# birdnet-team/birdnet-stm32

Hardware: AMD Instinct MI355X
Metric: audio chunks/sec (3 s @ 24 kHz) (higher is better)
Workload: dtype i8

## Files before the change

### birdnet-stm32_amd/birdnet_stm32/_hip.py

```python

from __future__ import annotations

import ctypes
import os
from ctypes import POINTER, byref, c_char_p, c_float, c_int, c_int32, c_int64, c_size_t, c_void_p

_PKG_ROOT = os.path.dirname(os.path.dirname(os.path.abspath(__file__)))
LIB_PATH = os.path.join(_PKG_ROOT, "lib", "libbirdnet_hip.so")

ABI_VERSION = 2

EXPORTS = (
    "bn_version", "bn_last_error", "bn_device_count", "bn_ctx_create", "bn_ctx_destroy", "bn_model_load",
    "bn_model_free", "bn_model_get_info", "bn_stft_mag", "bn_forward", "bn_infer_audio", "bn_debug_op_output",
    "bn_kernel_names", "bn_profile_enable", "bn_profile_collect", "bn_ingest_resample", "bn_ingest_chunks",
    "bn_pool_scores", "bn_mel_spectrogram", "bn_profile_only", "bn_chunk_peak_normalize", "bn_set_option", "bn_get_option", "bn_ctx_set_option", "bn_ctx_get_option", "bn_ctx_reset_options", "bn_preload_kernels", "bn_host_alloc_pinned", "bn_host_free_pinned", "bn_rank_orders",
    "bn_blob_check", "bn_debug_requant", "bn_stft_mag_exact", "bn_debug_input_bytes", "bn_debug_guard_stats", "bn_debug_tail_form", "bn_debug_mid_form", "bn_debug_mid_plan", "bn_debug_mid_split_giveups",
    "bn_forward_embed", "bn_infer_audio_embed", "bn_model_get_embedding_info", "bn_ingest_resample_span",
    "bn_head_forward", "bn_probe_create", "bn_probe_destroy", "bn_probe_epoch", "bn_probe_loss", "bn_probe_get", "bn_probe_set",
    "bn_probe_sweep_create", "bn_probe_sweep_destroy", "bn_probe_sweep_epoch", "bn_probe_sweep_loss", "bn_probe_sweep_snapshot", "bn_probe_sweep_get",
    "bn_probe_set_loss", "bn_probe_epoch_weighted", "bn_probe_sweep_set_loss", "bn_probe_sweep_epoch_weighted",
    "bn_probe_set_qat", "bn_probe_get_quantized", "bn_probe_scores",
    "bn_short_time_energy", "bn_activity_counts", "bn_search_inv_norms", "bn_search_topk", "bn_augment_inputs",
    "bn_kmeans_assign", "bn_kmeans_accumulate", "bn_kmeans_centroids",
    "bn_tsne_perplexity", "bn_tsne_gradient", "bn_tsne_update",
    "bn_bootstrap_rejections", "bn_bootstrap_counts", "bn_bootstrap_ap", "bn_head_i8_forward", "bn_head_i8_pass_classes",
)

EMB_F32, EMB_I8 = 0, 1
PROBE_ACTIVATIONS = {"sigmoid": 0, "softmax": 1}
PROBE_OPTIMIZERS = {"adam": 0, "adamw": 1, "sgd": 2}
PROBE_LOSSES = {"auto": 0, "focal": 1}
PROBE_QAT_WEIGHTS = {"off": 0, "per_class": 1, "per_tensor": 2}
PROBE_MAX_D, PROBE_MAX_C = 2048, 4096
PROBE_SWEEP_MAX_TRIALS = 64
PROBE_SWEEP_CURRENT, PROBE_SWEEP_SNAPSHOT = 0, 1
HEAD_I8_STEP_ROWS, HEAD_I8_MIN_WG_STEPS, HEAD_I8_MAX_WGS, HEAD_I8_LDS_BYTES = 64, 8, 1024, 160 * 1024



def head_i8_pass_classes(D: int, C: int) -> int:
    v = int(load_library().bn_head_i8_pass_classes(int(D), int(C)))
    check(min(v, 0))
    return v


class ProbeTrialStruct(ctypes.Structure):

    _fields_ = [("optimizer", ctypes.c_int32), ("lr", ctypes.c_float), ("weight_decay", ctypes.c_float), ("clipnorm", ctypes.c_float),
                ("dropout", ctypes.c_float), ("label_smoothing", ctypes.c_float)]


DTYPE_F32, DTYPE_I8 = 0, 1
SEARCH_METRICS = {"cosine": 0, "dot": 1}
SEARCH_MAX_K, SEARCH_MAX_D = 128, 2048
AUGMENT_MAX_MASKS = 4
SEARCH_STEP_ROWS, SEARCH_MIN_WG_STEPS, SEARCH_MAX_WGS = 64, 8, 1024
KMEANS_MAX_K, KMEANS_MAX_D = 4096, 2048
BOOTSTRAP_MAX_N = 32768
KMEANS_LDS_BYTES, KMEANS_MAX_TILE, KMEANS_STEP_ROWS, KMEANS_MIN_WG_STEPS, KMEANS_MAX_WGS, KMEANS_SEGMENT_ROWS = 160 * 1024, 128, 64, 8, 1024, 256
TSNE_TILE_I, TSNE_TILE_J, TSNE_SPLIT_J, TSNE_ROW_LANES, TSNE_MAX_K, TSNE_MAX_N = 256, 1024, 4096, 16, 128, 1 << 21


def kmeans_tile_centroids(D: int, K: int) -> int:
    pitch_bytes = (-(-int(D) // 64) * 64 + 4) * 4
    nt = 1
    while nt < KMEANS_MAX_TILE // 16 and 16 * nt < K:
        nt *= 2
    while nt > 1 and 16 * nt * pitch_bytes > KMEANS_LDS_BYTES:
        nt //= 2
    return 16 * nt


OPTION_NAMES = ("f32_strip", "f32_strip_th", "f32_front_staged", "f32_front2", "f32_pwdw", "f32_tile_slice", "f32_pw_ws", "i8_pwdw", "i8_pw_lds", "i8_pw_forms", "i8_add_tab", "front_tpw", "wave_dwpw", "i8_strip", "i8_strip_mfdw", "i8_strip_th", "i8_dw_pool", "i8_tail_fclds", "i8_tail", "i8_tail_mfdw", "i8_mid",
                "i8_mel_generic", "stft_rowmajor", "stft_exact", "stft_flagcap", "stft_guard", "stft_audit", "stft_minint", "ingest_blk", "ingest_generic")
SCHEDULING_OPTION_NAMES = ("i8_mid_split",)


class BnModelInfo(ctypes.Structure):
    _fields_ = [
        ("dtype", c_int32), ("input_kind", c_int32), ("input_elems", c_int32), ("fft_bins", c_int32),
        ("spec_width", c_int32), ("num_classes", c_int32), ("n_ops", c_int32), ("max_batch", c_int32),
        ("workspace_bytes", c_int64), ("const_bytes", c_int64),
    ]


class HipError(RuntimeError):
    """A libbirdnet_hip call returned a negative status."""


_lib = None


def load_library(path: str | None = None):
    global _lib
    if _lib is not None:
        return _lib
    path = path or os.environ.get("BIRDNET_HIP_LIB", LIB_PATH)
    if not os.path.isfile(path):
        raise RuntimeError(
            f"{path} not found: the HIP extension has not been built. Run `python -c 'import __graft_entry__ as g; "
            "g.build()'` (or `make -C birdnet-stm32_amd/csrc`). There is no CPU fallback for this path."
        )
    import torch

    lib = ctypes.CDLL(path)
    for name in EXPORTS:
        if not hasattr(lib, name):
            raise RuntimeError(f"{path} does not export {name}")
    lib.bn_version.restype = c_int
    lib.bn_last_error.restype = c_char_p
    lib.bn_device_count.restype = c_int
    lib.bn_ctx_create.argtypes = [c_int, c_int, POINTER(c_void_p)]
    lib.bn_ctx_destroy.argtypes = [c_void_p]
    lib.bn_ctx_destroy.restype = None
    lib.bn_model_load.argtypes = [c_void_p, c_char_p, c_size_t, POINTER(c_void_p)]
    lib.bn_model_free.argtypes = [c_void_p]
    lib.bn_model_free.restype = None
    lib.bn_model_get_info.argtypes = [c_void_p, POINTER(BnModelInfo)]
    lib.bn_stft_mag.argtypes = [c_void_p, c_void_p, c_int, c_int, c_int, c_int, c_int, c_int, c_void_p, c_void_p, c_void_p]
    lib.bn_stft_mag_exact.argtypes = lib.bn_stft_mag.argtypes
    lib.bn_debug_input_bytes.argtypes = [c_void_p, c_int, c_void_p, c_void_p]
    lib.bn_debug_guard_stats.argtypes = [c_void_p, c_int, POINTER(c_int64)]
    lib.bn_debug_tail_form.argtypes = [c_void_p, POINTER(c_int), POINTER(c_int)]
    lib.bn_debug_mid_form.argtypes = [c_void_p, POINTER(c_int), POINTER(c_int)]
    lib.bn_debug_mid_plan.argtypes = [c_void_p, POINTER(c_int), c_int]
    lib.bn_debug_mid_split_giveups.argtypes = [c_void_p, POINTER(c_int64)]
    lib.bn_forward.argtypes = [c_void_p, c_void_p, c_void_p, c_int, c_void_p, c_void_p, c_void_p]
    lib.bn_infer_audio.argtypes = [c_void_p, c_void_p, c_int, c_int, c_int, c_void_p, c_void_p, c_void_p]
    lib.bn_forward_embed.argtypes = [c_void_p, c_void_p, c_void_p, c_int, c_void_p, c_void_p, c_void_p, c_int, c_void_p]
    lib.bn_infer_audio_embed.argtypes = [c_void_p, c_void_p, c_int, c_int, c_int, c_void_p, c_void_p, c_void_p, c_int, c_void_p]
    lib.bn_model_get_embedding_info.argtypes = [c_void_p, POINTER(c_int), POINTER(c_int), POINTER(c_float), POINTER(c_int)]
    lib.bn_debug_op_output.argtypes = [c_void_p, c_int, c_int, c_void_p, c_size_t, POINTER(c_size_t), c_void_p]
    lib.bn_kernel_names.restype = c_char_p
    lib.bn_profile_enable.argtypes = [c_void_p, c_int]
    lib.bn_profile_only.argtypes = [c_void_p, c_int]
    lib.bn_chunk_peak_normalize.argtypes = [c_void_p, c_void_p, c_int, c_int, c_float, c_void_p, c_void_p]
    lib.bn_profile_collect.argtypes = [c_void_p, POINTER(ctypes.c_double), POINTER(c_int64), c_int]
    lib.bn_ingest_resample.argtypes = [c_void_p, c_void_p, c_int, c_int, c_void_p, c_void_p, c_int, c_int64, c_int64,
                                       c_void_p, c_int, c_int, c_int, c_int, c_void_p, c_void_p, c_void_p]
    lib.bn_ingest_resample_span.argtypes = [c_void_p, c_void_p, c_int, c_int, c_int64, c_int64, c_int64, c_int64, c_int64, c_void_p,
                                            c_int, c_int, c_int, c_int, c_void_p, c_void_p, c_void_p]
    lib.bn_ingest_chunks.argtypes = [c_void_p, c_void_p, c_void_p, c_void_p, c_void_p, c_void_p, c_int, c_int, c_void_p,
                                     c_void_p]
    lib.bn_pool_scores.argtypes = [c_void_p, c_void_p, c_void_p, c_int, c_int, c_int, c_float, c_void_p, c_void_p]
    lib.bn_mel_spectrogram.argtypes = [c_void_p, c_void_p, c_int, c_int, c_int, c_int, c_int, c_void_p, c_void_p, c_int, c_int, c_int,
                                       ctypes.c_double, c_void_p, c_int, c_void_p, c_void_p, c_void_p]
    lib.bn_blob_check.argtypes = [c_char_p, c_size_t]
    lib.bn_debug_requant.argtypes = [c_void_p, c_void_p, c_void_p, c_void_p, c_int, c_int, c_int, c_void_p, c_void_p]
    lib.bn_set_option.argtypes = [c_char_p, c_int]
    lib.bn_get_option.argtypes = [c_char_p, POINTER(c_int)]
    lib.bn_ctx_set_option.argtypes = [c_void_p, c_char_p, c_int]
    lib.bn_ctx_get_option.argtypes = [c_void_p, c_char_p, POINTER(c_int)]
    lib.bn_ctx_reset_options.argtypes = [c_void_p]
    lib.bn_preload_kernels.argtypes = [c_void_p]
    lib.bn_rank_orders.argtypes = [c_void_p, c_void_p, c_int, c_int, c_void_p, c_void_p, c_void_p]
    lib.bn_short_time_energy.argtypes = [c_void_p, c_void_p, c_void_p, c_void_p, c_void_p, c_void_p, c_int, c_int, c_int, c_void_p, c_void_p]
    lib.bn_activity_counts.argtypes = [c_void_p, c_void_p, c_int, c_int64, c_void_p, c_int, c_float, c_void_p, c_void_p, c_void_p]
    lib.bn_search_inv_norms.argtypes = [c_void_p, c_void_p, c_int, c_int64, c_int, c_int, c_void_p, c_void_p]
    lib.bn_search_topk.argtypes = [c_void_p, c_void_p, c_int, c_int64, c_int, c_int, c_void_p, c_void_p, c_int64, c_void_p, c_int, c_void_p, c_void_p,
                                   c_int, c_void_p, c_void_p, c_void_p]
    lib.bn_kmeans_assign.argtypes = [c_void_p, c_void_p, c_int, c_int64, c_int, c_int, c_void_p, c_void_p, c_void_p, c_int, c_void_p, c_void_p, c_void_p,
                                     c_void_p, c_void_p]
    lib.bn_kmeans_accumulate.argtypes = [c_void_p, c_void_p, c_int, c_int64, c_int, c_int, c_void_p, c_void_p, c_int, c_int, c_void_p, c_void_p, c_void_p]
    lib.bn_kmeans_centroids.argtypes = [c_void_p, c_void_p, c_void_p, c_int, c_int, c_void_p, c_void_p, c_void_p]
    lib.bn_tsne_perplexity.argtypes = [c_void_p, c_void_p, c_int64, c_int, ctypes.c_double, c_void_p, c_void_p, c_void_p]
    lib.bn_tsne_gradient.argtypes = [c_void_p, c_void_p, c_int64, c_void_p, c_void_p, c_void_p, c_float, c_void_p, c_void_p, c_void_p, c_void_p]
    lib.bn_tsne_update.argtypes = [c_void_p, c_void_p, c_void_p, c_void_p, c_void_p, c_int64, c_float, c_float, c_void_p]
    u64 = ctypes.c_uint64
    lib.bn_bootstrap_rejections.argtypes = [c_void_p, u64, u64, u64, u64, ctypes.c_uint32, c_int64, c_int64, c_void_p, c_int64, POINTER(c_int64), c_void_p]
    lib.bn_bootstrap_counts.argtypes = [c_void_p, u64, u64, u64, u64, c_int, c_int, c_void_p, c_void_p, c_void_p]
    lib.bn_bootstrap_ap.argtypes = [c_void_p, u64, u64, u64, u64, c_int, c_int, c_void_p, c_void_p, c_void_p, c_void_p, c_int, c_int, c_void_p, c_void_p, c_void_p]
    lib.bn_augment_inputs.argtypes = [c_void_p, c_void_p, c_int64, c_int, c_int, c_void_p, c_void_p, c_void_p, c_void_p, c_int, c_void_p, c_int, c_int64,
                                      c_void_p, c_void_p]
    lib.bn_host_alloc_pinned.argtypes = [c_void_p, ctypes.c_size_t]
    lib.bn_host_alloc_pinned.restype = c_void_p
    lib.bn_host_free_pinned.argtypes = [c_void_p]
    lib.bn_head_forward.argtypes = [c_void_p, c_void_p, c_int64, c_int, c_void_p, c_void_p, c_int, c_int, c_void_p, c_void_p]
    lib.bn_head_i8_forward.argtypes = [c_void_p, c_void_p, c_int64, c_int, c_void_p, c_void_p, c_void_p, c_void_p, c_int, c_int, c_void_p, c_int, c_float,
                                       c_void_p, c_void_p, c_void_p]
    lib.bn_head_i8_pass_classes.argtypes = [c_int, c_int]
    lib.bn_probe_create.argtypes = [c_void_p, c_int, c_int, c_int, c_int, c_float, c_float, c_float, c_float, ctypes.c_uint32, c_int64,
                                    c_void_p, c_void_p, POINTER(c_void_p), c_void_p]
    lib.bn_probe_destroy.argtypes = [c_void_p]
    lib.bn_probe_destroy.restype = None
    lib.bn_probe_epoch.argtypes = [c_void_p, c_void_p, c_void_p, c_void_p, c_int64, c_int, c_void_p, c_void_p]
    lib.bn_probe_loss.argtypes = [c_void_p, c_void_p, c_void_p, c_int64, c_void_p, c_void_p]
    lib.bn_probe_get.argtypes = [c_void_p, c_void_p, c_void_p, c_void_p]
    lib.bn_probe_set.argtypes = [c_void_p, c_void_p, c_void_p, c_void_p]
    lib.bn_probe_sweep_create.argtypes = [c_void_p, c_int, c_int, c_int, c_int, POINTER(ProbeTrialStruct), ctypes.c_uint32, c_int64, c_void_p, c_void_p,
                                          POINTER(c_void_p), c_void_p]
    lib.bn_probe_sweep_destroy.argtypes = [c_void_p]
    lib.bn_probe_sweep_destroy.restype = None
    lib.bn_probe_sweep_epoch.argtypes = [c_void_p, c_void_p, c_void_p, c_void_p, c_int64, c_int, c_void_p, c_void_p, c_void_p, c_void_p]
    lib.bn_probe_sweep_loss.argtypes = [c_void_p, c_void_p, c_void_p, c_int64, c_void_p, c_void_p, c_void_p]
    lib.bn_probe_sweep_snapshot.argtypes = [c_void_p, c_void_p, c_void_p]
    lib.bn_probe_sweep_get.argtypes = [c_void_p, c_int, c_int, c_void_p, c_void_p, c_void_p]
    lib.bn_probe_set_loss.argtypes = [c_void_p, c_int, c_float]
    lib.bn_probe_epoch_weighted.argtypes = [c_void_p, c_void_p, c_void_p, c_void_p, c_void_p, c_int64, c_int, c_void_p, c_void_p]
    lib.bn_probe_sweep_set_loss.argtypes = [c_void_p, c_int, c_float]
    lib.bn_probe_set_qat.argtypes = [c_void_p, c_int, c_int, c_float, c_int]
    lib.bn_probe_get_quantized.argtypes = [c_void_p, c_void_p, c_void_p]
    lib.bn_probe_scores.argtypes = [c_void_p, c_void_p, c_int64, c_void_p, c_void_p, c_void_p]
    lib.bn_probe_sweep_epoch_weighted.argtypes = [c_void_p, c_void_p, c_void_p, c_void_p, c_void_p, c_int64, c_int, c_void_p, c_void_p, c_void_p, c_void_p]
    if lib.bn_version() != ABI_VERSION:
        raise RuntimeError(f"libbirdnet_hip ABI {lib.bn_version()} != binding ABI {ABI_VERSION}")
    _lib = lib
    return lib


# ... 120 lines not shown
```

### birdnet-stm32_amd/birdnet_stm32/models/_lower_i8.py

```python

from __future__ import annotations

import numpy as np

from birdnet_stm32.models import _pack as pk
from birdnet_stm32.models import _quant as qz
from birdnet_stm32.models._netspec import same_pad

K_ALIGN = 64


class _Graph:
    def __init__(self, model):
        self.m = model
        self.t = model.tensors
        self.consumers: dict[int, list[int]] = {}
        for op in model.ops:
            for ti in op.inputs:
                if ti >= 0:
                    self.consumers.setdefault(ti, []).append(op.index)

    def q(self, ti: int) -> tuple[float, int]:
        t = self.t[ti]
        if t.scale.size != 1:
# ... 892 lines not shown
            val[op.outputs[0]], shape[op.outputs[0]] = v, (C,)
            i += 1
        elif op.name == "FULLY_CONNECTED":
            Cin = int(shape[src][-1])
            _expect(int(np.prod(shape[src])) == Cin, "FULLY_CONNECTED input must be a vector per chunk")
            s_i, z_i = g.q(src)
            s_o, z_o = g.q(op.outputs[0])
            wt_ = t[op.inputs[1]]
            Cout = int(wt_.shape[0])
            _expect(int(wt_.shape[1]) == Cin, "FULLY_CONNECTED weight shape")
            mu, sh = qz.channel_multipliers(s_i, wt_.scale, s_o, Cout)
            a_lo, a_hi = qz.activation_bounds(op.options["activation"], s_o, z_o)
            b = g.const(op.inputs[2]).astype(np.int64) if len(op.inputs) > 2 and op.inputs[2] >= 0 else np.zeros(Cout, np.int64)
            b = b - z_i * wt_.data.astype(np.int64).sum(axis=1)
            _expect_acc_range(wt_.data, b, 1, f"fully connected operator #{op.index}", mu, sh)
            Kp = (Cin + 3) // 4 * 4
            w_pad = np.zeros((Cout, Kp), np.int8)
            w_pad[:, :Cin] = wt_.data
            nxt = ops[i + 1] if i + 1 < len(ops) else None
            fold_lut = (nxt is not None and nxt.name == "LOGISTIC" and nxt.inputs[0] == op.outputs[0] and g.consumers.get(op.outputs[0], []) == [nxt.index]
                        and i + 2 < len(ops) and ops[i + 2].name != "DEQUANTIZE")
            tt = dict(w=pb.tensor(w_pad, np.int8), bias=pb.tensor(b, np.int32), mult=pb.tensor(mu, np.int32), shift=pb.tensor(sh, np.int32))
            out_t = op.outputs[0]
            if fold_lut:
                s_h, z_h = g.q(nxt.outputs[0])
                tt["lut"] = pb.tensor(qz.logistic_table(s_o, z_o, s_h, z_h), np.int8)
                out_t = nxt.outputs[0]
            v = pb.value(Cout)
            if not fold_lut:
                tail_head.update(fc_op=len(plan.ops), fc_cin=Cin, NC=Cout, fc_zp_out=z_o, fc_lo=a_lo, fc_hi=a_hi, fc_w=wt_.data, fc_b=b, fc_m=mu, fc_s=sh)
            pb.op(pk.I8_FC, val[src], v, p=dict(Cin=Cin, Cout=Cout, zp_out=z_o, act_min=a_lo, act_max=a_hi, has_lut=int(fold_lut)), t=tt, name=f"t{out_t}", out_shape=(Cout,), out_dtype="int8")
            val[out_t], shape[out_t] = v, (Cout,)
            i += 2 if fold_lut else 1
        elif op.name == "MUL":
            a_t, b_t = op.inputs
            if len(shape[a_t]) != 3:
                a_t, b_t = b_t, a_t
            _expect(len(shape[a_t]) == 3 and int(np.prod(shape[b_t])) == shape[a_t][2] and shape[a_t][2] % 4 == 0, "MUL must scale a map by a per-channel vector")
            H, Wd, C = shape[a_t]
            s1, z1 = g.q(a_t)
            s2, z2 = g.q(b_t)
            so, zo = g.q(op.outputs[0])
            mu, sh = qz.quantize_multiplier(float(np.float32(s1)) * float(np.float32(s2)) / float(np.float32(so)))
            lo_, hi_ = qz.activation_bounds(op.options["activation"], so, zo)
            v = pb.value(H * Wd * C)
            pb.op(pk.I8_SCALE, val[a_t], v, in1=val[b_t], p=dict(P=H * Wd, C=C, zp_x=z1, zp_gate=z2, mult=mu, shift=sh, zp_out=zo, act_min=lo_, act_max=hi_),
                  name=f"t{op.outputs[0]}", out_shape=(H, Wd, C), out_dtype="int8")
            val[op.outputs[0]], shape[op.outputs[0]] = v, (H, Wd, C)
            i += 1
        elif op.name in ("LOGISTIC", "DEQUANTIZE"):
            fc_out = src
            _expect(len(shape[fc_out]) == 1, "the head must follow the classifier")
            Cout = shape[fc_out][0]
            s_fc, z_fc = g.q(fc_out)
            lut_t, s_h, z_h, has = -1, s_fc, z_fc, 0
            if op.name == "LOGISTIC":
                s_h, z_h = g.q(op.outputs[0])
                lut_t, has = pb.tensor(qz.logistic_table(s_fc, z_fc, s_h, z_h), np.int8), 1
                last = op.outputs[0]
                i += 1
            else:
                last = fc_out
            _expect(i < len(ops) and ops[i].name == "DEQUANTIZE" and ops[i].inputs[0] == last, "DEQUANTIZE must end the graph")
            softmax, beta = 0, 1.0
            if i + 1 < len(ops) and ops[i + 1].name == "SOFTMAX":
                _expect(not has and ops[i + 1].inputs[0] == ops[i].outputs[0], "float32 SOFTMAX must read the dequantised classifier output")
                softmax, beta = 1, float(ops[i + 1].options.get("beta", 1.0))
                i += 1
            if not softmax:
                tail_head.update(head_op=len(plan.ops), lut=qz.logistic_table(s_fc, z_fc, s_h, z_h) if has else None, zp_fc=z_fc, zp_head=z_h, s_fc=s_fc, s_head=s_h)
            pb.op(pk.I8_HEAD, val[fc_out], pk.SLOT_SCORES, p=dict(C=Cout, zp_fc=z_fc, zp_out=z_h, has_lut=has, softmax=softmax),
                  f=dict(s_fc=s_fc, s_out=s_h, beta=beta), t=dict(lut=lut_t), name=f"t{ops[i].outputs[0]}",
                  out_shape=(Cout,))
            i += 1
            _expect(i == len(ops), "operators after the head")
        else:
            _expect(False, f"operator #{op.index} {op.name} in the backbone")
    _mark_embedding(g, plan)
    if fuse and not keep_all:
        _add_tail_op(pb, plan, tail_blocks, tail_head)
        _tag_scale_pairs(pb)
        _tag_se_gates(pb)
        _tag_pwdw_pairs(pb)
    return pb.finalize(reuse=not keep_all)


def _mark_embedding(g: _Graph, plan: pk.Plan) -> None:
    ops = plan.ops
    writer = {o.out: i for i, o in enumerate(ops) if o.out >= 0}
    heads = [o for o in ops if o.kind == pk.I8_HEAD]
    if len(heads) != 1 or heads[0].in0 not in writer:
        return
    fc = ops[writer[heads[0].in0]]
    if fc.kind != pk.I8_FC or fc.in0 not in writer:
        return
    pool = ops[writer[fc.in0]]
    if pool.kind not in (pk.I8_MEAN, pk.I8_ATTNPOOL) or not pool.name.startswith("t"):
        return
    s, z = g.q(int(pool.name[1:]))
    pk.mark_embedding(pool, pool.get("C"), float(np.float32(s)), z)


def _tag_se_gates(pb: pk.PlanBuilder) -> None:
    ops = pb.plan.ops
    for i in range(len(ops) - 2):
        a, f1, f2 = ops[i], ops[i + 1], ops[i + 2]
        if a.kind != pk.I8_MEAN or f1.kind != pk.I8_FC or f2.kind != pk.I8_FC or f1.in0 != a.out or f2.in0 != f1.out:
            continue
        C, Cr = a.get("C"), f1.get("Cout")
        if f1.get("Cin") != C or f2.get("Cin") != Cr or Cr > 256 or C > 1024 or C % 4:
            continue
        others = [k for k, o in enumerate(ops) if (k != i + 1 and a.out in (o.in0, o.in1)) or (k != i + 2 and f1.out in (o.in0, o.in1))]
        if others or a.out < 0 or f1.out < 0 or f2.out < 0:
            continue
        a.p[pk.TAIL_TAG] = pk.SEGATE_HEAD
        f1.p[pk.TAIL_TAG] = f2.p[pk.TAIL_TAG] = pk.SEGATE_COVERED
        pb._extra_uses.append((i + 2, a.in0))


def _tag_pwdw_pairs(pb: pk.PlanBuilder) -> None:
    ops = pb.plan.ops
    for i in range(len(ops) - 1):
        e, d = ops[i], ops[i + 1]
        if e.kind != pk.I8_DWPW or d.kind != pk.I8_DW or any(e.get(k) for k in ("has_dw", "transposed", "has_add", "has_lut", "q_at_load")) or d.in0 != e.out or e.out < 0:
            continue
        if e.p[pk.TAIL_TAG] or d.p[pk.TAIL_TAG] or e.p[pk.OP_PATH] != d.p[pk.OP_PATH]:
            continue
        if d.get("C") != e.get("Cout") or (d.get("H"), d.get("W")) != (e.get("OH"), e.get("OW")) or d.get("zp_in") != e.get("pw_zp_out"):
            continue
        readers = [k for k, o in enumerate(ops) if k != i + 1 and e.out in (o.in0, o.in1)]
        writers = [k for k, o in enumerate(ops) if o.out == e.out]
        if readers or writers != [i]:
            continue
        e.p[pk.TAIL_TAG] = pk.PWDW8_HEAD
        d.p[pk.TAIL_TAG] = pk.PWDW8_COVERED
        if e.in0 >= 0:
            pb._extra_uses.append((i + 1, e.in0))


def _tag_scale_pairs(pb: pk.PlanBuilder) -> None:
    ops = pb.plan.ops
    for i in range(len(ops) - 1):
        a, b = ops[i], ops[i + 1]
        if a.kind != pk.I8_SCALE or b.kind != pk.I8_DWPW or any(b.get(k) for k in ("has_dw", "transposed", "has_lut", "q_at_load")) or b.in0 != a.out:
            continue
        if b.get("Cin") != a.get("C") or b.get("H") * b.get("W") != a.get("P") or b.get("Cin") > 768 or (b.get("sh"), b.get("sw")) != (1, 1):
            continue
        readers = [k for k, o in enumerate(ops) if k != i + 1 and a.out in (o.in0, o.in1)]
        if readers or b.in1 == a.out:
            continue
        a.p[pk.TAIL_TAG] = pk.SCALE_HEAD
        b.p[pk.TAIL_TAG] = pk.SCALE_COVERED
        pb._extra_uses.append((i + 1, a.in0))
        pb._extra_uses.append((i + 1, a.in1))


def _add_mid_op(pb, plan, blocks: list[dict]) -> None:
    if len(blocks) < 3:
        return
    chain = blocks[-3:]
    a, b, c = chain
    if (a["C"], a["N"], a["sh"], a["H"], a["W"], bool(a["add"][0])) != (32, 64, 2, 32, 64, False):
        return
    for blk in (b, c):
        if (blk["C"], blk["N"], blk["sh"], blk["H"], blk["W"], bool(blk["add"][0])) != (64, 64, 1, 16, 32, True) or not blk["res_is_input"]:
            return
    ops_idx = [blk["op"] for blk in chain]
# ... 55 lines not shown
```

### birdnet-stm32_amd/birdnet_stm32/models/runners.py

```python

from __future__ import annotations

import ctypes

import numpy as np

from birdnet_stm32 import _hip
from birdnet_stm32.models import _pack as pk


class HipRunner:

    def __init__(self, plan: pk.Plan, device: int = 0, max_batch: int = 1024, ctx: "_hip.Context | None" = None):
        import torch

        if not torch.cuda.is_available():
            raise RuntimeError("no ROCm device visible: HipRunner has no CPU fallback")
        self._torch = torch
        self.plan = plan
        self.device = torch.device("cuda", device)
        self.ctx = ctx if ctx is not None else _hip.Context(device, max_batch)
        self.model = _hip.Model(self.ctx, plan.to_blob())
        self.lib = self.ctx.lib
        info = self.model.info
# ... 150 lines not shown
        if self.input_kind in (pk.INPUT_MEL, pk.INPUT_WAVEFORM):
            res = self.predict_device(self.model_inputs_device(audio), return_logits=return_logits, **kw)
            if out is not None:
                out.copy_(res[0] if isinstance(res, tuple) else res)
            return res
        B, T = audio.shape
        hop = int(hop) if hop is not None else T // self.spec_width
        scores = out if out is not None else torch.empty((B, self.num_classes), dtype=torch.float32, device=self.device)
        logits = torch.empty_like(scores) if return_logits else None
        emb, code = (None, 0)
        if return_embeddings:
            emb, code = self._emb_buffer(B, emb_dtype, emb_out)
        with torch.cuda.device(self.device):
            for b0 in range(0, B, self.max_batch):
                nb = min(self.max_batch, B - b0)
                if emb is not None:
                    _hip.check(self.lib.bn_infer_audio_embed(self.model.handle, audio[b0:].data_ptr(), nb, T, hop, scores[b0:].data_ptr(),
                                                             logits[b0:].data_ptr() if logits is not None else None, emb[b0:].data_ptr(), code,
                                                             self._stream()))
                    continue
                _hip.check(
                    self.lib.bn_infer_audio(
                        self.model.handle, audio[b0:].data_ptr(), nb, T, hop, scores[b0:].data_ptr(),
                        logits[b0:].data_ptr() if logits is not None else None, self._stream(),
                    )
                )
        if emb is not None:
            return (scores, logits, emb) if return_logits else (scores, emb)
        return (scores, logits) if return_logits else scores

    def stft_device(self, audio, n_fft: int = 512, hop: int | None = None, spec_width: int | None = None, normalize: bool = True,
                    exact: bool = False):
        return stft_device(self.ctx, audio, n_fft, hop, spec_width or self.spec_width, normalize, exact=exact)

    def op_output(self, op_index: int, B: int) -> np.ndarray:
        torch = self._torch
        op = self.plan.ops[op_index]
        per = ctypes.c_size_t()
        _hip.check(self.lib.bn_debug_op_output(self.model.handle, op_index, B, None, 0, ctypes.byref(per), None))
        buf = torch.empty((B, per.value), dtype=torch.uint8, device=self.device)
        _hip.check(self.lib.bn_debug_op_output(self.model.handle, op_index, B, buf.data_ptr(), buf.numel(), ctypes.byref(per), self._stream()))
        torch.cuda.synchronize(self.device)
        raw = buf.cpu().numpy().reshape(-1)
        n = int(np.prod(op.out_shape))
        dt = np.dtype(op.out_dtype)
        return raw[: B * n * dt.itemsize].copy().view(dt).reshape(B, *op.out_shape)

    def input_bytes(self, B: int) -> np.ndarray:
        torch = self._torch
        out = torch.empty((B, self.fft_bins, self.spec_width), dtype=torch.int8, device=self.device)
        _hip.check(self.lib.bn_debug_input_bytes(self.model.handle, B, out.data_ptr(), self._stream()))
        torch.cuda.synchronize(self.device)
        return out.cpu().numpy()

    def guard_stats(self, B: int) -> dict:
        out = (ctypes.c_int64 * 8)()
        _hip.check(self.lib.bn_debug_guard_stats(self.model.handle, B, out))
        return {"listed": int(out[0]), "listed_max": int(out[1]), "dirty_blocks": int(out[2]), "whole_minmax": int(out[3]), "whole_fix": int(out[4]),
                "audited": int(out[5]), "audit_violations": int(out[6]), "interval_min": int(out[7])}

    def tail_form(self) -> tuple[int, int]:
        form, lds = ctypes.c_int(0), ctypes.c_int(0)
        _hip.check(self.lib.bn_debug_tail_form(self.model.handle, ctypes.byref(form), ctypes.byref(lds)))
        return form.value, lds.value

    def mid_form(self) -> tuple[int, int]:
        form, lds = ctypes.c_int(0), ctypes.c_int(0)
        _hip.check(self.lib.bn_debug_mid_form(self.model.handle, ctypes.byref(form), ctypes.byref(lds)))
        return form.value, lds.value

    def mid_plan(self) -> dict | None:
        out = (ctypes.c_int * 64)()
        _hip.check(self.lib.bn_debug_mid_plan(self.model.handle, out, 64))
        if not out[0]:
            return None
        parts = [(out[5 + 6 * i + 2 * k], out[6 + 6 * i + 2 * k]) for i in range(out[4]) for k in range(3) if out[6 + 6 * i + 2 * k]]
        return {"lds_bytes": out[1], "map_bytes": out[2], "bar_off": out[3], "blocks": out[4], "parts": parts}

    def mid_split_giveups(self) -> int:
        n = ctypes.c_int64(0)
        _hip.check(self.lib.bn_debug_mid_split_giveups(self.ctx.handle, ctypes.byref(n)))
        return int(n.value)

    def profile(self, enable: bool) -> None:
        _hip.check(self.lib.bn_profile_enable(self.model.handle, int(bool(enable))))

    def profile_only(self, op_index: int) -> None:
        _hip.check(self.lib.bn_profile_only(self.model.handle, int(op_index)))

    def profile_collect(self) -> list[dict]:
        n = len(self.plan.ops) + 3
        ms = (ctypes.c_double * n)()
        cnt = (ctypes.c_int64 * n)()
        _hip.check(self.lib.bn_profile_collect(self.model.handle, ms, cnt, n))
        rows = []
        for i in range(n):
            if i < len(self.plan.ops):
                op = self.plan.ops[i]
                rows.append({"op": i, "kind": pk.KIND_NAMES[op.kind], "name": op.name, "ms": ms[i], "launches": int(cnt[i]), "p": list(op.p)})
            else:
                kind, name = (("stft512", "stft"), ("stft_minmax_exact", "exact min/max"), ("stft512_f64_list", "float64 pass + redo"))[i - len(self.plan.ops)]
                rows.append({"op": i, "kind": kind, "name": name, "ms": ms[i], "launches": int(cnt[i]), "p": []})
        return rows

    def close(self):
        import sys

        pl = sys.modules.get("birdnet_stm32.audio.pipeline")
        if pl is not None:
            while pl._PREPARE:
                pl._PREPARE.pop().join()
        self.model.close()
        self.ctx.close()


def stft_device(ctx: _hip.Context, audio, n_fft: int = 512, hop: int | None = None, spec_width: int = 256, normalize: bool = True,
                return_minmax: bool = False, exact: bool = False):
    import torch

    if not (audio.is_cuda and audio.dtype == torch.float32 and audio.is_contiguous() and audio.dim() == 2):
        raise ValueError("audio must be a contiguous float32 CUDA tensor [B, T]")
    B, T = audio.shape
    hop = int(hop) if hop is not None else T // spec_width
    spec = torch.empty((B, n_fft // 2 + 1, spec_width), dtype=torch.float32, device=audio.device)
    minmax = torch.empty((B, 2), dtype=torch.float32, device=audio.device)
    with torch.cuda.device(audio.device):
        stream = ctypes.c_void_p(torch.cuda.current_stream(audio.device).cuda_stream)
        fn = ctx.lib.bn_stft_mag_exact if exact else ctx.lib.bn_stft_mag
        _hip.check(fn(ctx.handle, audio.data_ptr(), B, T, n_fft, hop, spec_width, int(normalize), spec.data_ptr(), minmax.data_ptr(), stream))
    return (spec, minmax) if return_minmax else spec


def lower_model_file(model_path: str, keep_all: bool = False, frontend_norm: bool | None = None, fuse: bool = True) -> pk.Plan:
    if model_path.lower().endswith(".tflite"):
        from birdnet_stm32.models._lower_i8 import lower_i8
        from birdnet_stm32.models._tflite_reader import load_tflite

        return lower_i8(load_tflite(model_path), keep_all=keep_all, fuse=fuse)
    from birdnet_stm32.models._keras_loader import load_keras_archive
    from birdnet_stm32.models._lower_f32 import lower_f32

    return lower_f32(load_keras_archive(model_path, frontend_norm=frontend_norm), keep_all=keep_all, fuse=fuse)


def load_model_runner(model_path: str, device: int = 0, max_batch: int = 1024, keep_all: bool = False,
                      frontend_norm: bool | None = None, fuse: bool = True, prepare_pipeline: bool = False) -> HipRunner:
    ctx = None
    if prepare_pipeline:
        import torch

        if not torch.cuda.is_available():
            raise RuntimeError("no ROCm device visible: HipRunner has no CPU fallback")
        from birdnet_stm32.audio.pipeline import prepare_for_evaluate

        ctx = _hip.Context(device, max_batch)
        prepare_for_evaluate(ctx, torch)
    plan = lower_model_file(model_path, keep_all=keep_all, frontend_norm=frontend_norm, fuse=fuse)
    return HipRunner(plan, device=device, max_batch=max_batch, ctx=ctx)
```

### birdnet-stm32_amd/csrc/bn_api.hip

```cpp
#include <hip/hip_runtime.h>

#include <algorithm>
#include <cctype>
#include <cmath>
#include <cstdarg>
#include <cstdio>
#include <cstdlib>
#include <cstring>
#include <string>
#include <vector>

#include "bn_model.h"

namespace {

thread_local std::string g_err;

constexpr int kFft = 512;

struct OptName {
    const char* name;
    int bn::Options::*field;
};
const OptName kOptions[] = {
    {"f32_strip", &bn::Options::f32_strip},       {"f32_strip_th", &bn::Options::f32_strip_th},
    {"f32_front_staged", &bn::Options::f32_front_staged}, {"f32_front2", &bn::Options::f32_front2}, {"f32_pwdw", &bn::Options::f32_pwdw}, {"f32_tile_slice", &bn::Options::f32_tile_slice}, {"f32_pw_ws", &bn::Options::f32_pw_ws}, {"i8_pwdw", &bn::Options::i8_pwdw}, {"i8_pw_lds", &bn::Options::i8_pw_lds}, {"i8_pw_forms", &bn::Options::i8_pw_forms}, {"i8_add_tab", &bn::Options::i8_add_tab}, {"front_tpw", &bn::Options::front_tpw},
    {"wave_dwpw", &bn::Options::wave_dwpw},       {"i8_strip", &bn::Options::i8_strip},
    {"i8_strip_th", &bn::Options::i8_strip_th}, {"i8_dw_pool", &bn::Options::i8_dw_pool}, {"i8_tail_fclds", &bn::Options::i8_tail_fclds},   {"i8_tail", &bn::Options::i8_tail}, {"i8_tail_mfdw", &bn::Options::i8_tail_mfdw}, {"i8_mid", &bn::Options::i8_mid}, {"i8_mid_split", &bn::Options::i8_mid_split},
    {"i8_mel_generic", &bn::Options::i8_mel_generic}, {"stft_rowmajor", &bn::Options::stft_rowmajor},
    {"i8_strip_mfdw", &bn::Options::i8_strip_mfdw}, {"stft_exact", &bn::Options::stft_exact}, {"stft_flagcap", &bn::Options::stft_flagcap}, {"stft_guard", &bn::Options::stft_guard}, {"stft_audit", &bn::Options::stft_audit}, {"stft_minint", &bn::Options::stft_minint},
    {"ingest_blk", &bn::Options::ingest_blk},
    {"ingest_generic", &bn::Options::ingest_generic},
};

bn::Options options_from_env() {
    bn::Options o;
    for (const OptName& e : kOptions) {
        std::string var = "BN_";
        for (const char* c = e.name; *c; ++c) var += (char)toupper((unsigned char)*c);
        if (const char* v = getenv(var.c_str())) o.*(e.field) = atoi(v);
    }
    return o;
}

}

namespace bn {
thread_local Options g_opt;

int fail(int code, const char* fmt, ...) {
    char buf[512];
    va_list ap;
    va_start(ap, fmt);
    vsnprintf(buf, sizeof buf, fmt, ap);
    va_end(ap);
    g_err = buf;
    return code;
}
}
using bn::fail;
using bn::kMaxGridBatch;
using bn::ProfScope;

bn::Options g_opt_default = options_from_env();
std::mutex g_opt_mu;

namespace bn {

int check_device(bn_ctx* ctx) {
    if (!ctx) return fail(BN_ERR_ARG, "null context");
    HIP_TRY(hipSetDevice(ctx->device));
    {
        std::lock_guard<std::mutex> lock(g_opt_mu);
        bn::g_opt = g_opt_default;
        for (const auto& ov : ctx->opt_override) bn::g_opt.*(ov.first) = ov.second;
    }
    return BN_OK;
}

int grow_device_buffer(void** p, size_t* have, size_t need, size_t alloc, hipStream_t s, int code, const char* what) {
    if (need <= *have) return BN_OK;
    HIP_TRY(hipStreamSynchronize(s));
    if (*p) (void)hipFree(*p);
    *p = nullptr;
    *have = 0;
    if (hipMalloc(p, alloc) != hipSuccess) {
        (void)hipGetLastError();
        return fail(code, "hipMalloc of %zu bytes for the %s workspace failed", alloc, what);
    }
    *have = alloc;
    return BN_OK;
}

}
using bn::check_device;
using bn::grow_device_buffer;

namespace {

int row_matrix_check(int dtype, int64_t n, int D, int max_D, int zero_point) {
    if (dtype != BN_DTYPE_F32 && dtype != BN_DTYPE_I8) return fail(BN_ERR_ARG, "unknown dtype %d", dtype);
    if (D < 1 || D > max_D) return fail(BN_ERR_ARG, "embedding width D=%d outside 1..%d", D, max_D);
    if (n < 0 || n > 0x7fffffffLL) return fail(BN_ERR_ARG, "bad row count %lld", (long long)n);
    if (dtype == BN_DTYPE_I8 && (zero_point < -128 || zero_point > 127)) return fail(BN_ERR_ARG, "zero point %d outside -128..127", zero_point);
    return BN_OK;
}

}

extern "C" {

int bn_version(void) { return BN_ABI_VERSION; }

// ... 444 lines not shown
    int rc = BN_OK;
    if (guarded) {
        if (T <= 0 || hop <= 0 || 1 + T / hop < W) rc = fail(BN_ERR_ARG, "T=%d hop=%d gives %d frames, fewer than spec_width=%d", T, hop, hop > 0 ? 1 + T / hop : 0, W);
        if (m->d_audit) HIP_TRY(hipMemsetAsync(m->d_audit, 0, 2 * sizeof(int), s));
        for (int b0 = 0; rc == BN_OK && b0 < B; b0 += kMaxGridBatch) {
            const int nb = B - b0 < kMaxGridBatch ? B - b0 : kMaxGridBatch;
            bn::StftGuard g = bn::guard_slice(m, (size_t)b0, bn::SpecStage{tiled, true, d_audio + (size_t)b0 * T, T, hop});
            {
                ProfScope prof(m, (int)m->ops.size(), s);
                bn::launch_stft512(m->ctx->tables, d_audio + (size_t)b0 * T, nb, T, hop, W, m->d_spec + b0 * in_stride, m->d_minmax + 2 * (size_t)b0, s,
                                   true, &g);
            }
            ProfScope prof(m, (int)m->ops.size() + 1, s);
            bn::launch_stft_minmax_exact(m->ctx->tables, d_audio + (size_t)b0 * T, nb, T, hop, W, m->d_spec + b0 * in_stride, true, g,
                                         m->d_minmax + 2 * (size_t)b0, s);
        }
    } else {
        ProfScope prof(m, (int)m->ops.size(), s);
        rc = stft_mag_impl(m->ctx, d_audio, B, T, kFft, hop, W, 0, m->d_spec, m->d_minmax, stream, tiled, exact_opt != 0);
    }
    if (rc == BN_OK) {
        for (int b0 = 0; b0 < B; b0 += kMaxGridBatch) {
            const int nb = B - b0 < kMaxGridBatch ? B - b0 : kMaxGridBatch;
            bn::RunArgs ra{m->d_spec + b0 * in_stride, m->d_minmax + 2 * (size_t)b0, nb, d_scores + b0 * C, d_logits ? d_logits + b0 * C : nullptr,
                           d_emb ? (char*)d_emb + b0 * D * esize : nullptr, emb_dtype, s};
            ra.slot_b0 = (size_t)b0;
            ra.spec = bn::SpecStage{tiled, guarded, d_audio + (size_t)b0 * T, T, hop};
            rc = bn::run_plan(m, ra);
            if (rc != BN_OK) break;
        }
    }
    m->last_tiled = tiled;
    m->last_B = rc == BN_OK ? B : 0;
    return rc;
}

extern "C" {

int bn_debug_tail_form(const bn_model* m, int* form, int* lds_bytes) {
    if (!m || !form || !lds_bytes) return fail(BN_ERR_ARG, "null argument");
    *form = 0;
    *lds_bytes = 0;
    for (size_t oi = 0; oi < m->ops.size(); ++oi) {
        if (m->ops[oi].kind != BN_OP_I8_TAIL || !m->prep[oi]->ok) continue;
        const bn::OpPrep& pr = *m->prep[oi];
        *form = pr.alt_ok ? 2 : 1;
        *lds_bytes = pr.alt_ok ? pr.chain.lds_bytes : pr.tail.lds_bytes;
    }
    return BN_OK;
}

int bn_debug_mid_form(const bn_model* m, int* form, int* lds_bytes) {
    if (!m || !form || !lds_bytes) return fail(BN_ERR_ARG, "null argument");
    *form = 0;
    *lds_bytes = 0;
    for (size_t oi = 0; oi < m->ops.size(); ++oi)
        if (m->ops[oi].kind == BN_OP_I8_MID && m->prep[oi]->ok) {
            *form = 1;
            *lds_bytes = m->prep[oi]->chain.lds_bytes;
        }
    return BN_OK;
}

int bn_debug_mid_plan(const bn_model* m, int* out, int n) {
    if (!m || !out || n < 1) return fail(BN_ERR_ARG, "null argument");
    out[0] = 0;
    for (size_t oi = 0; oi < m->ops.size(); ++oi)
        if (m->ops[oi].kind == BN_OP_I8_MID && m->prep[oi]->ok && m->prep[oi]->alt_ok) {
            if (!bn::tail2_plan_dump(m->prep[oi]->resident, out, n)) return fail(BN_ERR_ARG, "n=%d is too small for the plan", n);
            break;
        }
    return BN_OK;
}

int bn_debug_mid_split_giveups(bn_ctx* ctx, int64_t* count) {
    if (!ctx || !count) return fail(BN_ERR_ARG, "null argument");
    if (int rc = check_device(ctx)) return rc;
    const long n = bn::tail2_giveups();
    if (n < 0) return fail(BN_ERR_DEVICE, "could not read the chunk barriers' give-up counter");
    *count = n;
    return BN_OK;
}

int bn_debug_guard_stats(bn_model* m, int B, int64_t* out) {
    if (!m || !out) return fail(BN_ERR_ARG, "null argument");
    if (int rc = check_device(m->ctx)) return rc;
    if (!m->d_guard) return fail(BN_ERR_UNSUPPORTED, "the plan has no exactness pass");
    if (B <= 0 || B > m->last_B || B > kMaxGridBatch) return fail(BN_ERR_ARG, "B=%d: the last bn_infer_audio call left %d spectrograms", B, m->last_B);
    HIP_TRY(hipDeviceSynchronize());
    std::vector<int> cnt((size_t)B);
    int nw = 0, nh[2] = {0, 0};
    HIP_TRY(hipMemcpy(cnt.data(), m->guard.count, (size_t)B * sizeof(int), hipMemcpyDeviceToHost));
    HIP_TRY(hipMemcpy(&nw, m->guard.n_work, sizeof(int), hipMemcpyDeviceToHost));
    HIP_TRY(hipMemcpy(nh, m->guard.n_hard, 2 * sizeof(int), hipMemcpyDeviceToHost));
    int64_t total = 0, mx = 0;
    for (int c : cnt) {
        c %= m->guard.cap + 1;
        total += c;
        if (c > mx) mx = c;
    }
    out[0] = total;
    out[1] = mx;
    out[2] = nw;
    out[3] = nh[0];
    out[4] = nh[1];
    int au[2] = {0, 0};
    if (m->d_audit) HIP_TRY(hipMemcpy(au, m->d_audit, sizeof au, hipMemcpyDeviceToHost));
    out[5] = au[0];
    out[6] = au[1];
    std::vector<float> lo((size_t)B);
    HIP_TRY(hipMemcpy(lo.data(), m->guard.mn_lo, (size_t)B * sizeof(float), hipMemcpyDeviceToHost));
    int64_t wide = 0;
    for (float v : lo) wide += v >= 0.0f;
    out[7] = wide;
    return BN_OK;
}

int bn_debug_input_bytes(bn_model* m, int B, int8_t* d_out, void* stream) {
    if (!m || !d_out) return fail(BN_ERR_ARG, "null argument");
    if (int rc = check_device(m->ctx)) return rc;
    namespace k = bn::op::i8_dwpw;
    const OpRec* first = nullptr;
    for (const OpRec& o : m->ops)
        if (o.in0 == BN_SLOT_INPUT && o.kind == BN_OP_I8_DWPW && o.p[k::q_at_load] && o.p[k::transposed]) first = &o;
    if (!first || !m->d_spec) return fail(BN_ERR_UNSUPPORTED, "the plan's first operator is not the mel mixer with QUANTIZE fused into its load");
    if (B <= 0 || B > m->last_B || B > kMaxGridBatch) return fail(BN_ERR_ARG, "B=%d: the last bn_infer_audio call left %d spectrograms", B, m->last_B);
    bn::launch_spec_bytes(m->d_spec, m->d_minmax, B, (int)m->hdr.spec_width, m->last_tiled, first->f[k::qscale], first->p[k::qzp], d_out, (hipStream_t)stream);
    HIP_TRY(hipGetLastError());
    return BN_OK;
}

int bn_ingest_resample(bn_ctx* ctx, const void* d_pcm, int sample_format, int channels, const int64_t* d_in_off,
                       const int64_t* d_out_off, int n_windows, int64_t max_in_len, int64_t max_out_len, const float* d_taps,
                       int up, int down, int taps_per_phase, int n_pre_remove, float* d_mono, float* d_peak, void* stream) {
    if (int rc = check_device(ctx)) return rc;
    if (!d_pcm || !d_in_off || !d_out_off || !d_mono || !d_peak) return fail(BN_ERR_ARG, "null device pointer");
    if (sample_format < BN_PCM_S16 || sample_format > BN_PCM_F32) return fail(BN_ERR_ARG, "unknown sample format %d", sample_format);
    if (channels < 1 || channels > 8)
        return fail(BN_ERR_UNSUPPORTED, "%d channels: the channel mean is implemented for 1..8 channels", channels);
    if (n_windows < 0 || max_in_len < 0 || max_out_len < 0 || up < 1 || down < 1 || taps_per_phase < 0 || n_pre_remove < 0)
        return fail(BN_ERR_ARG, "bad ingest geometry");
    if (taps_per_phase > 0 && !d_taps) return fail(BN_ERR_ARG, "null filter");
    if (taps_per_phase == 0 && up != down) return fail(BN_ERR_ARG, "up=%d down=%d needs a filter", up, down);
    if (n_windows == 0 || max_out_len == 0) return BN_OK;
    if (n_windows > 65535) return fail(BN_ERR_ARG, "at most 65535 windows per call");
    if ((double)(max_out_len + n_pre_remove + 4096) * down >= 4294967296.0 || (double)max_in_len * up >= 4294967296.0)
        return fail(BN_ERR_UNSUPPORTED, "window too long for the 32-bit polyphase index (%lld samples, up=%d, down=%d)",
                    (long long)max_in_len, up, down);
    const size_t lds = bn::ingest_resample_lds_bytes(up, down, taps_per_phase, bn::ingest_resample_block(up, down, taps_per_phase));
    const bool fast_kernel = (up == 1 && (down == 2 || down == 4)) || (up > 1 && up <= 256 && (taps_per_phase == 21 || taps_per_phase == 29 || taps_per_phase == 39));
    if (lds > (fast_kernel ? 64 : 156) * 1024)
        return fail(BN_ERR_UNSUPPORTED, "resampling ratio %d/%d needs %zu bytes of LDS per workgroup (limit %d)", up, down, lds, (fast_kernel ? 64 : 156) * 1024);
    hipStream_t s = (hipStream_t)stream;
    const size_t need = bn::ingest_partial_elems(n_windows, (long)max_out_len, up, down, taps_per_phase);
    if (need > ctx->block_peaks_elems) {
        if (ctx->d_block_peaks) HIP_TRY(hipFree(ctx->d_block_peaks));
        ctx->d_block_peaks = nullptr;
        ctx->block_peaks_elems = 0;
        HIP_TRY(hipMalloc(&ctx->d_block_peaks, need * sizeof(float)));
        ctx->block_peaks_elems = need;
    }
    bn::launch_ingest_resample(d_pcm, sample_format, channels, (const long*)d_in_off, (const long*)d_out_off, n_windows,
                               (long)max_out_len, d_taps, up, down, taps_per_phase, n_pre_remove, d_mono, ctx->d_block_peaks,
                               d_peak, s);
    HIP_TRY(hipGetLastError());
    return BN_OK;
// ... 220 lines not shown

int bn_ctx_set_option(bn_ctx* ctx, const char* name, int value) {
    if (!ctx || !name) return fail(BN_ERR_ARG, "null argument");
    for (const OptName& e : kOptions)
        if (strcmp(name, e.name) == 0) {
            std::lock_guard<std::mutex> lock(g_opt_mu);
            for (auto& ov : ctx->opt_override)
                if (ov.first == e.field) {
                    ov.second = value;
                    return BN_OK;
                }
            ctx->opt_override.emplace_back(e.field, value);
            return BN_OK;
        }
    return fail(BN_ERR_ARG, "unknown option '%s'", name);
}

int bn_ctx_get_option(bn_ctx* ctx, const char* name, int* value) {
    if (!ctx || !name || !value) return fail(BN_ERR_ARG, "null argument");
    for (const OptName& e : kOptions)
        if (strcmp(name, e.name) == 0) {
            std::lock_guard<std::mutex> lock(g_opt_mu);
            *value = g_opt_default.*(e.field);
            for (const auto& ov : ctx->opt_override)
                if (ov.first == e.field) *value = ov.second;
            return BN_OK;
        }
    return fail(BN_ERR_ARG, "unknown option '%s'", name);
}

int bn_ctx_reset_options(bn_ctx* ctx) {
    if (!ctx) return fail(BN_ERR_ARG, "null context");
    std::lock_guard<std::mutex> lock(g_opt_mu);
    ctx->opt_override.clear();
    return BN_OK;
}

void* bn_host_alloc_pinned(bn_ctx* ctx, size_t bytes) {
    if (!ctx || bytes == 0) {
        fail(BN_ERR_ARG, "null context or empty allocation");
        return nullptr;
    }
    if (check_device(ctx) != BN_OK) return nullptr;
    void* p = nullptr;
    if (hipHostMalloc(&p, bytes, hipHostMallocDefault) != hipSuccess) {
        (void)hipGetLastError();
        fail(BN_ERR_DEVICE, "hipHostMalloc of %zu bytes failed", bytes);
        return nullptr;
    }
    return p;
}

int bn_host_free_pinned(void* p) {
    if (p && hipHostFree(p) != hipSuccess) {
        (void)hipGetLastError();
        return fail(BN_ERR_DEVICE, "hipHostFree failed");
    }
    return BN_OK;
}

int bn_preload_kernels(bn_ctx* ctx) {
    if (!ctx) return fail(BN_ERR_ARG, "null context");
    if (int rc = check_device(ctx)) return rc;
    bn::preload_ingest(); bn::preload_stft(); bn::preload_stft_exact(); bn::preload_i8_fused(); bn::preload_i8_strip(); bn::preload_i8_tail2();
    bn::preload_i8_tail(); bn::preload_i8(); bn::preload_i8_pw(); bn::preload_f32(); bn::preload_f32_fused(); bn::preload_f32_strip();
    bn::preload_f32_pw(); bn::preload_melspec(); bn::preload_sort(); bn::preload_probe(); bn::preload_probe_sweep(); bn::preload_activity(); bn::preload_search(); bn::preload_augment(); bn::preload_kmeans(); bn::preload_tsne(); bn::preload_bootstrap(); bn::preload_head_i8();
    return BN_OK;
}

int bn_get_option(const char* name, int* value) {
    if (!name || !value) return fail(BN_ERR_ARG, "null argument");
    for (const OptName& e : kOptions)
        if (strcmp(name, e.name) == 0) {
            std::lock_guard<std::mutex> lock(g_opt_mu);
            *value = g_opt_default.*(e.field);
            return BN_OK;
        }
    return fail(BN_ERR_ARG, "unknown option '%s'", name);
}

const char* bn_kernel_names(void) {
    return "ingest_resample_kernel\ningest_decimate_kernel\ningest_peak_kernel\ningest_chunks_kernel\nchunk_peaknorm_kernel\npool_scores_kernel\nstft512_mag_kernel\nspec_normalize_kernel\nmelspec_finish_kernel\nf32_mel_kernel\nf32_melfin_kernel\nf32_mag_kernel\nf32_rawfe_kernel\nf32_stem_kernel\nf32_dw_kernel\n"
           "f32_pw_kernel\nf32_pw_ws_kernel\nf32_dwpw_kernel\nf32_dwpw_wave_kernel\nf32_strip_kernel\nf32_front_strip_kernel\nf32_front2_kernel\nf32_pwdw_kernel\nf32_dw_stream_kernel\nf32_front_kernel\nf32_gap_kernel\nf32_gap_dense_kernel\nf32_gap_dense_emb_kernel\nf32_dense_kernel\nf32_segate_kernel\nf32_scale_kernel\nf32_attnpool_kernel\n"
           "i8_quant_kernel\ni8_mel_kernel\ni8_stem_kernel\ni8_dw_kernel\ni8_pw_kernel\ni8_dwpw_kernel\ni8_mel_mfma_kernel\ni8_strip_kernel\ni8_strip_mf_kernel\ni8_front_strip_kernel\ni8_front_kernel\ni8_tail_kernel\ni8_tail_emb_kernel\ni8_tail2_kernel\ni8_tail2_emb_kernel\ni8_mid2_kernel\ni8_mean_kernel\ni8_fc_kernel\ni8_scale_kernel\ni8_maxnorm_kernel\ni8_rawfe_kernel\ni8_pwdw_kernel\ni8_dw_stream_kernel\ni8_stem_stream_kernel\ni8_segate_kernel\ni8_pw_wave_kernel\ni8_pw_lds_kernel\ni8_attnpool_kernel\n"
           "i8_head_kernel\ni8_head_softmax_kernel\nemb_store_kernel\nprobe_fwd_kernel\nprobe_dw_kernel\nprobe_reduce_kernel\nprobe_update_kernel\nprobe_loss_sum_kernel\nprobe_sweep_snapshot_kernel\nste_kernel\nactivity_count_kernel\nsearch_inv_norms_kernel\nsearch_score_kernel\nsearch_merge_kernel\naugment_kernel\nkmeans_assign_kernel\nkmeans_keys_kernel\nkmeans_offsets_kernel\nkmeans_segments_kernel\nkmeans_partial_kernel\nkmeans_fold_kernel\nkmeans_scale_kernel\ntsne_perplexity_kernel\ntsne_repulsion_kernel\ntsne_fold_kernel\ntsne_z_kernel\ntsne_attraction_kernel\ntsne_update_kernel\nbootstrap_table_kernel\nbootstrap_reject_kernel\nbootstrap_prepare_kernel\nbootstrap_resample_kernel\nhead_i8_kernel";
}

}

extern "C" {

int bn_search_inv_norms(bn_ctx* ctx, const void* d_rows, int dtype, int64_t n, int D, int zero_point, float* d_inv, void* stream) {
    if (int rc = check_device(ctx)) return rc;
    if (int rc = row_matrix_check(dtype, n, D, BN_SEARCH_MAX_D, zero_point)) return rc;
    if (!d_rows || !d_inv) return fail(BN_ERR_ARG, "null device pointer");
    if (dtype == BN_DTYPE_F32 && (uintptr_t)d_rows % 4) return fail(BN_ERR_ARG, "float32 rows must be 4-byte aligned");
    if (n == 0) return BN_OK;
    bn::launch_search_inv_norms(d_rows, dtype == BN_DTYPE_I8, (long)n, D, zero_point, d_inv, (hipStream_t)stream);
    HIP_TRY(hipGetLastError());
    return BN_OK;
}

int bn_search_topk(bn_ctx* ctx, const void* d_db, int dtype, int64_t n, int D, int zero_point, const float* d_db_inv, const void* d_queries,
                   int64_t Q, const float* d_q_inv, int metric, const int32_t* d_db_group, const int32_t* d_q_group, int k, int32_t* d_idx,
                   float* d_score, void* stream) {
    if (int rc = check_device(ctx)) return rc;
    if (int rc = row_matrix_check(dtype, n, D, BN_SEARCH_MAX_D, zero_point)) return rc;
    if (k < 1 || k > BN_SEARCH_MAX_K) return fail(BN_ERR_ARG, "k=%d outside 1..%d", k, BN_SEARCH_MAX_K);
    if (Q < 0 || Q > 0x7fffffffLL) return fail(BN_ERR_ARG, "bad query count %lld", (long long)Q);
    if (metric != BN_SEARCH_COSINE && metric != BN_SEARCH_DOT) return fail(BN_ERR_ARG, "unknown metric %d", metric);
    if (!d_db || !d_queries || !d_idx || !d_score) return fail(BN_ERR_ARG, "null device pointer");
    if (metric == BN_SEARCH_COSINE && (!d_db_inv || !d_q_inv)) return fail(BN_ERR_ARG, "the cosine metric needs both inverse-norm arrays");
    if ((d_db_group == nullptr) != (d_q_group == nullptr)) return fail(BN_ERR_ARG, "d_db_group and d_q_group go together");
    if (dtype == BN_DTYPE_F32 && ((uintptr_t)d_db % 4 || (uintptr_t)d_queries % 4)) return fail(BN_ERR_ARG, "float32 rows must be 4-byte aligned");
    if (Q == 0) return BN_OK;
    const bool i8 = dtype == BN_DTYPE_I8;
    hipStream_t s = (hipStream_t)stream;
    bn::SearchGeom g{};
    if (!bn::search_geometry((long)n, D, (int)Q, k, i8, &g)) return fail(BN_ERR_ARG, "D=%d k=%d: no query tile fits the LDS", D, k);
    const size_t per_query = (size_t)g.nwg * k * (sizeof(float) + sizeof(int32_t));
    const int pass_q = 16 * g.nt;
    int64_t group = (int64_t)(BN_SEARCH_WORKSPACE_BYTES / per_query) / pass_q * pass_q;
    if (group < pass_q) group = pass_q;
    if (group > Q) group = Q;
    const size_t need = (size_t)group * per_query;
    if (int rc = grow_device_buffer(&ctx->d_search_work, &ctx->search_work_bytes, need, need, s, BN_ERR_NOMEM, "search")) return rc;
    float* part_score = (float*)ctx->d_search_work;
    int* part_idx = (int*)(part_score + (size_t)group * g.nwg * k);
    const size_t row_bytes = (size_t)D * (i8 ? 1 : 4);
    for (int64_t q0 = 0; q0 < Q; q0 += group) {
        const int nq = (int)std::min<int64_t>(group, Q - q0);
        bn::SearchArgs a{};
        a.db = d_db; a.q = (const char*)d_queries + (size_t)q0 * row_bytes;
        a.db_inv = d_db_inv; a.q_inv = d_q_inv ? d_q_inv + q0 : nullptr;
        a.db_group = d_db_group; a.q_group = d_q_group ? d_q_group + q0 : nullptr;
        a.part_score = part_score; a.part_idx = part_idx;
        a.n = (int)n; a.D = D; a.Q = nq; a.k = k; a.zp = i8 ? zero_point : 0; a.cosine = metric == BN_SEARCH_COSINE;
        a.steps_per_wg = g.steps_per_wg;
        if (!bn::launch_search_scores(a, g, i8, s)) return fail(BN_ERR_DEVICE, "the search kernel's LDS request was refused");
        bn::launch_search_merge(part_score, part_idx, g.nwg, nq, k, d_idx + (size_t)q0 * k, d_score + (size_t)q0 * k, s);
        HIP_TRY(hipGetLastError());
    }
    return BN_OK;
}

}

namespace {

int kmeans_shape_check(int dtype, int64_t n, int D, int K, int zero_point) {
    if (int rc = row_matrix_check(dtype, n, D, BN_KMEANS_MAX_D, zero_point)) return rc;
    if (K < 1 || K > BN_KMEANS_MAX_K) return fail(BN_ERR_ARG, "K=%d outside 1..%d", K, BN_KMEANS_MAX_K);
    return BN_OK;
}

}

extern "C" {

int bn_kmeans_assign(bn_ctx* ctx, const void* d_rows, int dtype, int64_t n, int D, int zero_point, const float* d_row_inv, const float* d_centroids,
                     const float* d_cent_inv, int K, const int32_t* d_prev_label, int32_t* d_label, float* d_score, int64_t* d_changed, void* stream) {
    if (int rc = check_device(ctx)) return rc;
    if (int rc = kmeans_shape_check(dtype, n, D, K, zero_point)) return rc;
    if (!d_rows || !d_row_inv || !d_centroids || !d_cent_inv || !d_label || !d_score || !d_changed) return fail(BN_ERR_ARG, "null device pointer");
    if (d_prev_label == d_label) return fail(BN_ERR_ARG, "d_prev_label must not be d_label");
    if (dtype == BN_DTYPE_F32 && (uintptr_t)d_rows % 4) return fail(BN_ERR_ARG, "float32 rows must be 4-byte aligned");
    if ((uintptr_t)d_row_inv % 4 || (uintptr_t)d_centroids % 4 || (uintptr_t)d_cent_inv % 4 || (uintptr_t)d_prev_label % 4 || (uintptr_t)d_label % 4 ||
// ... 204 lines not shown
```

### birdnet-stm32_amd/csrc/bn_i8_strip.hip

```cpp
#include <stdlib.h>

#include "bn_kernels.h"
#include "bn_requant.h"

namespace bn {
namespace {

template <int QL> struct RawRow { int t[3][QL]; };
template <int QL> struct TRow { int c[QL][4]; };

template <int QL>
__device__ __forceinline__ RawRow<QL> load_row(__amdgpu_buffer_rsrc_t rsrc, const int voff[3], int soff) {
    RawRow<QL> r;
#pragma unroll
    for (int j = 0; j < 3; ++j) {
        if constexpr (QL == 2) {
            const v2i v = __builtin_bit_cast(v2i, __builtin_amdgcn_raw_buffer_load_b64(rsrc, voff[j], soff, 0));
            r.t[j][0] = v.x; r.t[j][1] = v.y;
        } else {
            const v4i v = __builtin_bit_cast(v4i, __builtin_amdgcn_raw_buffer_load_b128(rsrc, voff[j], soff, 0));
            r.t[j][0] = v.x; r.t[j][1] = v.y; r.t[j][2] = v.z; r.t[j][3] = v.w;
        }
    }
    return r;
}

template <int CW, int NW, int COUT, int S, bool ADD, bool W8 = false>
__global__ __launch_bounds__(64 * NW * (ADD ? 8 / NW : (NW == 1 ? 4 : 1)))
__attribute__((amdgpu_waves_per_eu(CW == 32 ? (((S == 1 && !ADD && COUT / NW >= 64) || W8) ? 3 : 4) : 2)))
void i8_strip_kernel(Strip8Args a) {
    constexpr int CIN = CW * NW, CL = CW / 4, QL = CL / 4;
    constexpr int CWO = COUT / NW, NT = CWO / 16, COL = CWO / 4;
    constexpr int SPB = ADD ? 8 / NW : (NW == 1 ? 4 : 1);
    constexpr int NTHREADS = 64 * NW * SPB;
    static_assert(NW == 1 || CW == 32, "the channel split works on 32-channel slices");
    static_assert(!ADD || (CIN == COUT && S == 1), "the residual is the block input");
    static_assert(NT == 2 || NT == 4, "8 or 16 output channels per lane");
    constexpr int nDWW = 4 * QL * 12, nDWB = 4 * QL * 4, nDWC = 4 * QL * 12, nPWA = NT * NW * 64 * QL, nPWB = 4 * NT * 4, nPWC = 4 * NT * 12;
    constexpr int kDWW = 0;
    constexpr int kDWB = kDWW + NW * nDWW;
    constexpr int kDWC = kDWB + NW * nDWB;
    constexpr int kPWA = kDWC + NW * nDWC;
    constexpr int kPWB = kPWA + NW * nPWA;
    constexpr int kPWC = kPWB + NW * nPWB;
    extern __shared__ __attribute__((aligned(16))) unsigned char lds_all[];
    const unsigned char* add_tab = lds_all;
    v4i* c_dw = reinterpret_cast<v4i*>(lds_all + (ADD ? 65536 : 0));
    v4i* c_pw = c_dw + NW * nDWC / 3;
    v4i* c_dww = c_pw + NW * nPWC / 3;
    constexpr bool DWW_LDS = NW > 1;
    v2i* xchg = reinterpret_cast<v2i*>(c_dww + (DWW_LDS ? NW * nDWW / 4 : 0));
    const int tid = threadIdx.x;
    {
        const v4i* src = reinterpret_cast<const v4i*>(a.cst);
        auto stage = [&](v4i* dst, const v4i* q3, int n_quads, bool fold) {
            for (int i = tid; i < n_quads; i += NTHREADS) {
                const v4i m = q3[3 * i], c1 = q3[3 * i + 1], sh = q3[3 * i + 2];
                dst[4 * i] = m;
                if (fold) {
                    const long c[4] = {rq64(c1.x), rq64(c1.y), rq64(c1.z), rq64(c1.w)};
                    dst[4 * i + 1] = (v4i){(int)c[0], (int)(c[0] >> 32), (int)c[1], (int)(c[1] >> 32)};
                    dst[4 * i + 2] = (v4i){(int)c[2], (int)(c[2] >> 32), (int)c[3], (int)(c[3] >> 32)};
                    dst[4 * i + 3] = (v4i){pack_shifts(sh - 1), 0, 0, 0};
                } else {
                    dst[4 * i + 1] = c1;
                    dst[4 * i + 2] = sh;
                    dst[4 * i + 3] = (v4i){0, 0, 0, 0};
                }
            }
        };
        stage(c_dw, src + kDWC / 4, NW * nDWC / 12, true);
        stage(c_pw, src + kPWC / 4, NW * nPWC / 12, !ADD);
        if constexpr (DWW_LDS)
            for (int i = tid; i < NW * nDWW / 4; i += NTHREADS) c_dww[i] = src[kDWW / 4 + i];
        if constexpr (ADD) {
            const v4i* tsrc = reinterpret_cast<const v4i*>(a.add_tab);
            v4i* tdst = reinterpret_cast<v4i*>(lds_all);
            for (int i = tid; i < 4096; i += NTHREADS) tdst[i] = tsrc[i];
        }
    }
    __syncthreads();

    const int lane = tid & 63;
    const int wave = __builtin_amdgcn_readfirstlane(tid >> 6);
// ... 171 lines not shown
    auto epi_part = [&](const v4i (&acc)[NT], const int (&cenv)[QL], int oh) {
        int outw[NT];
#pragma unroll
        for (int t = 0; t < NT; ++t) {
            const v4i m = my_pw[(kq * NT + t) * 4 + 0], c1 = my_pw[(kq * NT + t) * 4 + 1], sh = my_pw[(kq * NT + t) * 4 + 2];
            const int e1 = ADD ? 0 : reinterpret_cast<const int*>(my_pw + (kq * NT + t) * 4 + 3)[0];
            const long cc[4] = {__builtin_bit_cast(long, (v2i){c1.x, c1.y}), __builtin_bit_cast(long, (v2i){c1.z, c1.w}),
                                __builtin_bit_cast(long, (v2i){sh.x, sh.y}), __builtin_bit_cast(long, (v2i){sh.z, sh.w})};
            int qv[4];
#pragma unroll
            for (int e = 0; e < 4; ++e) {
                int v = med3(ADD ? rq(acc[t][e], m[e], c1[e], sh[e]) : rq_hi(acc[t][e], m[e], cc[e], e1, e), a.pw_lo, a.pw_hi);
                if constexpr (ADD)
                    v = add_tab[(uint32_t)perm(cenv[t % QL], v, 0x0c0c0400u + (e << 8))];
                qv[e] = v;
            }
            outw[t] = perm(perm(qv[3], qv[2], 0x0c0c0400u), perm(qv[1], qv[0], 0x0c0c0400u), 0x05040100u);
        }
        const int soff = oh * a.OW * COUT;
        if constexpr (NT == 2) {
            __builtin_amdgcn_raw_buffer_store_b64(__builtin_bit_cast(__attribute__((__vector_size__(2 * sizeof(int)))) int, (v2i){outw[0], outw[1]}), rs_out, voff_out, soff, 0);
        } else {
            v4i ov = {outw[0], outw[1], outw[2], outw[3]};
            __builtin_amdgcn_raw_buffer_store_b128(__builtin_bit_cast(__attribute__((__vector_size__(4 * sizeof(int)))) int, ov), rs_out, voff_out, soff, 0);
            asm volatile("s_nop 1" : "+v"(ov));
        }
    };
    v4i pacc[NT];
    int pcen[QL] = {};
    int poh = 0;
    auto emit = [&](int i0, int i1, int i2, int oh, int step) {
        int bfrag[QL];
        dw_part(i0, i1, i2, bfrag);
        if constexpr (NW > 1 && !PIPE) {
            v2i* buf = xchg + ((step & 1) * SPB + wave / NW) * (NW * 64);
            buf[w * 64 + lane] = (v2i){bfrag[0], bfrag[1]};
            lds_barrier();
            v4i acc[NT];
            mma_part(bfrag, buf, acc);
            epi_part(acc, cen[i1], oh);
        } else if constexpr (PIPE) {
            v2i* buf = xchg + ((step & 1) * SPB + wave / NW) * (NW * 64);
            buf[w * 64 + lane] = (v2i){bfrag[0], bfrag[1]};
            if (step > 0) epi_part(pacc, pcen, poh);
            lds_barrier();
            mma_part(bfrag, buf, pacc);
#pragma unroll
            for (int ql = 0; ql < QL; ++ql) pcen[ql] = cen[i1][ql];
            poh = oh;
        } else {
            v4i acc[NT];
            mma_part(bfrag, nullptr, acc);
            epi_part(acc, cen[i1], oh);
        }
    };

    constexpr int P = 3 - S;
    issue(0, 0);
    issue(1, 1);
#pragma unroll
    for (int rr = 0; rr < P; ++rr) {
        consume(rr & 1, rr, rr % 3);
        issue(rr & 1, rr + 2);
    }
    constexpr int U = 6 / S;
    for (int k = 0; k < steps; k += U) {
#pragma unroll
        for (int u = 0; u < U; ++u) {
            if (k + u >= steps) break;
#pragma unroll
            for (int s = 0; s < S; ++s) {
                const int rs = P + S * u + s;
                consume(rs & 1, S * k + rs, rs % 3);
                issue(rs & 1, S * k + rs + 2);
            }
            emit((S * u) % 3, (S * u + 1) % 3, (S * u + 2) % 3, oh0 + k + u, k + u);
        }
    }
    if constexpr (PIPE) {
        if (steps > 0) epi_part(pacc, pcen, poh);
    }
}

__global__ __launch_bounds__(512) __attribute__((amdgpu_waves_per_eu(4))) void i8_strip_mf_kernel(Strip8Args a) {
    constexpr int CIN = 32, COUT = 32, QL = 2, NT = 2, NW = 1, SPB = 8, NTHREADS = 512;
    constexpr int nDWW = 4 * QL * 12, nDWB = 4 * QL * 4, nDWC = 4 * QL * 12, nPWA = NT * NW * 64 * QL, nPWB = 4 * NT * 4;
    constexpr int kDWW = 0, kDWB = kDWW + nDWW, kDWC = kDWB + nDWB, kPWA = kDWC + nDWC, kPWB = kPWA + nPWA, kPWC = kPWB + nPWB;
    extern __shared__ __attribute__((aligned(16))) unsigned char lds_all[];
    const unsigned char* add_tab = lds_all;
    v4i* c_dw = reinterpret_cast<v4i*>(lds_all + 65536);
    v4i* c_pw = c_dw + nDWC / 3;
    const int tid = threadIdx.x;
    {
        const v4i* src = reinterpret_cast<const v4i*>(a.cst);
        for (int i = tid; i < nDWC / 12; i += NTHREADS) {
            const v4i m = src[kDWC / 4 + 3 * i], c1 = src[kDWC / 4 + 3 * i + 1], sh = src[kDWC / 4 + 3 * i + 2];
            const long c[4] = {rq64(c1.x), rq64(c1.y), rq64(c1.z), rq64(c1.w)};
            c_dw[4 * i] = m;
            c_dw[4 * i + 1] = (v4i){(int)c[0], (int)(c[0] >> 32), (int)c[1], (int)(c[1] >> 32)};
            c_dw[4 * i + 2] = (v4i){(int)c[2], (int)(c[2] >> 32), (int)c[3], (int)(c[3] >> 32)};
            c_dw[4 * i + 3] = (v4i){pack_shifts(sh - 1), 0, 0, 0};
        }
        for (int i = tid; i < 4 * NT; i += NTHREADS) {
            c_pw[4 * i] = src[kPWC / 4 + 3 * i];
            c_pw[4 * i + 1] = src[kPWC / 4 + 3 * i + 1];
            c_pw[4 * i + 2] = src[kPWC / 4 + 3 * i + 2];
            c_pw[4 * i + 3] = (v4i){0, 0, 0, 0};
        }
        const v4i* tsrc = reinterpret_cast<const v4i*>(a.add_tab);
        v4i* tdst = reinterpret_cast<v4i*>(lds_all);
        for (int i = tid; i < 4096; i += NTHREADS) tdst[i] = tsrc[i];
    }
    __syncthreads();

    const int lane = tid & 63;
    const int wave = __builtin_amdgcn_readfirstlane(tid >> 6);
    const int n = lane & 15, g = lane >> 4;
    const int strips_x = a.OW >> 4;
    const int rblocks = (a.OH + a.TH - 1) / a.TH;
    int wid = xcd_tile(blockIdx.x, gridDim.x) * SPB + wave;
    if (wid >= a.B * strips_x * rblocks) return;
    const int sx = wid % strips_x;
    wid /= strips_x;
    const int ry = wid % rblocks;
    const int chunk = wid / rblocks;
    const int oh0 = ry * a.TH;
    const int steps = (a.OH - oh0) < a.TH ? (a.OH - oh0) : a.TH;
    const int ow = sx * 16 + n;

    v4i dwa[2][3];
    v4i dwb[2];
#pragma unroll
    for (int ct = 0; ct < 2; ++ct) {
        const int c = 16 * ct + n;
#pragma unroll
        for (int dy = 0; dy < 3; ++dy) {
            const int taps = a.cst[kDWW + (((c >> 3) * QL + ((c >> 2) & 1)) * 3 + dy) * 4 + (c & 3)];
            const int b = g < 3 ? ((taps >> (8 * g)) & 0xff) << (8 * (n & 3)) : 0;
            dwa[ct][dy] = (v4i){(n >> 2) == 0 ? b : 0, (n >> 2) == 1 ? b : 0, (n >> 2) == 2 ? b : 0, (n >> 2) == 3 ? b : 0};
        }
        dwb[ct] = reinterpret_cast<const v4i*>(a.cst + kDWB)[4 * ct + g];
    }
    long pwa[NT];
    v4i pwb[NT];
#pragma unroll
    for (int t = 0; t < NT; ++t) {
        const uint32_t lo = (uint32_t)a.cst[kPWA + (t * 64 + (n + 16 * (g >> 1))) * QL + (g & 1)];
        const uint32_t hi = (uint32_t)a.cst[kPWA + (t * 64 + (n + 16 * (2 + (g >> 1)))) * QL + (g & 1)];
        pwa[t] = (long)(((unsigned long)hi << 32) | lo);
        pwb[t] = reinterpret_cast<const v4i*>(a.cst + kPWB)[g * NT + t];
    }

    const int zp4 = (a.zp_in & 0xff) * 0x01010101;
    const v4i zrow = {zp4, zp4, zp4, zp4};
    const int icol = ow + g - 1;
    const bool outside = g < 3 && (icol < 0 || icol >= a.W);
    const bool outer = sx == 0 || sx == strips_x - 1;
    const int in_chunk_bytes = a.H * a.W * CIN, row_bytes = a.W * CIN;
    const __amdgpu_buffer_rsrc_t rs_in =
        __builtin_amdgcn_make_buffer_rsrc(const_cast<int8_t*>(a.x) + (size_t)chunk * in_chunk_bytes, 0, in_chunk_bytes, 0x00020000);
    const __amdgpu_buffer_rsrc_t rs_out =
        __builtin_amdgcn_make_buffer_rsrc(a.y + (size_t)chunk * a.OH * a.OW * COUT, 0, a.OH * a.OW * COUT, 0x00020000);
    const int ccol = g == 3 ? icol - 1 : icol;
    const int voff_b = (ccol < 0 ? 0 : (ccol >= a.W ? a.W - 1 : ccol)) * CIN;
    const int voff_r = ow * CIN + 8 * g;
    const int voff_out = ow * COUT + 8 * g;
    const int ir0 = oh0 - a.pt;
    const int rows_needed = steps + 2;

    v4i rawb[2][2];
    v2i rawr[2];
    v4i brow[3][2];
    v2i cen[3];
    auto row_ok = [&](int rr) { const int ir = ir0 + rr; return rr < rows_needed && ir >= 0 && ir < a.H; };
    auto issue = [&](int slot, int rr) {
        if (row_ok(rr)) {
            const int so = (ir0 + rr) * row_bytes;
            rawb[slot][0] = __builtin_bit_cast(v4i, __builtin_amdgcn_raw_buffer_load_b128(rs_in, voff_b, so, 0));
            rawb[slot][1] = __builtin_bit_cast(v4i, __builtin_amdgcn_raw_buffer_load_b128(rs_in, voff_b + 16, so, 0));
            rawr[slot] = __builtin_bit_cast(v2i, __builtin_amdgcn_raw_buffer_load_b64(rs_in, voff_r, so, 0));
        }
    };
    auto consume = [&](int slot, int rr, int ti) {
        if (row_ok(rr)) {
            brow[ti][0] = rawb[slot][0];
            brow[ti][1] = rawb[slot][1];
            if (outer) {
#pragma unroll
                for (int ct = 0; ct < 2; ++ct)
#pragma unroll
                    for (int e = 0; e < 4; ++e) brow[ti][ct][e] = outside ? zp4 : brow[ti][ct][e];
            }
            cen[ti] = rawr[slot];
        } else {
            brow[ti][0] = zrow;
            brow[ti][1] = zrow;
            cen[ti] = (v2i){zp4, zp4};
        }
    };
    auto emit = [&](int i0, int i1, int i2, int oh) {
        asm volatile("" ::: "memory");
        int bfrag[2];
        v4i acc[2];
#pragma unroll
        for (int ct = 0; ct < 2; ++ct) acc[ct] = __builtin_amdgcn_mfma_i32_16x16x64_i8(dwa[ct][0], brow[i0][ct], dwb[ct], 0, 0, 0);
#pragma unroll
        for (int ct = 0; ct < 2; ++ct) acc[ct] = __builtin_amdgcn_mfma_i32_16x16x64_i8(dwa[ct][1], brow[i1][ct], acc[ct], 0, 0, 0);
#pragma unroll
        for (int ct = 0; ct < 2; ++ct) acc[ct] = __builtin_amdgcn_mfma_i32_16x16x64_i8(dwa[ct][2], brow[i2][ct], acc[ct], 0, 0, 0);
#pragma unroll
        for (int ct = 0; ct < 2; ++ct) {
            const int q = 4 * ct + g;
            const v4i m = c_dw[q * 4 + 0], c01 = c_dw[q * 4 + 1], c23 = c_dw[q * 4 + 2];
            const int e1 = reinterpret_cast<const int*>(c_dw + q * 4 + 3)[0];
            const long cc[4] = {__builtin_bit_cast(long, (v2i){c01.x, c01.y}), __builtin_bit_cast(long, (v2i){c01.z, c01.w}),
                                __builtin_bit_cast(long, (v2i){c23.x, c23.y}), __builtin_bit_cast(long, (v2i){c23.z, c23.w})};
            int qv[4];
#pragma unroll
            for (int e = 0; e < 4; ++e) qv[e] = med3(rq_hi(acc[ct][e], m[e], cc[e], e1, e), a.dw_lo, a.dw_hi);
            bfrag[ct] = perm(perm(qv[3], qv[2], 0x0c0c0400u), perm(qv[1], qv[0], 0x0c0c0400u), 0x05040100u);
        }
        const long bf = ((long)(uint32_t)bfrag[1] << 32) | (uint32_t)bfrag[0];
        int outw[NT];
#pragma unroll
        for (int t = 0; t < NT; ++t) {
            const v4i pacc = __builtin_amdgcn_mfma_i32_16x16x32_i8(pwa[t], bf, pwb[t], 0, 0, 0);
            const v4i m = c_pw[(g * NT + t) * 4 + 0], c1 = c_pw[(g * NT + t) * 4 + 1], sh = c_pw[(g * NT + t) * 4 + 2];
            int qv[4];
#pragma unroll
            for (int e = 0; e < 4; ++e) {
                const int v = med3(rq(pacc[e], m[e], c1[e], sh[e]), a.pw_lo, a.pw_hi);
                qv[e] = add_tab[(uint32_t)perm(cen[i1][t], v, 0x0c0c0400u + (e << 8))];
            }
            outw[t] = perm(perm(qv[3], qv[2], 0x0c0c0400u), perm(qv[1], qv[0], 0x0c0c0400u), 0x05040100u);
        }
        __builtin_amdgcn_raw_buffer_store_b64(__builtin_bit_cast(__attribute__((__vector_size__(2 * sizeof(int)))) int, (v2i){outw[0], outw[1]}), rs_out, voff_out,
                                              oh * a.OW * COUT, 0);
    };

    issue(0, 0);
    issue(1, 1);
#pragma unroll
    for (int rr = 0; rr < 2; ++rr) {
        consume(rr & 1, rr, rr % 3);
        issue(rr & 1, rr + 2);
    }
    for (int k = 0; k < steps; k += 6) {
#pragma unroll
        for (int u = 0; u < 6; ++u) {
            if (k + u >= steps) break;
            const int rs = 2 + u;
            consume(rs & 1, k + rs, rs % 3);
            issue(rs & 1, k + rs + 2);
            emit(u % 3, (u + 1) % 3, (u + 2) % 3, oh0 + k + u);
        }
    }
}

template <int CW, int NW, int COUT, int S, bool ADD, bool W8 = false>
void launch_strip(const Strip8Args& a, hipStream_t s) {
    constexpr int SPB = ADD ? 8 / NW : (NW == 1 ? 4 : 1);
    constexpr int QL = CW / 16, NT = COUT / NW / 16;
    constexpr size_t smem = (ADD ? 65536 : 0) + (size_t)NW * (4 * QL * 16 + 4 * NT * 16) * 4 + (NW > 1 ? NW * 4 * QL * 12 * 4 + 2 * SPB * NW * 64 * 8 : 0);
    const long per_chunk = (long)(W8 ? 1 : a.OW / 16) * ((a.OH + a.TH - 1) / a.TH);
    const long blocks = NW == 1 ? (a.B * per_chunk + SPB - 1) / SPB : ((a.B + SPB - 1) / SPB) * per_chunk;
    auto kern = i8_strip_kernel<CW, NW, COUT, S, ADD, W8>;
    if (smem > 65536) (void)ensure_dynamic_lds(reinterpret_cast<const void*>(kern), smem);
    hipLaunchKernelGGL(kern, dim3((unsigned)blocks), dim3(64 * NW * SPB), smem, s, a);
}

constexpr int kF_STA = 0, kF_STB = 64, kF_STC = 80, kF_DWW = 128, kF_DWB = 176, kF_DWC = 192, kF_PWA = 240, kF_PWB = 368, kF_PWC = 400;

__global__ __launch_bounds__(256) void i8_front_strip_kernel(FrontStrip8Args a) {
    const int tid = threadIdx.x;
    const int lane = tid & 63;
    const int wave = __builtin_amdgcn_readfirstlane(tid >> 6);
    const int n = lane & 15, kq = lane >> 4;
    const int strips_x = a.OW >> 4;
    const int rblocks = (a.OH + a.TH - 1) / a.TH;
    int wid = xcd_tile(blockIdx.x, gridDim.x) * 4 + wave;
    if (wid >= a.B * strips_x * rblocks) return;
    const int sx = wid % strips_x;
    wid /= strips_x;
    const int ry = wid % rblocks;
    const int chunk = wid / rblocks;
    const int oh0 = ry * a.TH;
    const int nrows = (a.OH - oh0) < a.TH ? (a.OH - oh0) : a.TH;
    const int ow = sx * 16 + n;

    const v4i* c4 = reinterpret_cast<const v4i*>(a.cst);
    const long sta = (long)(uint32_t)a.cst[kF_STA + lane];
    const v4i stb = c4[kF_STB / 4 + kq];
    const v4i stm = c4[kF_STC / 4 + kq * 3 + 0], stc1 = c4[kF_STC / 4 + kq * 3 + 1], ste = c4[kF_STC / 4 + kq * 3 + 2];
    const long stc[4] = {rq64(stc1.x), rq64(stc1.y), rq64(stc1.z), rq64(stc1.w)};
    const int ste1 = pack_shifts(ste - 1);
    int stlo[4], sthi[4];
#pragma unroll
    for (int e = 0; e < 4; ++e) shifted_bounds(a.st_lo, a.st_hi, ste[e] - 1, stlo[e], sthi[e]);
    int dww[3][4];
#pragma unroll
    for (int i = 0; i < 3; ++i) {
        const v4i v = c4[kF_DWW / 4 + kq * 3 + i];
        dww[i][0] = v.x; dww[i][1] = v.y; dww[i][2] = v.z; dww[i][3] = v.w;
    }
    const v4i dwb = c4[kF_DWB / 4 + kq];
    __shared__ v4i cq_lds[4][4][3][5];
    auto stage_quad = [&](v4i* q, v4i m, v4i c1, v4i sh, int lo, int hi) {
        int blo[4], bhi[4];
        long c[4];
#pragma unroll
        for (int e = 0; e < 4; ++e) {
            c[e] = rq64(c1[e]);
            shifted_bounds(lo, hi, sh[e] - 1, blo[e], bhi[e]);
        }
        if (n == 0) {
            q[0] = m;
            q[1] = (v4i){(int)c[0], (int)(c[0] >> 32), (int)c[1], (int)(c[1] >> 32)};
            q[2] = (v4i){(int)c[2], (int)(c[2] >> 32), (int)c[3], (int)(c[3] >> 32)};
            q[3] = (v4i){blo[0], blo[1], blo[2], blo[3]};
            q[4] = (v4i){bhi[0], bhi[1], bhi[2], bhi[3]};
        }
        return pack_shifts(sh - 1);
    };
    const int dwe1 = stage_quad(cq_lds[wave][kq][0], c4[kF_DWC / 4 + kq * 3 + 0], c4[kF_DWC / 4 + kq * 3 + 1], c4[kF_DWC / 4 + kq * 3 + 2], a.dw_lo, a.dw_hi);
    long pwa[2];
    v4i pwb[2];
    int pwe1[2];
#pragma unroll
    for (int t = 0; t < 2; ++t) {
        pwa[t] = (long)(uint32_t)a.cst[kF_PWA + t * 64 + lane];
        pwb[t] = c4[kF_PWB / 4 + kq * 2 + t];
        const v4i* pc = c4 + kF_PWC / 4 + (kq * 2 + t) * 3;
        pwe1[t] = stage_quad(cq_lds[wave][kq][1 + t], pc[0], pc[1], pc[2], a.pw_lo, a.pw_hi);
    }
    const v4i* my_cq = cq_lds[wave][kq][0];

    const int zfe4 = (a.zp_fe & 0xff) * 0x01010101;
    const int zst4 = (a.zp_st & 0xff) * 0x01010101;
    const bool last_strip = sx == strips_x - 1;
    const int zstrow = (a.zp_st & 0xff) * 0x00010101;
    const int fe_bytes = a.H0 * a.W0;
    const __amdgpu_buffer_rsrc_t rs_fe =
        __builtin_amdgcn_make_buffer_rsrc(const_cast<int8_t*>(a.fe) + (size_t)chunk * fe_bytes, 0, fe_bytes, 0x00020000);
    const __amdgpu_buffer_rsrc_t rs_out =
        __builtin_amdgcn_make_buffer_rsrc(a.y + (size_t)chunk * a.OH * a.OW * 32, 0, a.OH * a.OW * 32, 0x00020000);
    const bool right_fe = 4 * ow + 4 >= a.W0;
    const bool right_st = 2 * ow + 2 >= a.W0 / 2;
    const int pad_st = right_st ? 0x00ff0000 : 0;
    const int voff_out = ow * 32 + 8 * kq;
    const int sr0 = 2 * oh0;
    const int rows_needed = 2 * (nrows - 1) + 3;

    constexpr int FD = 6;
    v2i raw[FD];
    TRow<1> T[3];

    auto fe_row = [&](int srel) { return sr0 + srel - 1 + kq; };
    const int fe_off0 = (sr0 - 1 + kq) * a.W0 + 4 * ow;
    auto issue = [&](int slot, int srel) {
        raw[slot] = __builtin_bit_cast(v2i, __builtin_amdgcn_raw_buffer_load_b64(rs_fe, fe_off0 + srel * a.W0, 0, 0));
    };
    auto stem_row = [&](int slot, int srel, int ti) {
        if (srel < rows_needed && sr0 + srel < a.H0) {
            const int fr = fe_row(srel);
            const bool ok = fr >= 0 && fr < a.H0;
            const int A = ok ? raw[slot].x : zfe4;
            const int Bd = (ok && !right_fe) ? raw[slot].y : zfe4;
            const int x[3] = {A & 0x00ffffff, perm(Bd, A, 0x0c040302u), Bd & 0x00ffffff};
#pragma unroll
            for (int j = 0; j < 3; ++j) {
                const v4i acc = __builtin_amdgcn_mfma_i32_16x16x32_i8(sta, (long)(uint32_t)x[j], stb, 0, 0, 0);
                int h[4];
#pragma unroll
                for (int e = 0; e < 4; ++e) h[e] = med3(rq_h(acc[e], stm[e], stc[e]), stlo[e], sthi[e]);
                deposit_column(T[ti].c[0], h, ste1, j);
            }
            if (last_strip) {
#pragma unroll
                for (int e = 0; e < 4; ++e) T[ti].c[0][e] = (T[ti].c[0][e] & ~pad_st) | (zst4 & pad_st);
            }
        } else {
#pragma unroll
            for (int e = 0; e < 4; ++e) T[ti].c[0][e] = zstrow;
        }
    };
    auto emit = [&](int i0, int i1, int i2, int oh) {
        asm volatile("" ::: "memory");
        struct Quad { v4i m; long c[4]; int lo[4], hi[4]; };
        auto quad = [&](int i) {
            const v4i m = my_cq[5 * i], c01 = my_cq[5 * i + 1], c23 = my_cq[5 * i + 2], lo = my_cq[5 * i + 3], hi = my_cq[5 * i + 4];
            return Quad{m, {__builtin_bit_cast(long, (v2i){c01.x, c01.y}), __builtin_bit_cast(long, (v2i){c01.z, c01.w}),
                            __builtin_bit_cast(long, (v2i){c23.x, c23.y}), __builtin_bit_cast(long, (v2i){c23.z, c23.w})},
                        {lo.x, lo.y, lo.z, lo.w}, {hi.x, hi.y, hi.z, hi.w}};
        };
        int h[4];
        const Quad dq = quad(0);
#pragma unroll
        for (int e = 0; e < 4; ++e) {
            int acc = dot4_first(T[i0].c[0][e], dww[0][e], dwb[e]);
            acc = dot4(T[i1].c[0][e], dww[1][e], acc);
            acc = dot4(T[i2].c[0][e], dww[2][e], acc);
            h[e] = rq_h(acc, dq.m[e], dq.c[e]);
        }
        const long bf = (long)(uint32_t)clamp_deposit_quad(h, dq.lo, dq.hi, dwe1);
        int ov[2][4];
#pragma unroll
        for (int t = 0; t < 2; ++t) {
            const v4i acc = __builtin_amdgcn_mfma_i32_16x16x32_i8(pwa[t], bf, pwb[t], 0, 0, 0);
            const Quad pq = quad(1 + t);
#pragma unroll
            for (int e = 0; e < 4; ++e) ov[t][e] = med3(rq_h(acc[e], pq.m[e], pq.c[e]), pq.lo[e], pq.hi[e]);
        }
        int outw[2];
        deposit_two_quads(outw[0], outw[1], ov[0], ov[1], pwe1[0], pwe1[1]);
        __builtin_amdgcn_raw_buffer_store_b64(__builtin_bit_cast(__attribute__((__vector_size__(2 * sizeof(int)))) int, (v2i){outw[0], outw[1]}), rs_out, voff_out, oh * a.OW * 32, 0);
    };

#pragma unroll
    for (int rr = 0; rr < FD; ++rr) issue(rr, rr);
    stem_row(0, 0, 0);
    issue(0, FD);
    for (int k = 0; k < nrows; k += 3) {
#pragma unroll
        for (int u = 0; u < 3; ++u) {
            if (k + u >= nrows) break;
#pragma unroll
            for (int s = 0; s < 2; ++s) {
                const int rs = 1 + 2 * u + s;
                stem_row(rs % FD, 2 * k + rs, rs % 3);
                issue(rs % FD, 2 * k + rs + FD);
            }
            emit((2 * u) % 3, (2 * u + 1) % 3, (2 * u + 2) % 3, oh0 + k + u);
        }
    }
}

struct DwStream8Args {
    const int8_t* x; int8_t* y;
    const int8_t* w; const int32_t* bias; const int32_t* mult; const int32_t* shift;
    int B, H, W, C, OH, OW, TH, pt, pl, zp_in, zp_out, amin, amax, CQ, rq_right;
    int32_t* pool;
};

struct RqHi {
    long long c[4];
    int sh[4];
};
__device__ __forceinline__ void rq_hi_setup(RqHi& r, const int (&shift)[4], int zp_out) {
#pragma unroll
    for (int e = 0; e < 4; ++e) {
        const int ex = -shift[e];
        r.c[e] = (1ll << 30) + (((1ll << (ex - 1)) + (long long)zp_out * (1ll << ex)) << 31);
        r.sh[e] = ex - 1;
    }
}

#ifdef BN_TAIL_STAMPS
__device__ long long* g_dw_stamps = nullptr;
__device__ int g_dw_sel[2] = {0, 0};
constexpr int kDwStampWaves = 4096;
#define BN_DSTAMP(i) do { if (dstamp) dst_[i] = (long long)__builtin_amdgcn_s_memrealtime(); } while (0)
#else
#define BN_DSTAMP(i) do {} while (0)
#endif

template <int S, bool HI>
__global__ __launch_bounds__(256) void i8_dw_stream_kernel(DwStream8Args a) {
#ifdef BN_TAIL_STAMPS
    long long dst_[4] = {0, 0, 0, 0};
    const long dslot = ((long)blockIdx.x - (long)gridDim.x / 2) * 4 + (threadIdx.x >> 6);
    const bool dstamp = g_dw_stamps && a.C == g_dw_sel[0] && a.H == g_dw_sel[1] && dslot >= 0 && dslot < kDwStampWaves;
#endif
    BN_DSTAMP(0);
    const int tid = threadIdx.x, lane = tid & 63;
    const int wave = __builtin_amdgcn_readfirstlane(tid >> 6);
    const int CQ = a.CQ, NCOL = 64 / CQ;
    const int cq = lane % CQ, n = lane / CQ;
    const int groups = a.C / (4 * CQ);
    const int strips_x = (a.OW + NCOL - 1) / NCOL;
    const int rblocks = (a.OH + a.TH - 1) / a.TH;
    long wid = (long)xcd_tile(blockIdx.x, gridDim.x) * 4 + wave;
    if (wid >= (long)a.B * groups * strips_x * rblocks) return;
    const int g = (int)(wid % groups);
    wid /= groups;
    const int sx = (int)(wid % strips_x);
    wid /= strips_x;
    const int ry = (int)(wid % rblocks);
    const int chunk = (int)(wid / rblocks);
    const int oh0 = ry * a.TH;
    const int nrows = (a.OH - oh0) < a.TH ? (a.OH - oh0) : a.TH;
    const int ow = sx * NCOL + n;
    const bool live = ow < a.OW;
    const int c0 = 4 * (g * CQ + cq);

    int wr[3][4], bias[4], mult[4], shift[4];
    RqHi rqh;
    auto load_constants = [&]() {
        int wq[9];
#pragma unroll
        for (int t = 0; t < 9; ++t) wq[t] = *reinterpret_cast<const int*>(a.w + t * a.C + c0);
        const v4i b4 = *reinterpret_cast<const v4i*>(a.bias + c0), m4 = *reinterpret_cast<const v4i*>(a.mult + c0), s4 = *reinterpret_cast<const v4i*>(a.shift + c0);
        int sum[4] = {0, 0, 0, 0};
#pragma unroll
        for (int i = 0; i < 3; ++i) {
            const int r0 = wq[3 * i], r1 = wq[3 * i + 1], r2 = wq[3 * i + 2];
            const int lo = perm(r1, r0, 0x05010400u), hi = perm(r1, r0, 0x07030602u);
            wr[i][0] = perm(r2, lo, 0x0c040100u);
            wr[i][1] = perm(r2, lo, 0x0c050302u);
            wr[i][2] = perm(r2, hi, 0x0c060100u);
            wr[i][3] = perm(r2, hi, 0x0c070302u);
#pragma unroll
            for (int e = 0; e < 4; ++e) sum[e] = dot4(wr[i][e], 0x00010101, sum[e]);
        }
#pragma unroll
        for (int e = 0; e < 4; ++e) {
            bias[e] = b4[e] - a.zp_in * sum[e];
            mult[e] = m4[e];
// ... 208 lines not shown
                const int rs = P + S * u + s2;
                consume(rs % D, S * k + rs, rs % 3);
                issue(rs % D, S * k + rs + D);
            }
            emit((S * u) % 3, (S * u + 1) % 3, (S * u + 2) % 3, oh0 + k + u);
        }
    }
}

}

int i8_strip_waves(int Cin, int Cout, int stride, int OW, bool add) {
    if (stride != 1 && stride != 2) return 0;
    if (OW == 8) {
        if (add) return (stride == 1 && Cin == 256 && Cout == 256) ? 8 : 0;
        return (stride == 2 && Cin == 128 && Cout == 256) ? 4 : 0;
    }
    if (OW % 16) return 0;
    if (add && (stride != 1 || Cin != Cout)) return 0;
    if (Cin == 64 && Cout == 64) return 2;
    if ((Cin == 32 || Cin == 64) && (Cout == 32 || Cout == 64)) return 1;
    if (add) return Cin == 128 ? 4 : 0;
    if (Cin == 64 && Cout == 128) return 2;
    if (Cin == 128 && Cout == 128) return 4;
    return 0;
}

bool i8_strip_supported(int Cin, int Cout, int stride, int OW, bool add) { return i8_strip_waves(Cin, Cout, stride, OW, add) != 0; }

void launch_i8_strip(Strip8Args a, int Cin, int Cout, int stride, hipStream_t s) {
    const bool add = a.add.enabled != 0;
    const int nw = i8_strip_waves(Cin, Cout, stride, a.OW, add);
    int th = a.OH;
    if (a.OW != 8) {
        while (th > 4 && (long)a.B * (a.OW / 16) * ((a.OH + th - 1) / th) * nw < 8192) th = (th + 1) / 2;
        if (const int v = g_opt.i8_strip_th; v >= 1) th = v < a.OH ? v : a.OH;
    }
    a.TH = th;
#define BN_STRIP(CW, NW, CO, ST, AD) \
    if (Cin == CW * NW && nw == NW && Cout == CO && stride == ST && add == AD) return launch_strip<CW, NW, CO, ST, AD>(a, s);
    if (Cin == 32 && nw == 1 && Cout == 32 && stride == 1 && add && g_opt.i8_strip_mfdw && a.pt == 1 && a.pl == 1 && a.OW % 16 == 0 && a.W == a.OW && a.H == a.OH) {
        const long per_chunk = (long)(a.OW / 16) * ((a.OH + a.TH - 1) / a.TH);
        const long blocks = (a.B * per_chunk + 7) / 8;
        const size_t smem = 65536 + (size_t)(4 * 2 * 16 + 4 * 2 * 16) * 4;
        (void)ensure_dynamic_lds(reinterpret_cast<const void*>(i8_strip_mf_kernel), smem);
        hipLaunchKernelGGL(i8_strip_mf_kernel, dim3((unsigned)blocks), dim3(512), smem, s, a);
        return;
    }
    BN_STRIP(32, 1, 32, 1, true)
    BN_STRIP(32, 4, 128, 1, true)
    BN_STRIP(32, 2, 64, 1, true)
    BN_STRIP(32, 2, 64, 1, false)
    BN_STRIP(32, 2, 64, 2, false)
    BN_STRIP(32, 1, 32, 1, false)
    BN_STRIP(32, 1, 64, 1, false)
    BN_STRIP(64, 1, 32, 1, false)
    BN_STRIP(32, 4, 128, 1, false)
    BN_STRIP(32, 2, 128, 1, false)
    BN_STRIP(32, 1, 32, 2, false)
    BN_STRIP(32, 1, 64, 2, false)
    BN_STRIP(64, 1, 32, 2, false)
    BN_STRIP(32, 4, 128, 2, false)
    BN_STRIP(32, 2, 128, 2, false)
#undef BN_STRIP
    if (a.OW == 8 && (a.OH & 1) == 0) {
        if (Cin == 128 && Cout == 256 && stride == 2 && !add) return launch_strip<32, 4, 256, 2, false, true>(a, s);
        if (Cin == 256 && Cout == 256 && stride == 1 && add) return launch_strip<32, 8, 256, 1, true, true>(a, s);
    }
}

bool i8_front_strip_supported(int H0, int W0, int C, int N, int OH, int OW) {
    return C == 16 && N == 32 && OW % 16 == 0 && H0 == 2 * OH && W0 == 4 * OW && W0 % 4 == 0;
}

void launch_i8_front_strip(FrontStrip8Args a, hipStream_t s) {
    int th = a.OH;
    while (th > 4 && (long)a.B * (a.OW / 16) * ((a.OH + th - 1) / th) < 8192) th = (th + 1) / 2;
    if (const int v = g_opt.i8_strip_th; v >= 1) th = v < a.OH ? v : a.OH;
    a.TH = th;
    const long waves = (long)a.B * (a.OW / 16) * ((a.OH + th - 1) / th);
    hipLaunchKernelGGL(i8_front_strip_kernel, dim3((unsigned)((waves + 3) / 4)), dim3(256), 0, s, a);
}

struct PwDw8Args {
    const int8_t* x; int8_t* y;
    const int8_t* pw_w; const int32_t* pw_b; const int32_t* pw_mult; const int32_t* pw_shift;
    const int8_t* dw_w; const int32_t* dw_b; const int32_t* dw_mult; const int32_t* dw_shift;
    int B, H, W, Cin, hid, OH, OW, pt, pl, RB;
    int h_zp, h_amin, h_amax;
    int o_zp, o_amin, o_amax;
};

template <int S, int KS>
__global__ __launch_bounds__(768) void i8_pwdw_kernel(PwDw8Args a) {
    extern __shared__ __attribute__((aligned(16))) int ring8[];
    const int tid = threadIdx.x, lane = tid & 63;
    const int wave = __builtin_amdgcn_readfirstlane(tid >> 6);
    const int r = lane & 15, q = lane >> 4;
    const int hq = a.hid >> 2;
    const int rowd = (a.W + 2) * hq;
    const int rblocks = (a.OH + a.RB - 1) / a.RB;
    const int wid = xcd_tile(blockIdx.x, gridDim.x);
    const int ry = wid % rblocks, chunk = wid / rblocks;
    const int oh0 = ry * a.RB;
    const int nrows = (a.OH - oh0) < a.RB ? (a.OH - oh0) : a.RB;
    const int h_lo = S * oh0 - a.pt;
    const int nhid = S * (nrows - 1) + 3;
    auto row_ok = [&](int k) { return k >= 0 && k < nhid && h_lo + k >= 0 && h_lo + k < a.H; };
    const int zp4 = (a.h_zp & 0xff) * 0x01010101, zprow = (a.h_zp & 0xff) * 0x00010101;

    v4i* dwt = reinterpret_cast<v4i*>(ring8 + 2 * rowd);
    v4i* pwt = dwt + 6 * hq;
    for (int quad = tid; quad < hq; quad += 768) {
        const int c0 = 4 * quad;
        v4i wrow[3], bb;
#pragma unroll
        for (int e = 0; e < 4; ++e) {
            int sum = 0;
#pragma unroll
            for (int ii = 0; ii < 3; ++ii) {
                const int k0 = a.dw_w[(ii * 3 + 0) * a.hid + c0 + e], k1 = a.dw_w[(ii * 3 + 1) * a.hid + c0 + e], k2 = a.dw_w[(ii * 3 + 2) * a.hid + c0 + e];
                wrow[ii][e] = (k0 & 0xff) | ((k1 & 0xff) << 8) | ((k2 & 0xff) << 16);
                sum += k0 + k1 + k2;
            }
            bb[e] = a.dw_b[c0 + e] - a.h_zp * sum;
        }
        dwt[6 * quad + 0] = wrow[0]; dwt[6 * quad + 1] = wrow[1]; dwt[6 * quad + 2] = wrow[2]; dwt[6 * quad + 3] = bb;
        dwt[6 * quad + 4] = *reinterpret_cast<const v4i*>(a.dw_mult + c0);
        dwt[6 * quad + 5] = *reinterpret_cast<const v4i*>(a.dw_shift + c0);
        pwt[3 * quad + 0] = *reinterpret_cast<const v4i*>(a.pw_b + c0);
        pwt[3 * quad + 1] = *reinterpret_cast<const v4i*>(a.pw_mult + c0);
        pwt[3 * quad + 2] = *reinterpret_cast<const v4i*>(a.pw_shift + c0);
    }
    for (int i = tid; i < 4 * hq; i += 768) {
        const int slot = i / (2 * hq), rest = i - slot * 2 * hq;
        ring8[slot * rowd + (rest < hq ? 0 : (a.W + 1) * hq) + (rest % hq)] = zp4;
    }

    const int npt = a.W >> 4, nct = a.hid >> 4, ntiles = npt * nct;
    v4i af[2][KS];
    int pos_t[2], dst_t[2], cq_t[2];
    bool live_t[2];
#pragma unroll
    for (int u = 0; u < 2; ++u) {
        const int t = 2 * wave + u;
        live_t[u] = t < ntiles;
        const int ptile = live_t[u] ? t % npt : 0, ct = live_t[u] ? t / npt : 0;
#pragma unroll
        for (int ks = 0; ks < KS; ++ks) af[u][ks] = reinterpret_cast<const v4i*>(a.pw_w)[((size_t)ks * nct + ct) * 64 + lane];
        cq_t[u] = 4 * ct + q;
        pos_t[u] = 16 * ptile + r;
        dst_t[u] = (pos_t[u] + 1) * hq + 4 * ct + q;
    }
    const int row_bytes = a.W * a.Cin;
    const __amdgpu_buffer_rsrc_t rs_in =
        __builtin_amdgcn_make_buffer_rsrc(const_cast<int8_t*>(a.x) + (size_t)chunk * a.H * row_bytes, 0, a.H * row_bytes, 0x00020000);
    auto request = [&](v4i (&bf)[2][KS], int k) {
        if (!row_ok(k)) return;
        const int soff = (h_lo + k) * row_bytes;
#pragma unroll
        for (int u = 0; u < 2; ++u)
#pragma unroll
            for (int ks = 0; ks < KS; ++ks) {
                const int koff = 64 * ks + 16 * q;
                bf[u][ks] = (v4i){0, 0, 0, 0};
                if (live_t[u] && koff < a.Cin) bf[u][ks] = __builtin_bit_cast(v4i, __builtin_amdgcn_raw_buffer_load_b128(rs_in, pos_t[u] * a.Cin + koff, soff, 0));
// ... 183 lines not shown
```

### birdnet-stm32_amd/csrc/bn_kernels.h

```cpp
#pragma once
#include <hip/hip_runtime.h>
#include <stdint.h>

#include <map>
#include <mutex>
#include <string>
#include <utility>
#include <vector>

#include "bn_blob.h"
#include "bn_chain_plan.h"

namespace bn {

struct Options {
    int f32_strip = 1;
    int f32_strip_th = 0;
    int f32_front_staged = 1;
    int i8_pwdw = 0;
    int f32_pw_ws = 1;
    int f32_tile_slice = 0;
    int f32_pwdw = 2;
    int f32_front2 = 1;
    int front_tpw = 0;
    int wave_dwpw = 1;
    int i8_strip = 1;
    int i8_strip_th = 0;
    int i8_dw_pool = 1;
    int i8_pw_lds = 1;
    int i8_pw_forms = 1;
    int i8_add_tab = 1;
    int i8_tail_fclds = 1;
    int i8_tail = 1;
    int i8_mid = 1;
    int i8_tail_mfdw = 1;
    int i8_mel_generic = 0;
    int stft_rowmajor = 0;
    int i8_mid_split = 1;
    int i8_strip_mfdw = 1;
    int stft_exact = 2;
    int stft_guard = 0;
    int stft_audit = 0;
    int stft_minint = 1;
    int stft_flagcap = 1022;
    int ingest_blk = 0;
    int ingest_generic = 0;
};
extern thread_local Options g_opt;

inline bool ensure_dynamic_lds(const void* kernel, size_t bytes) {
    static std::mutex mu;
    static std::map<std::pair<const void*, int>, size_t> allowed;
    int dev = 0;
    if (hipGetDevice(&dev) != hipSuccess) return false;
    std::lock_guard<std::mutex> lock(mu);
    size_t& have = allowed[{kernel, dev}];
    if (bytes <= have) return true;
    if (hipFuncSetAttribute(kernel, hipFuncAttributeMaxDynamicSharedMemorySize, (int)bytes) != hipSuccess) {
        (void)hipGetLastError();
        return false;
    }
    have = bytes;
    return true;
}

bool check_plan(const BlobHeader& h, const std::vector<SlotRec>& slots, const std::vector<TensorRec>& tensors,
                const std::vector<OpRec>& ops, std::string& err);

__device__ __forceinline__ int xcd_tile(int b, int nb) {
    const int nb8 = nb & ~7;
    return b < nb8 ? (b & 7) * (nb8 >> 3) + (b >> 3) : b;
}

struct StftTables {
    const float* window;
    const float4* tw256;
    const float4* tw512;
    const double* hann64;
    const double* cs64;
    const double2* cs2;
};

constexpr int kGuardCand = 62;
constexpr int kRecIds = 4, kRecExtra = kRecIds + 2 * kGuardCand, kRecVals = kRecExtra + 4;
constexpr int kGuardRec = kRecVals + 2 * kGuardCand;
constexpr int kGuardBudget = 48;
constexpr int kGuardMaxBudget = 1024;
struct StftGuard {
    float* eps;
    int* rec;
    float* mn_lo;
    int* count;
    int cap;
    int* dirty;
    int* work;
    int* n_work;
    int* hard;
    int* n_hard;
    int hard_cap;
    const float* audio;
    int T, hop;
    StftTables tabs;
    float k_l2, k_peak;
    int* audit;
    float audit_scale;
    float slack_scale;
    int min_interval;
    int flag_cap;
};

void launch_minmax_init(float* minmax, int B, hipStream_t s);
void launch_stft512(const StftTables& tb, const float* audio, int B, int T, int hop, int W, float* spec,
                    float* minmax, hipStream_t s, bool tile_major = false, const StftGuard* guard = nullptr);
void launch_stft512_f64(const StftTables& tb, const float* audio, int B, int T, int hop, int W, float* spec, float* minmax, hipStream_t s,
                        bool tile_major = false);
void launch_spec_bytes(const float* spec, const float* minmax, int B, int W, bool tile_major, float qscale, int qzp, int8_t* out, hipStream_t s);
void launch_stft_minmax_exact(const StftTables& tb, const float* audio, int B, int T, int hop, int W, float* spec, bool tile_major,
                              const StftGuard& g, float* minmax, hipStream_t s);
void launch_stft_fix(const StftTables& tb, const float* audio, int B, int T, int hop, int W, float* spec, bool tile_major, const StftGuard& g,
                     const float* minmax, float qscale, int qzp, hipStream_t s);
bool launch_stft512_mel(const StftTables& tb, const float* audio, int B, int T, int hop, int W, float* mel_out, int M,
                        const float* wvals, const int* bands, float* minmax, hipStream_t s, int square = 0);
// ... 108 lines not shown
                           const int32_t* shift, hipStream_t s);
struct I8AddParams {
    int enabled, z1, m1, s1, m2, s2, mo, so, zo, amin, amax;
};
void launch_i8_pw(const int8_t* x, const int8_t* res, int8_t* y, int B, int P, int Cin, int Cout, int zp_out, int amin,
                  int amax, const I8AddParams& add, const int8_t* w, const int32_t* bias, const int32_t* mult,
                  const int32_t* shift, hipStream_t s);
void launch_i8_mean(const int8_t* x, int8_t* y, int B, int P, int C, int zp_in, int mult, int shift, int zp_out,
                    hipStream_t s);
void launch_i8_fc(const int8_t* x, int8_t* y, int B, int Cin, int Cout, int zp_out, int amin, int amax, const int8_t* w,
                  const int32_t* bias, const int32_t* mult, const int32_t* shift, const int8_t* lut, hipStream_t s);
void launch_i8_segate(const int8_t* x, int8_t* y, int B, int P, int C, int zp_in, int mean_mult, int mean_shift, int mean_zp, int R, int zo1, int amin1,
                      int amax1, const int8_t* w1, const int32_t* b1, const int32_t* m1, const int32_t* s1, const int8_t* lut1, int zo2, int amin2,
                      int amax2, const int8_t* w2, const int32_t* b2, const int32_t* m2, const int32_t* s2, const int8_t* lut2, hipStream_t s, int32_t* sums = nullptr);
void launch_i8_scale(const int8_t* x, const int8_t* gate, int8_t* y, int B, int P, int C, int zx, int zg, int mult, int shift, int zo,
                     int amin, int amax, hipStream_t s);
void launch_i8_rawfe(const float* x, int8_t* y, int B, int T, int W, int M, int stride, int pad_left, float q_scale, int q_zp, int zp_out, int amin,
                     int amax, const int8_t* w, const int32_t* bias, const int32_t* mult, const int32_t* shift, const int8_t* lut, hipStream_t s);
void launch_i8_maxnorm(const int8_t* x, int8_t* y, int B, int C, int W, const int8_t* den_tab, const int8_t* div_tab, const int8_t* lut, hipStream_t s);
bool launch_i8_attnpool(const int8_t* x, int8_t* y, int B, const int* p, const int8_t* w, const int32_t* table, hipStream_t s);
void launch_i8_head_softmax(const int8_t* x, float* scores, float* logits, int B, int C, int zp_fc, float s_fc, float beta, hipStream_t s);
void launch_i8_head(const int8_t* x, float* scores, float* logits, int B, int C, int zp_fc, int zp_out, float s_fc,
                    float s_out, const int8_t* lut, hipStream_t s);

void launch_debug_requant(const int32_t* x, const int32_t* mult, const int32_t* shift, int n, int mode, int zp, int32_t* out, hipStream_t s);

struct DwPw8Args {
    const int8_t* x;
    const int8_t* res;
    int8_t* y;
    const int8_t* dw_w;
    const int32_t* dw_b;
    const int32_t* dw_mult;
    const int32_t* dw_shift;
    const int8_t* pw_w;
    const int32_t* pw_b;
    const int32_t* pw_mult;
    const int32_t* pw_shift;
    const int8_t* lut;
    int B, H, W, Cin, Cout, sh, sw, pt, pl, OH, OW, TH, TW, NB, has_dw, transposed;
    int dw_zp_in, dw_zp_out, dw_amin, dw_amax, pw_zp_out, pw_amin, pw_amax;
    I8AddParams add;
    int rq_right;
    const float* qx;
    const float* qminmax;
    float qscale;
    int qzp, qfill, qF;
    int qtiled;
    int qmode;
    StftGuard qguard;
    const int8_t* gate;
    int g_zx, g_zg, g_mult, g_shift, g_zo, g_amin, g_amax;
    const int8_t* add_tab;
};
bool i8_dwpw_supported(int Cin, int Cout);
bool i8_pwdw_supported(const DwPw8Args& expand, const I8ConvGeom& dw);
bool launch_i8_pwdw(const DwPw8Args& expand, const I8ConvGeom& dw, const int8_t* dw_w, const int32_t* dw_b, const int32_t* dw_mult, const int32_t* dw_shift,
                    int8_t* y, hipStream_t s);
bool i8_pw_lds_supported(const DwPw8Args& a);
void launch_i8_pw_lds(const DwPw8Args& a, hipStream_t s);
bool i8_pw_wave_takes(const DwPw8Args& a);
bool i8_mel_mfma_supported(const DwPw8Args& a);
struct Strip8Args {
    const int8_t* x;
    int8_t* y;
    const int32_t* cst;
    int B, H, W, OH, OW, TH, pt, pl;
    int zp_in, dw_lo, dw_hi;
    int pw_lo, pw_hi, pw_zp_out;
    I8AddParams add;
    const int8_t* add_tab;
};
struct FrontStrip8Args {
    const int8_t* fe;
    int8_t* y;
    const int32_t* cst;
    int B, H0, W0, OH, OW, TH;
    int zp_fe, st_lo, st_hi, zp_st, dw_lo, dw_hi, pw_lo, pw_hi;
};
bool i8_front_strip_supported(int H0, int W0, int C, int N, int OH, int OW);
void launch_i8_front_strip(FrontStrip8Args a, hipStream_t s);
bool i8_strip_supported(int Cin, int Cout, int stride, int OW, bool add);
void launch_i8_strip(Strip8Args a, int Cin, int Cout, int stride, hipStream_t s);
struct EmbOut {
    void* emb;
    int f32, zp;
    float scale;
};
template <class Args>
struct WithEmb {
    Args a;
    EmbOut e;
};
bool launch_i8_tail(Tail8Args a, hipStream_t s, const EmbOut* emb = nullptr);

long tail2_giveups();
bool launch_i8_tail2(Tail2Args a, hipStream_t s, const EmbOut* emb = nullptr);
bool launch_i8_mid2(Tail2Args a, hipStream_t s);

struct I8FrontParams {
    const int8_t* stem_w; const int32_t* stem_b; const int32_t* stem_mult; const int32_t* stem_shift;
    const int8_t* dw_w; const int32_t* dw_b; const int32_t* dw_mult; const int32_t* dw_shift;
    const int8_t* pw_w; const int32_t* pw_b; const int32_t* pw_mult; const int32_t* pw_shift;
    int H0, W0, C, N, OH, OW;
    int stem_zp_in, stem_zp_out, stem_amin, stem_amax, dw_zp_out, dw_amin, dw_amax, pw_zp_out, pw_amin, pw_amax;
    int rq_right;
};
bool i8_front_supported(int H0, int W0, int C, int N, int OH, int OW);
void launch_i8_front(const I8FrontParams& q, const int8_t* fe, int8_t* y, int B, hipStream_t s);
void launch_i8_dwpw(const DwPw8Args& a, hipStream_t s);

void preload_f32(); void preload_f32_fused(); void preload_f32_pw(); void preload_f32_strip(); void preload_i8(); void preload_i8_fused();
void preload_i8_pw(); void preload_i8_strip(); void preload_i8_tail(); void preload_i8_tail2(); void preload_ingest(); void preload_melspec();
void preload_stft(); void preload_stft_exact(); void preload_sort(); void preload_probe(); void preload_probe_sweep(); void preload_activity(); void preload_search(); void preload_augment(); void preload_kmeans(); void preload_tsne(); void preload_bootstrap(); void preload_head_i8();

struct ProbeFwdArgs {
    const float* X;
    const float* Y;
    const int* idx;
    const float* W;
    const float* b;
    float* out;
    float* loss_part;
    long n;
    int D, C, softmax;
    uint32_t drop_thresh;
    float drop_scale;
    uint32_t seed, step;
    float g_scale;
    const float* row_weight;
    int loss_kind;
    float focal_gamma;
};
struct ProbeDwArgs {
    const float* X; const int* idx; const float* G;
    float* partial;
    float* ss_part;
    int B, D, C, E, rows_per_group;
    uint32_t drop_thresh; float drop_scale; uint32_t seed, step;
};
struct ProbeUpdateArgs {
    float* params; float* m; float* v; const float* grad;
    const float* ss_part; int n_ss;
    const float* loss_part; int n_loss; float loss_scale; float* step_loss;
    int E, optimizer;
    float lr, alpha, weight_decay, clip;
};
bool launch_probe_fwd(const ProbeFwdArgs& a, int mode, hipStream_t s);
void launch_probe_dw(const ProbeDwArgs& a, int row_groups, hipStream_t s);
void launch_probe_reduce(float* partial, int E, int groups, float* ss_part, hipStream_t s);
void launch_probe_update(const ProbeUpdateArgs& a, hipStream_t s);
void launch_probe_loss_sum(const float* part, long n, float scale, float* out, hipStream_t s);
struct ProbeQatArgs {
    float s_out, z_out;
    int8_t* codes;
};
bool launch_probe_fwd_qat(const ProbeFwdArgs& a, const ProbeQatArgs& q, int mode, hipStream_t s);
void launch_probe_qat_weights(const float* P, float* Pq, float* amax, int D, int C, bool per_tensor, hipStream_t s);

struct ProbeSweepTrial {
    int optimizer;
    float weight_decay, clip;
    uint32_t drop_thresh;
    float drop_scale;
    int smooth;
    float smooth_keep, smooth_add;
// ... 119 lines not shown
```

### birdnet-stm32_amd/csrc/bn_ops.h

```cpp
#pragma once
#include "bn_blob.h"

#define BN_FIELDS_GEOM(c, p5) H, W, c, sh, sw, p5, OH, OW, pt, pl
#define BN_FIELDS_ADD has_add, add_z1, add_m1, add_s1, add_m2, add_s2, add_mo, add_so, add_zo, add_amin, add_amax

namespace bn {
namespace op {

namespace f32_mel {
enum Pi { F, W, M, mag, norm, P_END };
enum Ti { wvals, bands, magp, T_END };
}
namespace f32_mag {
enum Pi { M, W, mag, P_END };
enum Ti { rsv0, rsv1, magp, T_END };
}
namespace f32_rawfe {
enum Pi { T, W, M, stride, pad_left, mag, P_END };
enum Ti { fb, bias, magp, T_END };
}
namespace f32_stem {
enum Pi { BN_FIELDS_GEOM(Cout, act), P_END };
enum Ti { w, bias, T_END };
}
// ... 54 lines not shown
namespace i8_stem {
enum Pi { BN_FIELDS_GEOM(Cout, rsv5), zp_in, zp_out, act_min, act_max, P_END };
enum Ti { w, bias, mult, shift, T_END };
}
namespace i8_dw {
enum Pi { BN_FIELDS_GEOM(C, rsv5), zp_in, zp_out, act_min, act_max, P_END };
enum Ti { w, bias, mult, shift, T_END };
}
namespace i8_pw {
enum Pi { P, Cin, Cout, zp_out, act_min, act_max, BN_FIELDS_ADD, P_END };
enum Ti { w, bias, mult, shift, T_END };
}
namespace i8_mean {
enum Pi { P, C, zp_in, mult, shift, zp_out, P_END };
}
namespace i8_fc {
enum Pi { Cin, Cout, zp_out, act_min, act_max, has_lut, P_END };
enum Ti { w, bias, mult, shift, lut, T_END };
}
namespace i8_head {
enum Pi { C, zp_fc, zp_out, has_lut, softmax, P_END };
enum Ti { lut, T_END };
enum Fi { s_fc, s_out, beta, F_END };
}
namespace i8_dwpw {
enum Pi { BN_FIELDS_GEOM(Cin, qF), dw_zp_in, dw_zp_out, dw_amin, dw_amax, Cout, pw_zp_out, pw_amin, pw_amax, BN_FIELDS_ADD, has_dw, transposed, TH, TW, NB, has_lut, strip, q_at_load, qzp, qfill, P_END };
enum Ti { dw_w, dw_b, dw_mult, dw_shift, pw_w, pw_b, pw_mult, pw_shift, lut, strip_cst, add_tab, T_END };
enum Fi { qscale, F_END };
}
namespace i8_front {
enum Pi { H0, W0, C, N, OH, OW, stem_zp_in, stem_zp_out, stem_amin, stem_amax, dw_zp_out, dw_amin, dw_amax, pw_zp_out, pw_amin, pw_amax, strip, P_END };
enum Ti { stem_w, stem_b, stem_mult, stem_shift, dw_w, dw_b, dw_mult, dw_shift, pw_w, pw_b, pw_mult, pw_shift, strip_cst, T_END };
}
namespace i8_tail {
enum Pi { in_bytes, pw_macs, dw_macs, other_macs, n_classes, n_layers, H0, W0, C0, P_last, C_last, P_END };
enum Ti { cst, desc, cst2, desc2, T_END };
enum Fi { s_fc, s_head, F_END };
}
namespace i8_scale {
enum Pi { P, C, zp_x, zp_gate, mult, shift, zp_out, act_min, act_max, P_END };
}
namespace i8_maxnorm {
enum Pi { C, W, has_lut, P_END };
enum Ti { denom, div, lut, T_END };
}
namespace i8_rawfe {
enum Pi { T, W, M, stride, pad_left, q_zp, zp_out, act_min, act_max, has_lut, P_END };
enum Ti { w, bias, mult, shift, lut, T_END };
enum Fi { q_scale, F_END };
}
namespace i8_attnpool {
enum Pi { P, C, fc_bias, fc_mult, fc_shift, fc_zo, form, zx, za, mul_mult, mul_shift, mul_zo, mul_lo, mul_hi, sum_mult, sum_shift, sum_zo, P_END };
enum Ti { score, tables, T_END };
}
namespace i8_mid {
enum Pi { in_bytes, pw_macs, dw_macs, rsv3, rsv4, n_layers, H0, W0, C0, P_last, C_last, P_END };
enum Ti { cst, desc, T_END };
}

static_assert(f32_mel::P_END <= BN_OP_TAIL_TAG, "f32_mel: fields run into the cross-kind entries");
static_assert(f32_mag::P_END <= BN_OP_TAIL_TAG, "f32_mag: fields run into the cross-kind entries");
static_assert(f32_rawfe::P_END <= BN_OP_TAIL_TAG, "f32_rawfe: fields run into the cross-kind entries");
static_assert(f32_stem::P_END <= BN_OP_TAIL_TAG, "f32_stem: fields run into the cross-kind entries");
static_assert(f32_dw::P_END <= BN_OP_TAIL_TAG, "f32_dw: fields run into the cross-kind entries");
static_assert(f32_pw::P_END <= BN_OP_TAIL_TAG, "f32_pw: fields run into the cross-kind entries");
static_assert(f32_segate::P_END <= BN_OP_TAIL_TAG, "f32_segate: fields run into the cross-kind entries");
static_assert(f32_scale::P_END <= BN_OP_TAIL_TAG, "f32_scale: fields run into the cross-kind entries");
static_assert(f32_gap::P_END <= BN_OP_EMB_ZP, "f32_gap: fields run into the cross-kind entries");
static_assert(f32_dense::P_END <= BN_OP_TAIL_TAG, "f32_dense: fields run into the cross-kind entries");
static_assert(f32_attnpool::P_END <= BN_OP_EMB_ZP, "f32_attnpool: fields run into the cross-kind entries");
static_assert(f32_dwpw::P_END <= BN_OP_TAIL_TAG, "f32_dwpw: fields run into the cross-kind entries");
static_assert(f32_stftmel::P_END <= BN_OP_TAIL_TAG, "f32_stftmel: fields run into the cross-kind entries");
static_assert(f32_melfin::P_END <= BN_OP_TAIL_TAG, "f32_melfin: fields run into the cross-kind entries");
static_assert(f32_front::P_END <= BN_OP_FRONT2_DIST, "f32_front: fields run into the cross-kind entries");
static_assert(f32_gapdense::P_END <= BN_OP_EMB_ZP, "f32_gapdense: fields run into the cross-kind entries");
static_assert(i8_quant::P_END <= BN_OP_TAIL_TAG, "i8_quant: fields run into the cross-kind entries");
static_assert(i8_mel::P_END <= BN_OP_TAIL_TAG, "i8_mel: fields run into the cross-kind entries");
static_assert(i8_stem::P_END <= BN_OP_TAIL_TAG, "i8_stem: fields run into the cross-kind entries");
static_assert(i8_dw::P_END <= BN_OP_TAIL_TAG, "i8_dw: fields run into the cross-kind entries");
static_assert(i8_pw::P_END <= BN_OP_TAIL_TAG, "i8_pw: fields run into the cross-kind entries");
static_assert(i8_mean::P_END <= BN_OP_EMB_ZP, "i8_mean: fields run into the cross-kind entries");
static_assert(i8_fc::P_END <= BN_OP_TAIL_TAG, "i8_fc: fields run into the cross-kind entries");
static_assert(i8_head::P_END <= BN_OP_TAIL_TAG, "i8_head: fields run into the cross-kind entries");
static_assert(i8_front::P_END <= BN_OP_TAIL_TAG, "i8_front: fields run into the cross-kind entries");
static_assert(i8_tail::P_END <= BN_OP_EMB_ZP && (int)i8_tail::F_END <= BN_OP_EMB_SCALE, "i8_tail: fields run into the cross-kind entries");
static_assert(i8_scale::P_END <= BN_OP_TAIL_TAG, "i8_scale: fields run into the cross-kind entries");
static_assert(i8_maxnorm::P_END <= BN_OP_TAIL_TAG, "i8_maxnorm: fields run into the cross-kind entries");
static_assert(i8_rawfe::P_END <= BN_OP_TAIL_TAG, "i8_rawfe: fields run into the cross-kind entries");
static_assert(i8_attnpool::P_END <= BN_OP_EMB_ZP, "i8_attnpool: fields run into the cross-kind entries");
static_assert(i8_mid::P_END <= BN_OP_TAIL_TAG, "i8_mid: fields run into the cross-kind entries");
static_assert(i8_dwpw::has_lut == BN_OP_EMB_ZP && i8_dwpw::strip == BN_OP_EMB_DIM && i8_dwpw::q_at_load == BN_OP_EMB_TAG &&
                  i8_dwpw::qzp == BN_OP_FRONT2_DIST && i8_dwpw::qfill == BN_OP_TAIL_TAG && i8_dwpw::P_END == BN_OP_PATH,
              "i8_dwpw: the stated overlap with the cross-kind entries");
static_assert(i8_attnpool::P == 0 && i8_attnpool::sum_zo == 16 && i8_attnpool::P_END == 17, "i8_attnpool: launch_i8_attnpool reads p[0..16] in this order");
static_assert((int)i8_stem::P_END == i8_dw::P_END && (int)f32_stem::P_END == f32_dw::P_END && (int)i8_tail::C_last - i8_tail::n_layers == i8_mid::C_last - i8_mid::n_layers, "kinds decoded by one function share their layout");

}
}
```

### birdnet-stm32_amd/csrc/bn_plan_run.hip

```cpp
#include <algorithm>
#include <cstring>

#include "bn_model.h"
#include "bn_quant_in.h"

namespace bn {

namespace {

inline bool same_path(const OpRec& head, const OpRec& partner) {
    return partner.p[BN_OP_PATH] == BN_PATH_BOTH || partner.p[BN_OP_PATH] == head.p[BN_OP_PATH];
}
inline bool on_path(const OpRec& o, int mode) { return o.p[BN_OP_PATH] == BN_PATH_BOTH || o.p[BN_OP_PATH] == mode; }
inline int tag(const OpRec& o) { return o.p[BN_OP_TAIL_TAG]; }

bool gate_pools_dw(const OpRec& d, const OpRec& g) {
    namespace k = op::f32_dw;
    namespace q = op::f32_segate;
    return g.kind == BN_OP_F32_SEGATE && g.in0 == d.out && g.p[q::C] == d.p[k::C] && g.p[q::P] == d.p[k::OH] * d.p[k::OW];
}
int pwdw_row_blocks(const OpRec& d) {
    const int OH = d.p[op::f32_dw::OH], rb = f32_pwdw_rows(OH);
    return (OH + rb - 1) / rb;
}
// ... 185 lines not shown
    const bool tail_on, mid_on;

    size_t gap_for = (size_t)-1;
    int gap_R = 0, cand_R = 0;
    size_t cand_for = (size_t)-1;
    size_t pwdw_head_done = (size_t)-1;
    size_t pwdw_done = (size_t)-1;
    size_t front2_done = (size_t)-1;
    size_t segate_done[2] = {(size_t)-1, (size_t)-1};
    size_t pool8_for = (size_t)-1;
    size_t scale_done = (size_t)-1;
    int emb_written = 0;

    size_t oi = 0;
    const OpRec* o = nullptr;
    const int* p = nullptr;
    char *in0 = nullptr, *in1 = nullptr, *out = nullptr;
    const float* mm = nullptr;
    ProfScope* prof = nullptr;

    PlanRun(bn_model* m_, const RunArgs& a_)
        : m(m_), a(a_), B(a_.B), s(a_.s), mode(a_.d_audio ? BN_PATH_AUDIO : BN_PATH_INPUT), n(m_->ops.size()), tail_on(m_->has_tail && g_opt.i8_tail),
          mid_on(m_->has_mid && g_opt.i8_mid && g_opt.i8_strip) {}

    char* slot_ptr(int id) const {
        if (id == BN_SLOT_INPUT) return (char*)a.d_input;
        if (id == BN_SLOT_AUDIO) return (char*)a.d_audio;
        if (id == BN_SLOT_SCORES) return (char*)a.d_scores;
        if (id == BN_SLOT_LOGITS) return (char*)a.d_logits;
        if (id < 0 || id >= (int)m->d_slots.size()) return nullptr;
        return m->d_slots[id] + a.slot_b0 * m->slots[id].bytes_per_chunk;
    }
    const float* tf(const OpRec& r, int k) const { return (const float*)m->tensor(r.t[k]); }
    const int8_t* t8(const OpRec& r, int k) const { return (const int8_t*)m->tensor(r.t[k]); }
    const int32_t* t32(const OpRec& r, int k) const { return (const int32_t*)m->tensor(r.t[k]); }
    void* emb_for(const OpRec& r) const { return (a.d_emb && r.p[BN_OP_EMB_TAG] == BN_EMB_OP) ? a.d_emb : nullptr; }

    bool prep_ok() const { return m->prep[oi] && m->prep[oi]->ok; }

    void mark_slot(int sid, int v) {
        if (sid >= 0 && (size_t)sid < m->slot_valid.size()) m->slot_valid[sid] = (uint8_t)v;
    }
    void fused_into(size_t partner) {
        m->out_valid[oi] = 0;
        mark_slot(o->out, 0);
        m->out_valid[partner] = 1;
        mark_slot(m->ops[partner].out, 1);
    }

    DwPwArgs dwpw_args(const OpRec& d) const {
        namespace k = op::f32_dwpw;
        DwPwArgs r{};
        const int* q = d.p;
        r.x = (const float*)slot_ptr(d.in0);
        r.res = q[k::has_res] ? (const float*)slot_ptr(d.in1) : nullptr;
        r.gate = q[k::has_gate] ? (const float*)slot_ptr(q[k::gate_slot]) : nullptr;
        r.y = (float*)slot_ptr(d.out);
        r.dw_w = tf(d, k::dw_w); r.dw_b = tf(d, k::dw_b); r.pw_w = tf(d, k::pw_w); r.pw_b = tf(d, k::pw_b);
        r.B = B; r.H = q[k::H]; r.W = q[k::W]; r.Cin = q[k::Cin]; r.sh = q[k::sh]; r.sw = q[k::sw]; r.dw_act = q[k::dw_act];
        r.OH = q[k::OH]; r.OW = q[k::OW]; r.pt = q[k::pt]; r.pl = q[k::pl]; r.Cout = q[k::Cout]; r.pw_act = q[k::pw_act];
        r.has_dw = q[k::has_dw]; r.TH = q[k::TH]; r.TW = q[k::TW]; r.NB = q[k::NB];
        return r;
    }
    DwPw8Args dwpw8_args(const OpRec& d, size_t di) const {
        namespace k = op::i8_dwpw;
        DwPw8Args r{};
        const int* q = d.p;
        r.x = (const int8_t*)slot_ptr(d.in0);
        r.res = q[k::has_add] ? (const int8_t*)slot_ptr(d.in1) : nullptr;
        r.y = (int8_t*)slot_ptr(d.out);
        r.dw_w = t8(d, k::dw_w); r.dw_b = t32(d, k::dw_b); r.dw_mult = t32(d, k::dw_mult); r.dw_shift = t32(d, k::dw_shift);
        r.pw_w = t8(d, k::pw_w); r.pw_b = t32(d, k::pw_b); r.pw_mult = t32(d, k::pw_mult); r.pw_shift = t32(d, k::pw_shift);
        r.lut = q[k::has_lut] ? t8(d, k::lut) : nullptr;
        r.B = B; r.H = q[k::H]; r.W = q[k::W]; r.Cin = q[k::Cin]; r.sh = q[k::sh]; r.sw = q[k::sw]; r.OH = q[k::OH]; r.OW = q[k::OW];
        r.pt = q[k::pt]; r.pl = q[k::pl]; r.dw_zp_in = q[k::dw_zp_in]; r.dw_zp_out = q[k::dw_zp_out]; r.dw_amin = q[k::dw_amin]; r.dw_amax = q[k::dw_amax];
        r.Cout = q[k::Cout]; r.pw_zp_out = q[k::pw_zp_out]; r.pw_amin = q[k::pw_amin]; r.pw_amax = q[k::pw_amax];
        r.add = add_params(q, k::has_add);
        r.has_dw = q[k::has_dw]; r.transposed = q[k::transposed]; r.TH = q[k::TH]; r.TW = q[k::TW]; r.NB = q[k::NB];
        r.rq_right = m->prep[di]->rq_right;
        r.add_tab = (q[k::has_add] && !q[k::has_dw] && d.t[k::add_tab] >= 0) ? t8(d, k::add_tab) : nullptr;
        return r;
    }

    float* gap_target(size_t di) {
        const OpRec& d = m->ops[di];
        cand_for = (size_t)-1;
        if (g_opt.f32_pwdw < 2 || !m->d_gap_part || di + 1 >= n) return nullptr;
        const OpRec& g = m->ops[di + 1];
        const int R = pwdw_row_blocks(d);
        if (!gate_pools_dw(d, g) || (size_t)R * d.p[op::f32_dw::C] > m->gap_part_elems || !on_path(g, mode)) return nullptr;
        cand_for = di + 1;
        cand_R = R;
        return m->d_gap_part;
    }
    void take_gap() {
        gap_for = cand_for;
        gap_R = cand_R;
    }
    bool launch_pwdw(const DwPwArgs& ea, size_t di, const F32StemIn* st) {
        namespace k = op::f32_dw;
        const OpRec& d = m->ops[di];
        const int* q = d.p;
        return f32_pwdw_supported(ea, q[k::H], q[k::W], q[k::C], q[k::sh], q[k::sw], q[k::OH], q[k::OW]) &&
               launch_f32_pwdw(ea, tf(d, k::w), tf(d, k::bias), (float*)slot_ptr(d.out), q[k::sh], q[k::OH], q[k::OW], q[k::pt], q[k::pl], q[k::act], st,
                               gap_target(di), s);
    }

    bool segate_fused(size_t mi) const {
        namespace k = op::i8_mean;
        namespace f = op::i8_fc;
        if (mi + 2 >= n) return false;
        const OpRec& r = m->ops[mi];
        const OpRec& f1 = m->ops[mi + 1];
        const OpRec& f2 = m->ops[mi + 2];
        const int C = r.p[k::C];
        return r.kind == BN_OP_I8_MEAN && tag(r) == BN_SEGATE_HEAD && g_opt.i8_strip && same_path(r, f1) && same_path(r, f2) && f1.kind == BN_OP_I8_FC &&
               f2.kind == BN_OP_I8_FC && tag(f1) == BN_SEGATE_COVERED && tag(f2) == BN_SEGATE_COVERED && f1.in0 == r.out && f2.in0 == f1.out &&
               f1.p[f::Cin] == C && f2.p[f::Cin] == f1.p[f::Cout] && f2.p[f::Cout] == C && C % 4 == 0 && f2.out != r.in0;
    }

    int f32_stem() {
        namespace k = op::f32_stem;
        if (tag(*o) == BN_PWDW_STEM && g_opt.f32_pwdw && g_opt.f32_strip && oi + 2 < n) {
            namespace e_ = op::f32_dwpw;
            const OpRec& e = m->ops[oi + 1];
            const OpRec& d = m->ops[oi + 2];
            if (same_path(*o, e) && same_path(*o, d) && e.kind == BN_OP_F32_DWPW && tag(e) == BN_PWDW_HEAD && d.kind == BN_OP_F32_DW && tag(d) == BN_PWDW_COVERED &&
                e.in0 == o->out && d.in0 == e.out && d.out != o->in0 && d.out != o->out && d.out != e.out && e.p[e_::H] == p[k::OH] && e.p[e_::W] == p[k::OW] &&
                e.p[e_::Cin] == p[k::Cout]) {
                const DwPwArgs ea = dwpw_args(e);
                const F32StemIn st{(const float*)in0, tf(*o, k::w), tf(*o, k::bias), p[k::H], p[k::W], p[k::sh], p[k::sw], p[k::pt], p[k::pl], p[k::act]};
                if (ea.Cin <= 32 && launch_pwdw(ea, oi + 2, &st)) {
                    pwdw_head_done = oi + 1;
                    pwdw_done = oi + 2;
                    fused_into(oi + 2);
                    take_gap();
                    return BN_OK;
                }
            }
        }
        launch_f32_stem((const float*)in0, (float*)out, B, p[k::H], p[k::W], p[k::Cout], p[k::sh], p[k::sw], p[k::act], p[k::OH], p[k::OW], p[k::pt], p[k::pl],
                        tf(*o, k::w), tf(*o, k::bias), s);
        return BN_OK;
    }

    int f32_dw() {
        namespace k = op::f32_dw;
        float* gp = nullptr;
        int R = 0;
        if (g_opt.f32_pwdw >= 2 && m->d_gap_part && oi + 1 < n) {
            const OpRec& g = m->ops[oi + 1];
            R = f32_dw_stream_strips(B, p[k::C], p[k::OH], p[k::OW]);
            if (gate_pools_dw(*o, g) && (size_t)R * p[k::C] <= m->gap_part_elems && on_path(g, mode)) gp = m->d_gap_part;
        }
        if (launch_f32_dw((const float*)in0, (float*)out, B, p[k::H], p[k::W], p[k::C], p[k::sh], p[k::sw], p[k::act], p[k::OH], p[k::OW], p[k::pt], p[k::pl],
                          tf(*o, k::w), tf(*o, k::bias), gp, s) && gp) {
            gap_for = oi + 1;
            gap_R = R;
        }
        return BN_OK;
    }

    int f32_dwpw() {
        const DwPwArgs r = dwpw_args(*o);
        if (tag(*o) == BN_PWDW_HEAD && g_opt.f32_pwdw && g_opt.f32_strip && oi + 1 < n) {
            const OpRec& d = m->ops[oi + 1];
// ... 18 lines not shown
        const float* minmax = p[k::raw_mel] ? m->d_minmax : nullptr;
        const int dist = p[BN_OP_FRONT2_DIST];
        if (tag(*o) == BN_FRONT2_HEAD && g_opt.f32_front2 && g_opt.f32_strip && g_opt.f32_front_staged && dist > 0 && oi + (size_t)dist < n) {
            const OpRec& d = m->ops[oi + (size_t)dist];
            if (same_path(*o, d) && d.kind == BN_OP_F32_DWPW && tag(d) == BN_FRONT2_COVERED && d.in0 == o->out && d.out != o->in0) {
                const F32FrontStripArgs f{(const float*)in0, nullptr, tf(*o, k::stem_w), tf(*o, k::stem_b), tf(*o, k::dw_w), tf(*o, k::dw_b), tf(*o, k::pw_w),
                                          tf(*o, k::pw_b), minmax, tf(*o, k::wsum), tf(*o, k::magp), B, p[k::H0], p[k::W0], p[k::OH], p[k::OW], 0,
                                          p[k::stem_act], p[k::dw_act], p[k::pw_act], p[k::mag]};
                const DwPwArgs da = dwpw_args(d);
                if (p[k::C] == 16 && p[k::N] == 32 && f32_front2_supported(f, da) && launch_f32_front2(f, da, s)) {
                    front2_done = oi + (size_t)dist;
                    fused_into(front2_done);
                    return BN_OK;
                }
            }
        }
        launch_f32_front((const float*)in0, (float*)out, B, p[k::H0], p[k::W0], p[k::C], p[k::N], p[k::OH], p[k::OW], p[k::stem_act], p[k::dw_act], p[k::pw_act],
                         tf(*o, k::stem_w), tf(*o, k::stem_b), tf(*o, k::dw_w), tf(*o, k::dw_b), tf(*o, k::pw_w), tf(*o, k::pw_b), minmax, tf(*o, k::wsum),
                         tf(*o, k::magp), p[k::mag], s);
        return BN_OK;
    }

    int i8_conv() {
        namespace k = op::i8_dw;
        I8ConvGeom g = conv_geom8(*o);
        g.rq_right = m->prep[oi]->rq_right;
        const int8_t* w = t8(*o, k::w);
        const int32_t *bias = t32(*o, k::bias), *mult = t32(*o, k::mult), *shift = t32(*o, k::shift);
        if (o->kind == BN_OP_I8_DW) {
            int32_t* pool = nullptr;
            if (g_opt.i8_dw_pool && m->d_pool8 && oi + 1 < n && segate_fused(oi + 1)) {
                const OpRec& mo = m->ops[oi + 1];
                if (same_path(*o, mo) && mean_pools_dw8(*o, mo) && mo.p[op::i8_mean::P] == p[k::OH] * p[k::OW] && (size_t)p[k::C] <= m->pool8_C) pool = m->d_pool8;
            }
            if (launch_i8_dw_stream((const int8_t*)in0, (int8_t*)out, B, g, w, bias, mult, shift, s, pool)) {
                if (pool) pool8_for = oi + 1;
                return BN_OK;
            }
        }
        if (o->kind == BN_OP_I8_STEM && launch_i8_stem_stream((const int8_t*)in0, (int8_t*)out, B, g, w, bias, mult, shift, s)) return BN_OK;
        auto fn = o->kind == BN_OP_I8_STEM ? launch_i8_stem : launch_i8_dw;
        fn((const int8_t*)in0, (int8_t*)out, B, g, w, bias, mult, shift, s);
        return BN_OK;
    }

    int i8_dwpw() {
        namespace k = op::i8_dwpw;
        DwPw8Args r = dwpw8_args(*o, oi);
        if (tag(*o) == BN_PWDW8_HEAD && g_opt.i8_pwdw && g_opt.i8_strip && oi + 1 < n) {
            namespace dk = op::i8_dw;
            const OpRec& d = m->ops[oi + 1];
            if (same_path(*o, d) && d.kind == BN_OP_I8_DW && tag(d) == BN_PWDW8_COVERED && d.in0 == o->out && d.out != o->in0 && d.out != o->out) {
                const I8ConvGeom g = conv_geom8(d);
                if (i8_pwdw_supported(r, g) &&
                    launch_i8_pwdw(r, g, t8(d, dk::w), t32(d, dk::bias), t32(d, dk::mult), t32(d, dk::shift), (int8_t*)slot_ptr(d.out), s)) {
                    pwdw_done = oi + 1;
                    fused_into(oi + 1);
                    return BN_OK;
                }
            }
        }
        if (r.transposed && p[k::q_at_load]) {
            r.qx = (const float*)in0;
            r.qminmax = mm;
            r.qscale = o->f[k::qscale];
            r.qzp = p[k::qzp];
            r.qfill = p[k::qfill];
            r.qF = p[k::qF];
            r.qtiled = (a.spec.tiled && o->in0 == BN_SLOT_INPUT) ? 1 : 0;
            r.x = nullptr;
            if (!i8_mel_mfma_supported(r)) return fail(BN_ERR_FORMAT, "operator %zu: fused QUANTIZE needs the mel-mixer kernel's geometry", oi);
            if (a.spec.guard && r.qtiled && mm) {
                r.qguard = guard_slice(m, a.slot_b0, a.spec);
                r.qmode = 1;
                launch_i8_dwpw(r, s);
                prof->end();
                ProfScope fix(m, (int)n + 2, s);
                launch_stft_fix(m->ctx->tables, a.spec.audio, B, a.spec.T, a.spec.hop, r.W, (float*)in0, true, r.qguard, mm, r.qscale, r.qzp, s);
                r.qmode = 2;
                launch_i8_dwpw(r, s);
                return BN_OK;
            }
        }
        if (p[k::strip] && o->t[k::strip_cst] >= 0 && g_opt.i8_strip && r.has_dw && !r.transposed && r.sh == r.sw &&
            i8_strip_supported(r.Cin, r.Cout, r.sh, r.OW, r.add.enabled != 0) && (!r.add.enabled || (r.res == r.x && o->t[k::add_tab] >= 0))) {
            const int off = r.add.enabled ? 128 : 0;
            Strip8Args q{r.x, r.y, t32(*o, k::strip_cst), B, r.H, r.W, r.OH, r.OW, 0, r.pt, r.pl, r.dw_zp_in, r.dw_amin, r.dw_amax, r.pw_amin + off,
                         r.pw_amax + off, r.pw_zp_out, r.add, r.add.enabled ? t8(*o, k::add_tab) : nullptr};
            launch_i8_strip(q, r.Cin, r.Cout, r.sh, s);
            return BN_OK;
        }
        if (!i8_dwpw_supported(r.Cin, r.Cout) || r.TH * r.TW * r.NB != 64 || r.OH % r.TH || r.OW % r.TW)
            return fail(BN_ERR_FORMAT, "operator %zu: unsupported fused INT8 block geometry", oi);
        launch_i8_dwpw(r, s);
        return BN_OK;
    }

    int i8_front() {
        namespace k = op::i8_front;
        I8FrontParams q{};
        q.stem_w = t8(*o, k::stem_w); q.stem_b = t32(*o, k::stem_b); q.stem_mult = t32(*o, k::stem_mult); q.stem_shift = t32(*o, k::stem_shift);
        q.dw_w = t8(*o, k::dw_w); q.dw_b = t32(*o, k::dw_b); q.dw_mult = t32(*o, k::dw_mult); q.dw_shift = t32(*o, k::dw_shift);
        q.pw_w = t8(*o, k::pw_w); q.pw_b = t32(*o, k::pw_b); q.pw_mult = t32(*o, k::pw_mult); q.pw_shift = t32(*o, k::pw_shift);
        q.H0 = p[k::H0]; q.W0 = p[k::W0]; q.C = p[k::C]; q.N = p[k::N]; q.OH = p[k::OH]; q.OW = p[k::OW];
        q.stem_zp_in = p[k::stem_zp_in]; q.stem_zp_out = p[k::stem_zp_out]; q.stem_amin = p[k::stem_amin]; q.stem_amax = p[k::stem_amax];
        q.dw_zp_out = p[k::dw_zp_out]; q.dw_amin = p[k::dw_amin]; q.dw_amax = p[k::dw_amax];
        q.pw_zp_out = p[k::pw_zp_out]; q.pw_amin = p[k::pw_amin]; q.pw_amax = p[k::pw_amax];
        q.rq_right = m->prep[oi]->rq_right;
        if (p[k::strip] && o->t[k::strip_cst] >= 0 && g_opt.i8_strip && i8_front_strip_supported(q.H0, q.W0, q.C, q.N, q.OH, q.OW)) {
            FrontStrip8Args fa{(const int8_t*)in0, (int8_t*)out, t32(*o, k::strip_cst), B, q.H0, q.W0, q.OH, q.OW, 0, q.stem_zp_in, q.stem_amin, q.stem_amax,
                               q.stem_zp_out, q.dw_amin, q.dw_amax, q.pw_amin, q.pw_amax};
            launch_i8_front_strip(fa, s);
            return BN_OK;
        }
        if (!i8_front_supported(q.H0, q.W0, q.C, q.N, q.OH, q.OW)) return fail(BN_ERR_FORMAT, "operator %zu: unsupported INT8 front-block geometry", oi);
        launch_i8_front(q, (const int8_t*)in0, (int8_t*)out, B, s);
        return BN_OK;
    }

    int i8_mid() {
        const OpPrep& pr = *m->prep[oi];
        Tail2Args ma = g_opt.i8_mid_split && pr.alt_ok ? pr.resident : pr.chain;
        ma.x = (const int8_t*)in0;
        ma.y = (int8_t*)out;
        ma.cst = t32(*o, op::i8_mid::cst);
        ma.B = B;
        if (!launch_i8_mid2(ma, s)) return fail(BN_ERR_DEVICE, "could not raise the LDS limit of the fused stage-2 kernel");
        return BN_OK;
    }

    int i8_tail() {
        namespace k = op::i8_tail;
        const OpPrep& pr = *m->prep[oi];
        const EmbOut eo{a.d_emb, a.emb_dtype == BN_EMB_F32, p[BN_OP_EMB_ZP], o->f[BN_OP_EMB_SCALE]};
        const EmbOut* emb = emb_for(*o) ? &eo : nullptr;
        emb_written += emb != nullptr;
        bool launched;
        if (g_opt.i8_tail_mfdw && pr.alt_ok) {
            Tail2Args t2 = pr.chain;
            t2.x = (const int8_t*)in0;
            t2.scores = a.d_scores;
            t2.logits = a.d_logits;
            t2.cst = t32(*o, k::cst2);
            t2.B = B;
            launched = launch_i8_tail2(t2, s, emb);
        } else {
            Tail8Args ta = pr.tail;
            ta.x = (const int8_t*)in0;
            ta.scores = a.d_scores;
            ta.logits = a.d_logits;
            ta.cst = t32(*o, k::cst);
            ta.B = B;
            launched = launch_i8_tail(ta, s, emb);
        }
        if (!launched) return fail(BN_ERR_DEVICE, "could not raise the LDS limit of the fused tail kernel");
        return BN_OK;
    }

    int i8_mean() {
        namespace k = op::i8_mean;
        namespace f = op::i8_fc;
        if (segate_fused(oi)) {
            const OpRec& f1 = m->ops[oi + 1];
            const OpRec& f2 = m->ops[oi + 2];
            launch_i8_segate((const int8_t*)in0, (int8_t*)slot_ptr(f2.out), B, p[k::P], p[k::C], p[k::zp_in], p[k::mult], p[k::shift], p[k::zp_out],
                             f1.p[f::Cout], f1.p[f::zp_out], f1.p[f::act_min], f1.p[f::act_max], t8(f1, f::w), t32(f1, f::bias), t32(f1, f::mult), t32(f1, f::shift),
                             f1.p[f::has_lut] ? t8(f1, f::lut) : nullptr, f2.p[f::zp_out], f2.p[f::act_min], f2.p[f::act_max], t8(f2, f::w), t32(f2, f::bias),
                             t32(f2, f::mult), t32(f2, f::shift), f2.p[f::has_lut] ? t8(f2, f::lut) : nullptr, s, oi == pool8_for ? m->d_pool8 : nullptr);
            segate_done[0] = oi + 1;
            segate_done[1] = oi + 2;
            fused_into(oi + 2);
            return BN_OK;
        }
        launch_i8_mean((const int8_t*)in0, (int8_t*)out, B, p[k::P], p[k::C], p[k::zp_in], p[k::mult], p[k::shift], p[k::zp_out], s);
        return BN_OK;
    }

    int i8_scale() {
        namespace k = op::i8_scale;
        if (tag(*o) == BN_SCALE_HEAD && g_opt.i8_strip && oi + 1 < n) {
            namespace dk = op::i8_dwpw;
            const OpRec& d = m->ops[oi + 1];
            if (same_path(*o, d) && d.kind == BN_OP_I8_DWPW && tag(d) == BN_SCALE_COVERED && d.in0 == o->out && d.out != o->in0 && d.out != o->in1 &&
                d.p[dk::Cin] == p[k::C] && d.p[dk::OH] * d.p[dk::OW] == p[k::P]) {
                DwPw8Args a2 = dwpw8_args(d, oi + 1);
                a2.x = (const int8_t*)in0;
                a2.gate = (const int8_t*)in1;
                a2.g_zx = p[k::zp_x]; a2.g_zg = p[k::zp_gate]; a2.g_mult = p[k::mult]; a2.g_shift = p[k::shift]; a2.g_zo = p[k::zp_out];
                a2.g_amin = p[k::act_min]; a2.g_amax = p[k::act_max];
                if (!a2.has_dw && !a2.transposed && i8_pw_wave_takes(a2)) {
                    launch_i8_dwpw(a2, s);
                    scale_done = oi + 1;
                    fused_into(oi + 1);
                    return BN_OK;
// ... 189 lines not shown
```

### include/birdnet_hip.h

```cpp
#ifndef BIRDNET_HIP_H
#define BIRDNET_HIP_H

#include <stddef.h>
#include <stdint.h>

#ifdef __cplusplus
extern "C" {
#endif

#define BN_ABI_VERSION 2

#if defined(__GNUC__)
#define BN_API __attribute__((visibility("default")))
#else
#define BN_API
#endif

#define BN_OK 0
#define BN_ERR_ARG (-1)
#define BN_ERR_DEVICE (-2)
#define BN_ERR_FORMAT (-3)
#define BN_ERR_UNSUPPORTED (-4)
#define BN_ERR_NOMEM (-5)

// ... 33 lines not shown
BN_API void bn_model_free(bn_model* model);
BN_API int bn_model_get_info(const bn_model* model, bn_model_info* out);

BN_API int bn_stft_mag(bn_ctx* ctx, const float* d_audio, int B, int T, int n_fft, int hop, int W,
                int normalize, float* d_spec, float* d_minmax, void* stream);

BN_API int bn_stft_mag_exact(bn_ctx* ctx, const float* d_audio, int B, int T, int n_fft, int hop, int W,
                      int normalize, float* d_spec, float* d_minmax, void* stream);

BN_API int bn_forward(bn_model* model, const float* d_input, const float* d_minmax, int B,
               float* d_scores, float* d_logits, void* stream);

BN_API int bn_infer_audio(bn_model* model, const float* d_audio, int B, int T, int hop,
                   float* d_scores, float* d_logits, void* stream);

#define BN_EMB_F32 0
#define BN_EMB_I8 1

BN_API int bn_model_get_embedding_info(const bn_model* model, int* dim, int* dtype, float* scale, int* zero_point);

BN_API int bn_forward_embed(bn_model* model, const float* d_input, const float* d_minmax, int B, float* d_scores,
               float* d_logits, void* d_emb, int emb_dtype, void* stream);
BN_API int bn_infer_audio_embed(bn_model* model, const float* d_audio, int B, int T, int hop, float* d_scores,
               float* d_logits, void* d_emb, int emb_dtype, void* stream);


#define BN_PCM_S16 0
#define BN_PCM_S24 1
#define BN_PCM_S32 2
#define BN_PCM_F32 3

BN_API int bn_ingest_resample(bn_ctx* ctx, const void* d_pcm, int sample_format, int channels,
                       const int64_t* d_in_off, const int64_t* d_out_off, int n_windows, int64_t max_in_len,
                       int64_t max_out_len, const float* d_taps, int up, int down, int taps_per_phase,
                       int n_pre_remove, float* d_mono, float* d_peak, void* stream);

BN_API int bn_ingest_resample_span(bn_ctx* ctx, const void* d_pcm, int sample_format, int channels, int64_t s0, int64_t n_staged,
                       int64_t n_in, int64_t o0, int64_t o1, const float* d_taps, int up, int down, int taps_per_phase,
                       int n_pre_remove, float* d_mono_window, float* d_peak, void* stream);

BN_API int bn_ingest_chunks(bn_ctx* ctx, const float* d_mono, const float* d_peak, const int64_t* d_chunk_src,
                     const int32_t* d_chunk_valid, const int32_t* d_chunk_window, int n_chunks, int chunk_len,
                     float* d_chunks, void* stream);

BN_API int bn_short_time_energy(bn_ctx* ctx, const float* d_mono, const float* d_peak, const int64_t* d_win_off, const int32_t* d_win_index,
                         const int64_t* d_frame_off, int n_windows, int frame_len, int hop, float* d_ste, void* stream);

BN_API int bn_activity_counts(bn_ctx* ctx, const float* d_x, int B, int64_t n, const int32_t* d_idx, int m, float k, int32_t* d_active,
                       float* d_stats, void* stream);

BN_API int bn_rank_orders(bn_ctx* ctx, const float* d_scores, int n_rows, int n_classes, int32_t* d_cols, int32_t* d_flat, void* stream);

BN_API int bn_chunk_peak_normalize(bn_ctx* ctx, const float* d_x, int B, int T, float eps, float* d_y, void* stream);

#define BN_POOL_AVG 0
#define BN_POOL_MAX 1
#define BN_POOL_LME 2

BN_API int bn_pool_scores(bn_ctx* ctx, const float* d_scores, const int64_t* d_file_off, int n_files, int n_classes,
                   int method, float beta, float* d_pooled, void* stream);


#define BN_SPEC_MEL 0
#define BN_SPEC_LOGMEL 1
#define BN_SPEC_MFCC 2
#define BN_MAG_NONE 0
#define BN_MAG_PWL 1
#define BN_MAG_PCEN 2
#define BN_MAG_DB 3

BN_API int bn_mel_spectrogram(bn_ctx* ctx, const float* d_audio, int B, int T, int n_fft, int hop, int W,
                       const float* d_mel_w, const int32_t* d_mel_bands, int n_mels, int mode, int mag_scale,
                       double pcen_b, const float* d_dct, int n_mfcc, float* d_work, float* d_out, void* stream);

BN_API int bn_debug_op_output(bn_model* model, int op_index, int B, void* d_dst, size_t dst_bytes,
                       size_t* bytes_per_chunk, void* stream);

BN_API int bn_debug_input_bytes(bn_model* model, int B, int8_t* d_out, void* stream);
BN_API int bn_debug_guard_stats(bn_model* model, int B, int64_t* out);
BN_API int bn_debug_tail_form(const bn_model* model, int* form, int* lds_bytes);
BN_API int bn_debug_mid_form(const bn_model* model, int* form, int* lds_bytes);
BN_API int bn_debug_mid_plan(const bn_model* model, int* out, int n);
BN_API int bn_debug_mid_split_giveups(bn_ctx* ctx, int64_t* count);

BN_API int bn_debug_requant(bn_ctx* ctx, const int32_t* d_x, const int32_t* d_mult, const int32_t* d_shift, int n, int mode,
                     int zero_point, int32_t* d_out, void* stream);

BN_API int bn_profile_enable(bn_model* model, int enable);
BN_API int bn_profile_only(bn_model* model, int op_index);
BN_API int bn_profile_collect(bn_model* model, double* total_ms, int64_t* launches, int n);

BN_API int bn_set_option(const char* name, int value);
BN_API int bn_get_option(const char* name, int* value);
BN_API int bn_ctx_set_option(bn_ctx* ctx, const char* name, int value);
BN_API int bn_ctx_get_option(bn_ctx* ctx, const char* name, int* value);
BN_API int bn_ctx_reset_options(bn_ctx* ctx);

BN_API void* bn_host_alloc_pinned(bn_ctx* ctx, size_t bytes);
BN_API int bn_host_free_pinned(void* p);

#define BN_PROBE_MAX_D 2048
#define BN_PROBE_MAX_C 4096
#define BN_PROBE_ACT_SIGMOID 0
#define BN_PROBE_ACT_SOFTMAX 1
#define BN_PROBE_OPT_ADAM 0
#define BN_PROBE_OPT_ADAMW 1
#define BN_PROBE_OPT_SGD 2
#define BN_PROBE_WORKSPACE_BYTES (256u << 20)

typedef struct bn_probe bn_probe;

BN_API int bn_head_forward(bn_ctx* ctx, const float* d_emb, int64_t n, int D, const float* d_W, const float* d_b, int C, int activation,
                    float* d_scores, void* stream);

#define BN_HEAD_I8_STEP_ROWS 64
#define BN_HEAD_I8_MIN_WG_STEPS 8
#define BN_HEAD_I8_MAX_WGS 1024
#define BN_HEAD_I8_LDS_BYTES (160 * 1024)
BN_API int bn_head_i8_forward(bn_ctx* ctx, const int8_t* d_rows, int64_t n, int D, const int8_t* d_w, const int32_t* d_bias,
                       const int32_t* d_mult, const int32_t* d_shift, int C, int zp_out, const int8_t* d_lut, int activation, float s_fc,
                       int8_t* d_logit_bytes, float* d_scores, void* stream);

BN_API int bn_head_i8_pass_classes(int D, int C);

BN_API int bn_probe_create(bn_ctx* ctx, int D, int C, int activation, int optimizer, float lr, float weight_decay, float clipnorm,
                    float dropout, uint32_t seed, int64_t total_steps, const float* d_W, const float* d_b, bn_probe** out, void* stream);
BN_API void bn_probe_destroy(bn_probe* probe);
BN_API int bn_probe_epoch(bn_probe* probe, const float* d_X, const float* d_Y, const int32_t* d_perm, int64_t n, int batch,
                   float* d_step_loss, void* stream);
BN_API int bn_probe_loss(bn_probe* probe, const float* d_X, const float* d_Y, int64_t n, float* d_out, void* stream);
BN_API int bn_probe_get(bn_probe* probe, float* d_W, float* d_b, void* stream);
BN_API int bn_probe_set(bn_probe* probe, const float* d_W, const float* d_b, void* stream);
#define BN_PROBE_LOSS_CE 0
#define BN_PROBE_LOSS_FOCAL 1
BN_API int bn_probe_set_loss(bn_probe* probe, int loss, float focal_gamma);
BN_API int bn_probe_epoch_weighted(bn_probe* probe, const float* d_X, const float* d_Y, const float* d_row_weight, const int32_t* d_perm,
                            int64_t n, int batch, float* d_step_loss, void* stream);
#define BN_PROBE_QAT_OFF 0
#define BN_PROBE_QAT_PER_CLASS 1
#define BN_PROBE_QAT_PER_TENSOR 2
BN_API int bn_probe_set_qat(bn_probe* probe, int weight_mode, int quantize_logits, float s_out, int z_out);
BN_API int bn_probe_get_quantized(bn_probe* probe, float* d_Wq, void* stream);
BN_API int bn_probe_scores(bn_probe* probe, const float* d_X, int64_t n, float* d_scores, int8_t* d_codes, void* stream);

#define BN_PROBE_SWEEP_MAX_TRIALS 64
#define BN_PROBE_SWEEP_BYTES (2048ull << 20)
#define BN_PROBE_SWEEP_CURRENT 0
#define BN_PROBE_SWEEP_SNAPSHOT 1

typedef struct bn_probe_trial {
    int32_t optimizer;
    float lr;
    float weight_decay;
    float clipnorm;
    float dropout;
    float label_smoothing;
} bn_probe_trial;

typedef struct bn_probe_sweep bn_probe_sweep;

BN_API int bn_probe_sweep_create(bn_ctx* ctx, int D, int C, int activation, int T, const bn_probe_trial* trials, uint32_t seed,
                          int64_t total_steps, const float* d_W, const float* d_b, bn_probe_sweep** out, void* stream);
BN_API void bn_probe_sweep_destroy(bn_probe_sweep* sweep);
BN_API int bn_probe_sweep_epoch(bn_probe_sweep* sweep, const float* d_X, const float* d_Y, const int32_t* d_perm, int64_t n, int batch,
                         const float* d_step_sizes, const uint8_t* d_active, float* d_step_loss, void* stream);
BN_API int bn_probe_sweep_loss(bn_probe_sweep* sweep, const float* d_X, const float* d_Y, int64_t n, const uint8_t* d_active, float* d_out,
// ... 78 lines not shown
```

Baseline: 2.397 million.

## Fuse INT8 front strip and following DW-PW strip via LDS row ring

Adds a fused i8_front2 kernel that runs the front-strip block and the next 32->32 depthwise-pointwise residual strip in one 1024-thread workgroup. Producer waves write output rows into an LDS ring buffer and consumer waves spin on per-strip counters, so the intermediate activation no longer goes through global memory and one launch is removed. The planner tags eligible front/dwpw pairs and the runtime falls back to the old path when the geometry does not match. The cost is intra-workgroup spin synchronisation with a give-up counter, higher LDS use, and lower occupancy.

```diff
diff --git a/birdnet-stm32_amd/birdnet_stm32/_hip.py b/birdnet-stm32_amd/birdnet_stm32/_hip.py
--- a/birdnet-stm32_amd/birdnet_stm32/_hip.py
+++ b/birdnet-stm32_amd/birdnet_stm32/_hip.py
@@ -15,7 +15,7 @@
     "bn_model_free", "bn_model_get_info", "bn_stft_mag", "bn_forward", "bn_infer_audio", "bn_debug_op_output",
     "bn_kernel_names", "bn_profile_enable", "bn_profile_collect", "bn_ingest_resample", "bn_ingest_chunks",
     "bn_pool_scores", "bn_mel_spectrogram", "bn_profile_only", "bn_chunk_peak_normalize", "bn_set_option", "bn_get_option", "bn_ctx_set_option", "bn_ctx_get_option", "bn_ctx_reset_options", "bn_preload_kernels", "bn_host_alloc_pinned", "bn_host_free_pinned", "bn_rank_orders",
-    "bn_blob_check", "bn_debug_requant", "bn_stft_mag_exact", "bn_debug_input_bytes", "bn_debug_guard_stats", "bn_debug_tail_form", "bn_debug_mid_form", "bn_debug_mid_plan", "bn_debug_mid_split_giveups",
+    "bn_blob_check", "bn_debug_requant", "bn_stft_mag_exact", "bn_debug_input_bytes", "bn_debug_guard_stats", "bn_debug_tail_form", "bn_debug_mid_form", "bn_debug_mid_plan", "bn_debug_mid_split_giveups", "bn_debug_front2_giveups",
     "bn_forward_embed", "bn_infer_audio_embed", "bn_model_get_embedding_info", "bn_ingest_resample_span",
     "bn_head_forward", "bn_probe_create", "bn_probe_destroy", "bn_probe_epoch", "bn_probe_loss", "bn_probe_get", "bn_probe_set",
     "bn_probe_sweep_create", "bn_probe_sweep_destroy", "bn_probe_sweep_epoch", "bn_probe_sweep_loss", "bn_probe_sweep_snapshot", "bn_probe_sweep_get",
@@ -74,7 +74,7 @@
 
 OPTION_NAMES = ("f32_strip", "f32_strip_th", "f32_front_staged", "f32_front2", "f32_pwdw", "f32_tile_slice", "f32_pw_ws", "i8_pwdw", "i8_pw_lds", "i8_pw_forms", "i8_add_tab", "front_tpw", "wave_dwpw", "i8_strip", "i8_strip_mfdw", "i8_strip_th", "i8_dw_pool", "i8_tail_fclds", "i8_tail", "i8_tail_mfdw", "i8_mid",
                 "i8_mel_generic", "stft_rowmajor", "stft_exact", "stft_flagcap", "stft_guard", "stft_audit", "stft_minint", "ingest_blk", "ingest_generic")
-SCHEDULING_OPTION_NAMES = ("i8_mid_split",)
+SCHEDULING_OPTION_NAMES = ("i8_mid_split", "i8_front2")
 
 
 class BnModelInfo(ctypes.Structure):
@@ -126,6 +126,7 @@
     lib.bn_debug_mid_form.argtypes = [c_void_p, POINTER(c_int), POINTER(c_int)]
     lib.bn_debug_mid_plan.argtypes = [c_void_p, POINTER(c_int), c_int]
     lib.bn_debug_mid_split_giveups.argtypes = [c_void_p, POINTER(c_int64)]
+    lib.bn_debug_front2_giveups.argtypes = [c_void_p, POINTER(c_int64)]
     lib.bn_forward.argtypes = [c_void_p, c_void_p, c_void_p, c_int, c_void_p, c_void_p, c_void_p]
     lib.bn_infer_audio.argtypes = [c_void_p, c_void_p, c_int, c_int, c_int, c_void_p, c_void_p, c_void_p]
     lib.bn_forward_embed.argtypes = [c_void_p, c_void_p, c_void_p, c_int, c_void_p, c_void_p, c_void_p, c_int, c_void_p]
diff --git a/birdnet-stm32_amd/birdnet_stm32/models/_lower_i8.py b/birdnet-stm32_amd/birdnet_stm32/models/_lower_i8.py
--- a/birdnet-stm32_amd/birdnet_stm32/models/_lower_i8.py
+++ b/birdnet-stm32_amd/birdnet_stm32/models/_lower_i8.py
@@ -998,7 +998,30 @@
         _tag_scale_pairs(pb)
         _tag_se_gates(pb)
         _tag_pwdw_pairs(pb)
+        _tag_front2(pb)
     return pb.finalize(reuse=not keep_all)
+
+
+def _tag_front2(pb: pk.PlanBuilder) -> None:
+    ops = pb.plan.ops
+    for i, o in enumerate(ops):
+        if not (o.kind == pk.I8_DWPW and [o.get(k) for k in ("has_dw", "Cin", "Cout", "sh", "sw", "has_add", "strip", "transposed", "has_lut", "q_at_load")]
+                == [1, 32, 32, 1, 1, 1, 1, 0, 0, 0] and o.in0 == o.in1 and o.in0 >= 0 and not o.p[pk.TAIL_TAG]):
+            continue
+        v = o.in0
+        fronts = [j for j in range(i) if ops[j].kind == pk.I8_FRONT and ops[j].out == v]
+        readers = [k for k, r in enumerate(ops) if k != i and (r.in0 == v or r.in1 == v)]
+        writers = [k for k, r in enumerate(ops) if r.out == v]
+        if not fronts or readers or writers != fronts:
+            continue
+        if any((ops[j].get("C"), ops[j].get("N"), ops[j].get("OH"), ops[j].get("OW"), ops[j].get("strip")) != (16, 32, o.get("H"), o.get("W"), 1)
+               or o.get("W") != 64 or ops[j].p[pk.TAIL_TAG] or ops[j].p[pk.OP_PATH] != o.p[pk.OP_PATH] or i - j >= 8 for j in fronts):
+            continue
+        for j in fronts:
+            ops[j].p[pk.TAIL_TAG] = pk.FRONT2_HEAD
+            ops[j].p[pk.FRONT2_DIST] = i - j
+            if ops[j].in0 >= 0:
+                pb._extra_uses.append((i, ops[j].in0))
 
 
 def _mark_embedding(g: _Graph, plan: pk.Plan) -> None:
diff --git a/birdnet-stm32_amd/birdnet_stm32/models/runners.py b/birdnet-stm32_amd/birdnet_stm32/models/runners.py
--- a/birdnet-stm32_amd/birdnet_stm32/models/runners.py
+++ b/birdnet-stm32_amd/birdnet_stm32/models/runners.py
@@ -256,6 +256,11 @@
         _hip.check(self.lib.bn_debug_mid_split_giveups(self.ctx.handle, ctypes.byref(n)))
         return int(n.value)
 
+    def front2_giveups(self) -> int:
+        n = ctypes.c_int64(0)
+        _hip.check(self.lib.bn_debug_front2_giveups(self.ctx.handle, ctypes.byref(n)))
+        return int(n.value)
+
     def profile(self, enable: bool) -> None:
         _hip.check(self.lib.bn_profile_enable(self.model.handle, int(bool(enable))))
 
diff --git a/birdnet-stm32_amd/csrc/bn_api.hip b/birdnet-stm32_amd/csrc/bn_api.hip
--- a/birdnet-stm32_amd/csrc/bn_api.hip
+++ b/birdnet-stm32_amd/csrc/bn_api.hip
@@ -28,7 +28,7 @@
     {"wave_dwpw", &bn::Options::wave_dwpw},       {"i8_strip", &bn::Options::i8_strip},
     {"i8_strip_th", &bn::Options::i8_strip_th}, {"i8_dw_pool", &bn::Options::i8_dw_pool}, {"i8_tail_fclds", &bn::Options::i8_tail_fclds},   {"i8_tail", &bn::Options::i8_tail}, {"i8_tail_mfdw", &bn::Options::i8_tail_mfdw}, {"i8_mid", &bn::Options::i8_mid}, {"i8_mid_split", &bn::Options::i8_mid_split},
     {"i8_mel_generic", &bn::Options::i8_mel_generic}, {"stft_rowmajor", &bn::Options::stft_rowmajor},
-    {"i8_strip_mfdw", &bn::Options::i8_strip_mfdw}, {"stft_exact", &bn::Options::stft_exact}, {"stft_flagcap", &bn::Options::stft_flagcap}, {"stft_guard", &bn::Options::stft_guard}, {"stft_audit", &bn::Options::stft_audit}, {"stft_minint", &bn::Options::stft_minint},
+    {"i8_strip_mfdw", &bn::Options::i8_strip_mfdw}, {"i8_front2", &bn::Options::i8_front2}, {"stft_exact", &bn::Options::stft_exact}, {"stft_flagcap", &bn::Options::stft_flagcap}, {"stft_guard", &bn::Options::stft_guard}, {"stft_audit", &bn::Options::stft_audit}, {"stft_minint", &bn::Options::stft_minint},
     {"ingest_blk", &bn::Options::ingest_blk},
     {"ingest_generic", &bn::Options::ingest_generic},
 };
@@ -639,6 +639,15 @@
     return BN_OK;
 }
 
+int bn_debug_front2_giveups(bn_ctx* ctx, int64_t* count) {
+    if (!ctx || !count) return fail(BN_ERR_ARG, "null argument");
+    if (int rc = check_device(ctx)) return rc;
+    const long n = bn::front2_giveups();
+    if (n < 0) return fail(BN_ERR_DEVICE, "could not read the give-up counter of the front pair's ring");
+    *count = n;
+    return BN_OK;
+}
+
 int bn_debug_guard_stats(bn_model* m, int B, int64_t* out) {
     if (!m || !out) return fail(BN_ERR_ARG, "null argument");
     if (int rc = check_device(m->ctx)) return rc;
@@ -1025,7 +1034,7 @@
 const char* bn_kernel_names(void) {
     return "ingest_resample_kernel\ningest_decimate_kernel\ningest_peak_kernel\ningest_chunks_kernel\nchunk_peaknorm_kernel\npool_scores_kernel\nstft512_mag_kernel\nspec_normalize_kernel\nmelspec_finish_kernel\nf32_mel_kernel\nf32_melfin_kernel\nf32_mag_kernel\nf32_rawfe_kernel\nf32_stem_kernel\nf32_dw_kernel\n"
            "f32_pw_kernel\nf32_pw_ws_kernel\nf32_dwpw_kernel\nf32_dwpw_wave_kernel\nf32_strip_kernel\nf32_front_strip_kernel\nf32_front2_kernel\nf32_pwdw_kernel\nf32_dw_stream_kernel\nf32_front_kernel\nf32_gap_kernel\nf32_gap_dense_kernel\nf32_gap_dense_emb_kernel\nf32_dense_kernel\nf32_segate_kernel\nf32_scale_kernel\nf32_attnpool_kernel\n"
-           "i8_quant_kernel\ni8_mel_kernel\ni8_stem_kernel\ni8_dw_kernel\ni8_pw_kernel\ni8_dwpw_kernel\ni8_mel_mfma_kernel\ni8_strip_kernel\ni8_strip_mf_kernel\ni8_front_strip_kernel\ni8_front_kernel\ni8_tail_kernel\ni8_tail_emb_kernel\ni8_tail2_kernel\ni8_tail2_emb_kernel\ni8_mid2_kernel\ni8_mean_kernel\ni8_fc_kernel\ni8_scale_kernel\ni8_maxnorm_kernel\ni8_rawfe_kernel\ni8_pwdw_kernel\ni8_dw_stream_kernel\ni8_stem_stream_kernel\ni8_segate_kernel\ni8_pw_wave_kernel\ni8_pw_lds_kernel\ni8_attnpool_kernel\n"
+           "i8_quant_kernel\ni8_mel_kernel\ni8_stem_kernel\ni8_dw_kernel\ni8_pw_kernel\ni8_dwpw_kernel\ni8_mel_mfma_kernel\ni8_strip_kernel\ni8_strip_mf_kernel\ni8_front_strip_kernel\ni8_front2_kernel\ni8_front_kernel\ni8_tail_kernel\ni8_tail_emb_kernel\ni8_tail2_kernel\ni8_tail2_emb_kernel\ni8_mid2_kernel\ni8_mean_kernel\ni8_fc_kernel\ni8_scale_kernel\ni8_maxnorm_kernel\ni8_rawfe_kernel\ni8_pwdw_kernel\ni8_dw_stream_kernel\ni8_stem_stream_kernel\ni8_segate_kernel\ni8_pw_wave_kernel\ni8_pw_lds_kernel\ni8_attnpool_kernel\n"
            "i8_head_kernel\ni8_head_softmax_kernel\nemb_store_kernel\nprobe_fwd_kernel\nprobe_dw_kernel\nprobe_reduce_kernel\nprobe_update_kernel\nprobe_loss_sum_kernel\nprobe_sweep_snapshot_kernel\nste_kernel\nactivity_count_kernel\nsearch_inv_norms_kernel\nsearch_score_kernel\nsearch_merge_kernel\naugment_kernel\nkmeans_assign_kernel\nkmeans_keys_kernel\nkmeans_offsets_kernel\nkmeans_segments_kernel\nkmeans_partial_kernel\nkmeans_fold_kernel\nkmeans_scale_kernel\ntsne_perplexity_kernel\ntsne_repulsion_kernel\ntsne_fold_kernel\ntsne_z_kernel\ntsne_attraction_kernel\ntsne_update_kernel\nbootstrap_table_kernel\nbootstrap_reject_kernel\nbootstrap_prepare_kernel\nbootstrap_resample_kernel\nhead_i8_kernel";
 }
 
diff --git a/birdnet-stm32_amd/csrc/bn_front2_ring.h b/birdnet-stm32_amd/csrc/bn_front2_ring.h
--- /dev/null
+++ b/birdnet-stm32_amd/csrc/bn_front2_ring.h
@@ -0,0 +1,18 @@
+#pragma once
+
+namespace bn {
+namespace front2 {
+
+constexpr int kMinRing = 3;
+
+constexpr int ring_row(int row, int R) { return row % R; }
+
+constexpr int lo_strip(int sx) { return sx > 0 ? sx - 1 : 0; }
+constexpr int hi_strip(int sx, int strips) { return sx + 1 < strips ? sx + 1 : strips - 1; }
+
+constexpr int need_produced(int r, int H) { return r + 2 < H ? r + 2 : H; }
+
+constexpr int need_consumed(int p, int R) { return p < R ? 0 : p - R + 2; }
+
+}
+}
diff --git a/birdnet-stm32_amd/csrc/bn_i8_strip.hip b/birdnet-stm32_amd/csrc/bn_i8_strip.hip
--- a/birdnet-stm32_amd/csrc/bn_i8_strip.hip
+++ b/birdnet-stm32_amd/csrc/bn_i8_strip.hip
@@ -1,5 +1,6 @@
 #include <stdlib.h>
 
+#include "bn_front2_ring.h"
 #include "bn_kernels.h"
 #include "bn_requant.h"
 
@@ -337,50 +338,83 @@
     }
 }
 
-__global__ __launch_bounds__(512) __attribute__((amdgpu_waves_per_eu(4))) void i8_strip_mf_kernel(Strip8Args a) {
-    constexpr int CIN = 32, COUT = 32, QL = 2, NT = 2, NW = 1, SPB = 8, NTHREADS = 512;
+constexpr int kF2Pitch = 48, kF2Cols = 64, kF2RowBytes = kF2Cols * kF2Pitch;
+struct Front2Ring {
+    unsigned char* rows;
+    unsigned* produced;
+    unsigned* consumed;
+};
+__device__ unsigned g_front2_giveups = 0;
+
+__device__ __forceinline__ void ring_publish(unsigned* ctr) {
+    asm volatile("s_waitcnt lgkmcnt(0)" ::: "memory");
+    __builtin_amdgcn_fence(__ATOMIC_RELEASE, "workgroup", "local");
+    if ((threadIdx.x & 63) == 0) __hip_atomic_fetch_add(ctr, 1u, __ATOMIC_RELAXED, __HIP_MEMORY_SCOPE_WORKGROUP);
+}
+
+__device__ __forceinline__ void ring_wait(const unsigned* ctr, int sx, int strips, int need, int& seen, bool& gave_up) {
+    if (seen >= need || gave_up) return;
+    const unsigned *c0 = ctr + front2::lo_strip(sx), *c1 = ctr + sx, *c2 = ctr + front2::hi_strip(sx, strips);
+    bool done = false;
+#pragma unroll 1
+    for (int spins = 0; spins < (1 << 20); ++spins) {
+        const int v0 = (int)__hip_atomic_load(c0, __ATOMIC_RELAXED, __HIP_MEMORY_SCOPE_WORKGROUP);
+        const int v1 = (int)__hip_atomic_load(c1, __ATOMIC_RELAXED, __HIP_MEMORY_SCOPE_WORKGROUP);
+        const int v2 = (int)__hip_atomic_load(c2, __ATOMIC_RELAXED, __HIP_MEMORY_SCOPE_WORKGROUP);
+        const int v = __builtin_amdgcn_readfirstlane(min(v0, min(v1, v2)));
+        if (v >= need) {
+            seen = v;
+            done = true;
+            break;
+        }
+        __builtin_amdgcn_s_sleep(1);
+    }
+    if (!done) {
+        gave_up = true;
+        if ((threadIdx.x & 63) == 0) atomicAdd(&g_front2_giveups, 1u);
+    }
+    __builtin_amdgcn_fence(__ATOMIC_ACQUIRE, "workgroup", "local");
+}
+
+constexpr int kMfLdsBytes = 65536 + (4 * 2 * 16 + 4 * 2 * 16) * 4;
+
+template <int NTHREADS>
+__device__ __forceinline__ void strip_mf_stage(const Strip8Args& a, unsigned char* lds_all, int tid) {
+    constexpr int QL = 2, NT = 2, NW = 1;
     constexpr int nDWW = 4 * QL * 12, nDWB = 4 * QL * 4, nDWC = 4 * QL * 12, nPWA = NT * NW * 64 * QL, nPWB = 4 * NT * 4;
     constexpr int kDWW = 0, kDWB = kDWW + nDWW, kDWC = kDWB + nDWB, kPWA = kDWC + nDWC, kPWB = kPWA + nPWA, kPWC = kPWB + nPWB;
-    extern __shared__ __attribute__((aligned(16))) unsigned char lds_all[];
-    const unsigned char* add_tab = lds_all;
     v4i* c_dw = reinterpret_cast<v4i*>(lds_all + 65536);
     v4i* c_pw = c_dw + nDWC / 3;
-    const int tid = threadIdx.x;
-    {
-        const v4i* src = reinterpret_cast<const v4i*>(a.cst);
-        for (int i = tid; i < nDWC / 12; i += NTHREADS) {
-            const v4i m = src[kDWC / 4 + 3 * i], c1 = src[kDWC / 4 + 3 * i + 1], sh = src[kDWC / 4 + 3 * i + 2];
-            const long c[4] = {rq64(c1.x), rq64(c1.y), rq64(c1.z), rq64(c1.w)};
-            c_dw[4 * i] = m;
-            c_dw[4 * i + 1] = (v4i){(int)c[0], (int)(c[0] >> 32), (int)c[1], (int)(c[1] >> 32)};
-            c_dw[4 * i + 2] = (v4i){(int)c[2], (int)(c[2] >> 32), (int)c[3], (int)(c[3] >> 32)};
-            c_dw[4 * i + 3] = (v4i){pack_shifts(sh - 1), 0, 0, 0};
-        }
-        for (int i = tid; i < 4 * NT; i += NTHREADS) {
-            c_pw[4 * i] = src[kPWC / 4 + 3 * i];
-            c_pw[4 * i + 1] = src[kPWC / 4 + 3 * i + 1];
-            c_pw[4 * i + 2] = src[kPWC / 4 + 3 * i + 2];
-            c_pw[4 * i + 3] = (v4i){0, 0, 0, 0};
-        }
-        const v4i* tsrc = reinterpret_cast<const v4i*>(a.add_tab);
-        v4i* tdst = reinterpret_cast<v4i*>(lds_all);
-        for (int i = tid; i < 4096; i += NTHREADS) tdst[i] = tsrc[i];
-    }
-    __syncthreads();
-
-    const int lane = tid & 63;
-    const int wave = __builtin_amdgcn_readfirstlane(tid >> 6);
+    const v4i* src = reinterpret_cast<const v4i*>(a.cst);
+    for (int i = tid; i < nDWC / 12; i += NTHREADS) {
+        const v4i m = src[kDWC / 4 + 3 * i], c1 = src[kDWC / 4 + 3 * i + 1], sh = src[kDWC / 4 + 3 * i + 2];
+        const long c[4] = {rq64(c1.x), rq64(c1.y), rq64(c1.z), rq64(c1.w)};
+        c_dw[4 * i] = m;
+        c_dw[4 * i + 1] = (v4i){(int)c[0], (int)(c[0] >> 32), (int)c[1], (int)(c[1] >> 32)};
+        c_dw[4 * i + 2] = (v4i){(int)c[2], (int)(c[2] >> 32), (int)c[3], (int)(c[3] >> 32)};
+        c_dw[4 * i + 3] = (v4i){pack_shifts(sh - 1), 0, 0, 0};
+    }
+    for (int i = tid; i < 4 * NT; i += NTHREADS) {
+        c_pw[4 * i] = src[kPWC / 4 + 3 * i];
+        c_pw[4 * i + 1] = src[kPWC / 4 + 3 * i + 1];
+        c_pw[4 * i + 2] = src[kPWC / 4 + 3 * i + 2];
+        c_pw[4 * i + 3] = (v4i){0, 0, 0, 0};
+    }
+    const v4i* tsrc = reinterpret_cast<const v4i*>(a.add_tab);
+    v4i* tdst = reinterpret_cast<v4i*>(lds_all);
+    for (int i = tid; i < 4096; i += NTHREADS) tdst[i] = tsrc[i];
+}
+
+template <int R>
+__device__ __forceinline__ void strip_mf_walk(const Strip8Args& a, const unsigned char* lds_all, int lane, int chunk, int sx, int oh0, int steps, const Front2Ring& ring) {
+    constexpr int CIN = 32, COUT = 32, QL = 2, NT = 2, NW = 1;
+    constexpr int nDWW = 4 * QL * 12, nDWB = 4 * QL * 4, nDWC = 4 * QL * 12, nPWA = NT * NW * 64 * QL;
+    constexpr int kDWW = 0, kDWB = kDWW + nDWW, kDWC = kDWB + nDWB, kPWA = kDWC + nDWC, kPWB = kPWA + nPWA;
+    const unsigned char* add_tab = lds_all;
+    const v4i* c_dw = reinterpret_cast<const v4i*>(lds_all + 65536);
+    const v4i* c_pw = c_dw + nDWC / 3;
     const int n = lane & 15, g = lane >> 4;
     const int strips_x = a.OW >> 4;
-    const int rblocks = (a.OH + a.TH - 1) / a.TH;
-    int wid = xcd_tile(blockIdx.x, gridDim.x) * SPB + wave;
-    if (wid >= a.B * strips_x * rblocks) return;
-    const int sx = wid % strips_x;
-    wid /= strips_x;
-    const int ry = wid % rblocks;
-    const int chunk = wid / rblocks;
-    const int oh0 = ry * a.TH;
-    const int steps = (a.OH - oh0) < a.TH ? (a.OH - oh0) : a.TH;
     const int ow = sx * 16 + n;
 
     v4i dwa[2][3];
@@ -420,6 +454,9 @@
     const int voff_b = (ccol < 0 ? 0 : (ccol >= a.W ? a.W - 1 : ccol)) * CIN;
     const int voff_r = ow * CIN + 8 * g;
     const int voff_out = ow * COUT + 8 * g;
+    const int roff_b = voff_b / CIN * kF2Pitch, roff_r = ow * kF2Pitch + 8 * g;
+    int seen = 0;
+    bool gave_up = false;
     const int ir0 = oh0 - a.pt;
     const int rows_needed = steps + 2;
 
@@ -429,15 +466,25 @@
     v2i cen[3];
     auto row_ok = [&](int rr) { const int ir = ir0 + rr; return rr < rows_needed && ir >= 0 && ir < a.H; };
     auto issue = [&](int slot, int rr) {
-        if (row_ok(rr)) {
-            const int so = (ir0 + rr) * row_bytes;
-            rawb[slot][0] = __builtin_bit_cast(v4i, __builtin_amdgcn_raw_buffer_load_b128(rs_in, voff_b, so, 0));
-            rawb[slot][1] = __builtin_bit_cast(v4i, __builtin_amdgcn_raw_buffer_load_b128(rs_in, voff_b + 16, so, 0));
-            rawr[slot] = __builtin_bit_cast(v2i, __builtin_amdgcn_raw_buffer_load_b64(rs_in, voff_r, so, 0));
+        if constexpr (R == 0) {
+            if (row_ok(rr)) {
+                const int so = (ir0 + rr) * row_bytes;
+                rawb[slot][0] = __builtin_bit_cast(v4i, __builtin_amdgcn_raw_buffer_load_b128(rs_in, voff_b, so, 0));
+                rawb[slot][1] = __builtin_bit_cast(v4i, __builtin_amdgcn_raw_buffer_load_b128(rs_in, voff_b + 16, so, 0));
+                rawr[slot] = __builtin_bit_cast(v2i, __builtin_amdgcn_raw_buffer_load_b64(rs_in, voff_r, so, 0));
+            }
         }
     };
     auto consume = [&](int slot, int rr, int ti) {
         if (row_ok(rr)) {
+            if constexpr (R > 0) {
+                const int ir = ir0 + rr;
+                ring_wait(ring.produced, sx, strips_x, front2::need_produced(ir - 1, a.H), seen, gave_up);
+                const unsigned char* rp = ring.rows + front2::ring_row(ir, R) * kF2RowBytes;
+                rawb[slot][0] = *reinterpret_cast<const v4i*>(rp + roff_b);
+                rawb[slot][1] = *reinterpret_cast<const v4i*>(rp + roff_b + 16);
+                rawr[slot] = *reinterpret_cast<const v2i*>(rp + roff_r);
+            }
             brow[ti][0] = rawb[slot][0];
             brow[ti][1] = rawb[slot][1];
             if (outer) {
@@ -491,6 +538,7 @@
         }
         __builtin_amdgcn_raw_buffer_store_b64(__builtin_bit_cast(__attribute__((__vector_size__(2 * sizeof(int)))) int, (v2i){outw[0], outw[1]}), rs_out, voff_out,
                                               oh * a.OW * COUT, 0);
+        if constexpr (R > 0) ring_publish(ring.consumed + sx);
     };
 
     issue(0, 0);
@@ -510,6 +558,27 @@
             emit(u % 3, (u + 1) % 3, (u + 2) % 3, oh0 + k + u);
         }
     }
+}
+
+__global__ __launch_bounds__(512) __attribute__((amdgpu_waves_per_eu(4))) void i8_strip_mf_kernel(Strip8Args a) {
+    constexpr int SPB = 8;
+    extern __shared__ __attribute__((aligned(16))) unsigned char lds_all[];
+    const int tid = threadIdx.x;
+    strip_mf_stage<512>(a, lds_all, tid);
+    __syncthreads();
+
+    const int wave = __builtin_amdgcn_readfirstlane(tid >> 6);
+    const int strips_x = a.OW >> 4;
+    const int rblocks = (a.OH + a.TH - 1) / a.TH;
+    int wid = xcd_tile(blockIdx.x, gridDim.x) * SPB + wave;
+    if (wid >= a.B * strips_x * rblocks) return;
+    const int sx = wid % strips_x;
+    wid /= strips_x;
+    const int ry = wid % rblocks;
+    const int chunk = wid / rblocks;
+    const int oh0 = ry * a.TH;
+    const int steps = (a.OH - oh0) < a.TH ? (a.OH - oh0) : a.TH;
+    strip_mf_walk<0>(a, lds_all, tid & 63, chunk, sx, oh0, steps, Front2Ring{});
 }
 
 template <int CW, int NW, int COUT, int S, bool ADD, bool W8 = false>
@@ -526,21 +595,12 @@
 
 constexpr int kF_STA = 0, kF_STB = 64, kF_STC = 80, kF_DWW = 128, kF_DWB = 176, kF_DWC = 192, kF_PWA = 240, kF_PWB = 368, kF_PWC = 400;
 
-__global__ __launch_bounds__(256) void i8_front_strip_kernel(FrontStrip8Args a) {
-    const int tid = threadIdx.x;
-    const int lane = tid & 63;
-    const int wave = __builtin_amdgcn_readfirstlane(tid >> 6);
+constexpr int kFrontCqWords = 4 * 3 * 5;
+
+template <int R>
+__device__ __forceinline__ void front_strip_walk(const FrontStrip8Args& a, int lane, int chunk, int sx, int oh0, int nrows, v4i* cq, const Front2Ring& ring) {
     const int n = lane & 15, kq = lane >> 4;
     const int strips_x = a.OW >> 4;
-    const int rblocks = (a.OH + a.TH - 1) / a.TH;
-    int wid = xcd_tile(blockIdx.x, gridDim.x) * 4 + wave;
-    if (wid >= a.B * strips_x * rblocks) return;
-    const int sx = wid % strips_x;
-    wid /= strips_x;
-    const int ry = wid % rblocks;
-    const int chunk = wid / rblocks;
-    const int oh0 = ry * a.TH;
-    const int nrows = (a.OH - oh0) < a.TH ? (a.OH - oh0) : a.TH;
     const int ow = sx * 16 + n;
 
     const v4i* c4 = reinterpret_cast<const v4i*>(a.cst);
@@ -559,7 +619,6 @@
         dww[i][0] = v.x; dww[i][1] = v.y; dww[i][2] = v.z; dww[i][3] = v.w;
     }
     const v4i dwb = c4[kF_DWB / 4 + kq];
-    __shared__ v4i cq_lds[4][4][3][5];
     auto stage_quad = [&](v4i* q, v4i m, v4i c1, v4i sh, int lo, int hi) {
         int blo[4], bhi[4];
         long c[4];
@@ -577,7 +636,8 @@
         }
         return pack_shifts(sh - 1);
     };
-    const int dwe1 = stage_quad(cq_lds[wave][kq][0], c4[kF_DWC / 4 + kq * 3 + 0], c4[kF_DWC / 4 + kq * 3 + 1], c4[kF_DWC / 4 + kq * 3 + 2], a.dw_lo, a.dw_hi);
+    v4i* const my_cq = cq + kq * 15;
+    const int dwe1 = stage_quad(my_cq, c4[kF_DWC / 4 + kq * 3 + 0], c4[kF_DWC / 4 + kq * 3 + 1], c4[kF_DWC / 4 + kq * 3 + 2], a.dw_lo, a.dw_hi);
     long pwa[2];
     v4i pwb[2];
     int pwe1[2];
@@ -586,9 +646,8 @@
         pwa[t] = (long)(uint32_t)a.cst[kF_PWA + t * 64 + lane];
         pwb[t] = c4[kF_PWB / 4 + kq * 2 + t];
         const v4i* pc = c4 + kF_PWC / 4 + (kq * 2 + t) * 3;
-        pwe1[t] = stage_quad(cq_lds[wave][kq][1 + t], pc[0], pc[1], pc[2], a.pw_lo, a.pw_hi);
-    }
-    const v4i* my_cq = cq_lds[wave][kq][0];
+        pwe1[t] = stage_quad(my_cq + 5 * (1 + t), pc[0], pc[1], pc[2], a.pw_lo, a.pw_hi);
+    }
 
     const int zfe4 = (a.zp_fe & 0xff) * 0x01010101;
     const int zst4 = (a.zp_st & 0xff) * 0x01010101;
@@ -609,6 +668,8 @@
     constexpr int FD = 6;
     v2i raw[FD];
     TRow<1> T[3];
+    int seen = 0;
+    bool gave_up = false;
 
     auto fe_row = [&](int srel) { return sr0 + srel - 1 + kq; };
     const int fe_off0 = (sr0 - 1 + kq) * a.W0 + 4 * ow;
@@ -668,7 +729,13 @@
         }
         int outw[2];
         deposit_two_quads(outw[0], outw[1], ov[0], ov[1], pwe1[0], pwe1[1]);
-        __builtin_amdgcn_raw_buffer_store_b64(__builtin_bit_cast(__attribute__((__vector_size__(2 * sizeof(int)))) int, (v2i){outw[0], outw[1]}), rs_out, voff_out, oh * a.OW * 32, 0);
+        if constexpr (R > 0) {
+            ring_wait(ring.consumed, sx, strips_x, front2::need_consumed(oh, R), seen, gave_up);
+            *reinterpret_cast<v2i*>(ring.rows + front2::ring_row(oh, R) * kF2RowBytes + ow * kF2Pitch + 8 * kq) = (v2i){outw[0], outw[1]};
+            ring_publish(ring.produced + sx);
+        } else {
+            __builtin_amdgcn_raw_buffer_store_b64(__builtin_bit_cast(__attribute__((__vector_size__(2 * sizeof(int)))) int, (v2i){outw[0], outw[1]}), rs_out, voff_out, oh * a.OW * 32, 0);
+        }
     };
 
 #pragma unroll
@@ -688,6 +755,46 @@
             emit((2 * u) % 3, (2 * u + 1) % 3, (2 * u + 2) % 3, oh0 + k + u);
         }
     }
+}
+
+__global__ __launch_bounds__(256) void i8_front_strip_kernel(FrontStrip8Args a) {
+    __shared__ v4i cq_lds[4][kFrontCqWords];
+    const int tid = threadIdx.x;
+    const int wave = __builtin_amdgcn_readfirstlane(tid >> 6);
+    const int strips_x = a.OW >> 4;
+    const int rblocks = (a.OH + a.TH - 1) / a.TH;
+    int wid = xcd_tile(blockIdx.x, gridDim.x) * 4 + wave;
+    if (wid >= a.B * strips_x * rblocks) return;
+    const int sx = wid % strips_x;
+    wid /= strips_x;
+    const int ry = wid % rblocks;
+    const int chunk = wid / rblocks;
+    const int oh0 = ry * a.TH;
+    const int nrows = (a.OH - oh0) < a.TH ? (a.OH - oh0) : a.TH;
+    front_strip_walk<0>(a, tid & 63, chunk, sx, oh0, nrows, cq_lds[wave], Front2Ring{});
+}
+
+constexpr int kF2Cq = kMfLdsBytes, kF2Ctr = kF2Cq + 8 * kFrontCqWords * 16, kF2Ring = kF2Ctr + 64;
+constexpr size_t front2_lds_bytes(int R) { return (size_t)kF2Ring + 2 * (size_t)R * kF2RowBytes; }
+static_assert(kF2Ring % 16 == 0 && front2_lds_bytes(12) <= 160 * 1024, "the ring starts on a 16-byte boundary and fits the CU's LDS");
+
+template <int R>
+__global__ __launch_bounds__(1024) void i8_front2_kernel(FrontStrip8Args f, Strip8Args d) {
+    static_assert(R >= front2::kMinRing, "a ring below the minimum stalls");
+    extern __shared__ __attribute__((aligned(16))) unsigned char lds_all[];
+    const int tid = threadIdx.x;
+    unsigned* ctr = reinterpret_cast<unsigned*>(lds_all + kF2Ctr);
+    if (tid < 16) ctr[tid] = 0;
+    strip_mf_stage<1024>(d, lds_all, tid);
+    __syncthreads();
+
+    const int wave = __builtin_amdgcn_readfirstlane(tid >> 6);
+    const int slot = wave >> 3, sx = wave & 3;
+    const int chunk = xcd_tile(blockIdx.x, gridDim.x) * 2 + slot;
+    if (chunk >= f.B) return;
+    const Front2Ring ring{lds_all + kF2Ring + slot * (R * kF2RowBytes), ctr + 8 * slot, ctr + 8 * slot + 4};
+    if (wave & 4) strip_mf_walk<R>(d, lds_all, tid & 63, chunk, sx, 0, d.OH, ring);
+    else front_strip_walk<R>(f, tid & 63, chunk, sx, 0, f.OH, reinterpret_cast<v4i*>(lds_all + kF2Cq) + (4 * slot + sx) * kFrontCqWords, ring);
 }
 
 struct DwStream8Args {
@@ -1062,6 +1169,29 @@
     hipLaunchKernelGGL(i8_front_strip_kernel, dim3((unsigned)((waves + 3) / 4)), dim3(256), 0, s, a);
 }
 
+bool i8_front2_supported(const FrontStrip8Args& f, const Strip8Args& d) {
+    return g_opt.i8_strip && g_opt.i8_strip_mfdw && g_opt.i8_strip_th == 0 && f.H0 == 64 && f.W0 == 256 && f.OH == 32 && f.OW == kF2Cols && d.H == f.OH &&
+           d.W == f.OW && d.OH == d.H && d.OW == d.W && d.pt == 1 && d.pl == 1 && d.add.enabled && d.add_tab && d.B == f.B && f.B > 0;
+}
+
+template <int R>
+static bool launch_front2(const FrontStrip8Args& f, const Strip8Args& d, hipStream_t s) {
+    if (!ensure_dynamic_lds(reinterpret_cast<const void*>(i8_front2_kernel<R>), front2_lds_bytes(R))) return false;
+    hipLaunchKernelGGL(i8_front2_kernel<R>, dim3((unsigned)((f.B + 1) / 2)), dim3(1024), front2_lds_bytes(R), s, f, d);
+    return true;
+}
+
+bool launch_i8_front2(const FrontStrip8Args& f, const Strip8Args& d, hipStream_t s) {
+    if (!i8_front2_supported(f, d)) return false;
+    return g_opt.i8_front2 == 8 ? launch_front2<8>(f, d, s) : launch_front2<12>(f, d, s);
+}
+
+long front2_giveups() {
+    unsigned n = 0;
+    if (hipDeviceSynchronize() != hipSuccess || hipMemcpyFromSymbol(&n, HIP_SYMBOL(g_front2_giveups), sizeof n) != hipSuccess) return -1;
+    return (long)n;
+}
+
 struct PwDw8Args {
     const int8_t* x; int8_t* y;
     const int8_t* pw_w; const int32_t* pw_b; const int32_t* pw_mult; const int32_t* pw_shift;
diff --git a/birdnet-stm32_amd/csrc/bn_kernels.h b/birdnet-stm32_amd/csrc/bn_kernels.h
--- a/birdnet-stm32_amd/csrc/bn_kernels.h
+++ b/birdnet-stm32_amd/csrc/bn_kernels.h
@@ -38,6 +38,7 @@
     int stft_rowmajor = 0;
     int i8_mid_split = 1;
     int i8_strip_mfdw = 1;
+    int i8_front2 = 1;
     int stft_exact = 2;
     int stft_guard = 0;
     int stft_audit = 0;
@@ -312,6 +313,8 @@
 void launch_i8_front_strip(FrontStrip8Args a, hipStream_t s);
 bool i8_strip_supported(int Cin, int Cout, int stride, int OW, bool add);
 void launch_i8_strip(Strip8Args a, int Cin, int Cout, int stride, hipStream_t s);
+bool launch_i8_front2(const FrontStrip8Args& f, const Strip8Args& d, hipStream_t s);
+long front2_giveups();
 struct EmbOut {
     void* emb;
     int f32, zp;
diff --git a/birdnet-stm32_amd/csrc/bn_ops.h b/birdnet-stm32_amd/csrc/bn_ops.h
--- a/birdnet-stm32_amd/csrc/bn_ops.h
+++ b/birdnet-stm32_amd/csrc/bn_ops.h
@@ -160,7 +160,7 @@
 static_assert(i8_mean::P_END <= BN_OP_EMB_ZP, "i8_mean: fields run into the cross-kind entries");
 static_assert(i8_fc::P_END <= BN_OP_TAIL_TAG, "i8_fc: fields run into the cross-kind entries");
 static_assert(i8_head::P_END <= BN_OP_TAIL_TAG, "i8_head: fields run into the cross-kind entries");
-static_assert(i8_front::P_END <= BN_OP_TAIL_TAG, "i8_front: fields run into the cross-kind entries");
+static_assert(i8_front::P_END <= BN_OP_FRONT2_DIST, "i8_front: fields run into the cross-kind entries");
 static_assert(i8_tail::P_END <= BN_OP_EMB_ZP && (int)i8_tail::F_END <= BN_OP_EMB_SCALE, "i8_tail: fields run into the cross-kind entries");
 static_assert(i8_scale::P_END <= BN_OP_TAIL_TAG, "i8_scale: fields run into the cross-kind entries");
 static_assert(i8_maxnorm::P_END <= BN_OP_TAIL_TAG, "i8_maxnorm: fields run into the cross-kind entries");
diff --git a/birdnet-stm32_amd/csrc/bn_plan_run.hip b/birdnet-stm32_amd/csrc/bn_plan_run.hip
--- a/birdnet-stm32_amd/csrc/bn_plan_run.hip
+++ b/birdnet-stm32_amd/csrc/bn_plan_run.hip
@@ -291,6 +291,17 @@
         return r;
     }
 
+    bool strip8_args(const OpRec& d, const DwPw8Args& r, Strip8Args& q) const {
+        namespace k = op::i8_dwpw;
+        if (!(d.p[k::strip] && d.t[k::strip_cst] >= 0 && g_opt.i8_strip && r.has_dw && !r.transposed && r.sh == r.sw &&
+              i8_strip_supported(r.Cin, r.Cout, r.sh, r.OW, r.add.enabled != 0) && (!r.add.enabled || (r.res == r.x && d.t[k::add_tab] >= 0))))
+            return false;
+        const int off = r.add.enabled ? 128 : 0;
+        q = Strip8Args{r.x, r.y, t32(d, k::strip_cst), B, r.H, r.W, r.OH, r.OW, 0, r.pt, r.pl, r.dw_zp_in, r.dw_amin, r.dw_amax, r.pw_amin + off,
+                       r.pw_amax + off, r.pw_zp_out, r.add, r.add.enabled ? t8(d, k::add_tab) : nullptr};
+        return true;
+    }
+
     float* gap_target(size_t di) {
         const OpRec& d = m->ops[di];
         cand_for = (size_t)-1;
@@ -475,11 +486,7 @@
                 return BN_OK;
             }
         }
-        if (p[k::strip] && o->t[k::strip_cst] >= 0 && g_opt.i8_strip && r.has_dw && !r.transposed && r.sh == r.sw &&
-            i8_strip_supported(r.Cin, r.Cout, r.sh, r.OW, r.add.enabled != 0) && (!r.add.enabled || (r.res == r.x && o->t[k::add_tab] >= 0))) {
-            const int off = r.add.enabled ? 128 : 0;
-            Strip8Args q{r.x, r.y, t32(*o, k::strip_cst), B, r.H, r.W, r.OH, r.OW, 0, r.pt, r.pl, r.dw_zp_in, r.dw_amin, r.dw_amax, r.pw_amin + off,
-                         r.pw_amax + off, r.pw_zp_out, r.add, r.add.enabled ? t8(*o, k::add_tab) : nullptr};
+        if (Strip8Args q; strip8_args(*o, r, q)) {
             launch_i8_strip(q, r.Cin, r.Cout, r.sh, s);
             return BN_OK;
         }
@@ -503,6 +510,21 @@
         if (p[k::strip] && o->t[k::strip_cst] >= 0 && g_opt.i8_strip && i8_front_strip_supported(q.H0, q.W0, q.C, q.N, q.OH, q.OW)) {
             FrontStrip8Args fa{(const int8_t*)in0, (int8_t*)out, t32(*o, k::strip_cst), B, q.H0, q.W0, q.OH, q.OW, 0, q.stem_zp_in, q.stem_amin, q.stem_amax,
                                q.stem_zp_out, q.dw_amin, q.dw_amax, q.pw_amin, q.pw_amax};
+            const int dist = p[BN_OP_FRONT2_DIST];
+            if (tag(*o) == BN_FRONT2_HEAD && g_opt.i8_front2 && dist > 0 && oi + (size_t)dist < n) {
+                namespace dk = op::i8_dwpw;
+                const size_t di = oi + (size_t)dist;
+                const OpRec& d = m->ops[di];
+                if (same_path(*o, d) && d.kind == BN_OP_I8_DWPW && tag(d) == 0 && m->prep[di] && d.in0 == o->out && d.in1 == o->out && d.out != o->in0 &&
+                    d.out != o->out && d.p[dk::Cin] == 32 && d.p[dk::Cout] == 32 && d.p[dk::sh] == 1 && d.p[dk::has_add] && !d.p[dk::has_lut]) {
+                    const DwPw8Args r = dwpw8_args(d, di);
+                    if (Strip8Args sa; strip8_args(d, r, sa) && launch_i8_front2(fa, sa, s)) {
+                        front2_done = di;
+                        fused_into(di);
+                        return BN_OK;
+                    }
+                }
+            }
             launch_i8_front_strip(fa, s);
             return BN_OK;
         }
diff --git a/include/birdnet_hip.h b/include/birdnet_hip.h
--- a/include/birdnet_hip.h
+++ b/include/birdnet_hip.h
@@ -139,6 +139,7 @@
 BN_API int bn_debug_mid_form(const bn_model* model, int* form, int* lds_bytes);
 BN_API int bn_debug_mid_plan(const bn_model* model, int* out, int n);
 BN_API int bn_debug_mid_split_giveups(bn_ctx* ctx, int64_t* count);
+BN_API int bn_debug_front2_giveups(bn_ctx* ctx, int64_t* count);
 
 BN_API int bn_debug_requant(bn_ctx* ctx, const int32_t* d_x, const int32_t* d_mult, const int32_t* d_shift, int n, int mode,
                      int zero_point, int32_t* d_out, void* stream);
```

After: 2.382 million. About the same (-0.6%).
